# probcomp/PClean

Hardware: AMD Instinct MI355X
Metric: rows/sec per Gibbs sweep on 1M-row synthetic hospital; F1 vs ground truth (higher is better)
Workload: dtype f64

## Files before the change

### pclean_amd/csrc/eval.hip

```cpp
#include "sweep_internal.h"
#include "static_tiles.h"

int build_gauss_dev(pclean_ctx* ctx, const pclean_gauss& g, const CandTable* t, GaussDev& d) {
  memset(&d, 0, sizeof d);
  if (g.x_col < 0 || g.x_col >= ctx->n_xcols) return pclean_fail(ctx, PCLEAN_ERR_ARG, "gauss: numeric column out of range");
  const MeanTable& m = ctx->mean[g.mean_table];
  if (!m.valid) return pclean_fail(ctx, PCLEAN_ERR_STATE, "gauss: mean table %d not set", g.mean_table);
  d.on = 1;
  d.n_dims = g.n_dims;
  d.n_locals = g.n_locals;
  d.x = ctx->xnum.p + (size_t)g.x_col * ctx->n_rows + ctx->active_begin;
  d.mu = m.v.p;
  for (int i = 0; i < g.n_dims; ++i) {
    d.src_kind[i] = g.src_kind[i];
    d.src_slot[i] = g.src[i];
    d.stride[i] = g.stride[i];
    d.src_ptr[i] = nullptr;
    if (g.src_kind[i] == PCLEAN_GSRC_CAND) {
      if (!t || g.src[i] < 0 || g.src[i] >= t->n_cols) return pclean_fail(ctx, PCLEAN_ERR_ARG, "gauss: candidate column out of range");
      d.src_ptr[i] = t->cols.p + (size_t)g.src[i] * t->n_rows;
    } else if (g.src_kind[i] == PCLEAN_GSRC_OBS) {
      if (g.src[i] < 0 || g.src[i] >= ctx->n_cols) return pclean_fail(ctx, PCLEAN_ERR_ARG, "gauss: observed column out of range");
      d.src_ptr[i] = ctx->obs.p + (size_t)g.src[i] * ctx->n_rows + ctx->active_begin;
    }
// ... 663 lines not shown
  fr.zero_row = f.zero_row.p;
  fr.alive = f.alive.p;
  fr.prior_e = c.leaf ? nullptr : f.prior_e.p;
  fr.prior_n = f.prior_n.p;
  fr.logc_m1 = c.leaf ? nullptr : t.logc_m1.p;
  fr.counts = c.leaf ? nullptr : t.counts.p;
  memcpy(fr.scal, t.scal, sizeof fr.scal);
}

static int try_fast_root(pclean_ctx* ctx, int block_id, int node_id, FastRootDev& fr, bool ev_mode = false) {
  if (node_id >= 64) return 0;
  const Block& b = ctx->block[block_id];
  const pclean_node& n = b.nodes[node_id];
  FastRootCall c{ctx, block_id, node_id, ev_mode, EvalSwitches::once(), b, n, ctx->cand[n.table], n.kind == PCLEAN_NODE_LEAF, fr};
  if (!fast_root_eligible(c)) return 0;
  int rc = ensure_compact_tables(c);
  if (!rc) rc = ensure_root_priors(c);
  if (rc) return rc;
  prefilter_bound(c);
  rc = ensure_obs_rowmajor(c);
  if (rc) return rc;
  fill_fast_root(c);
  return 1;
}

static int eval_node_lse(pclean_ctx* ctx, int block_id, int node_id, const ItemList& il, const int32_t* excl,
                         uint64_t seed, uint32_t sweep, double* lse_out);
static int make_item_groups(pclean_ctx* ctx, int block_id, int node_id, const ItemList& il, const int32_t* excl,
                            ItemGroups& g, int split_m = 0, bool want_members = true);

static double subtree_ub(pclean_ctx* ctx, const Block& b, int node_id) {
  const pclean_node& n = b.nodes[node_id];
  if (node_id < (int)b.node_gauss.size() && b.node_gauss[node_id] >= 0) return INFINITY;
  CandTable& t = ctx->cand[n.table];
  if (n.kind == PCLEAN_NODE_LEAF) {
    if (t.h_lse_ver != t.version) {
      double m = -INFINITY, acc = 0.0;
      for (double v : t.h_logc_full) m = std::max(m, v);
      if (m > -INFINITY)
        for (double v : t.h_logc_full) acc += std::exp(v - m);
      t.h_lse = m > -INFINITY ? m + std::log(acc) + 1e-9 : -INFINITY;
      t.h_lse_ver = t.version;
    }
    return t.h_lse;
  }
  double sum = 0.0;
  for (int c = 0; c < n.n_children; ++c) sum += subtree_ub(ctx, b, b.children[n.child_begin + c]);
  return std::max(0.0, sum);
}

__global__ void scatter_f64_kernel(int n, const int32_t* list, const double* src, double* dst) {
  const int j = blockIdx.x * blockDim.x + threadIdx.x;
  if (j < n) dst[list[j]] = src[j];
}
__global__ void sub_items_kernel(int n, const int32_t* list, const int32_t* p_row, const int32_t* p_ctx,
                                 const int32_t* p_excl, const int32_t* p_ev_lo, const int32_t* p_ev_hi,
                                 const int32_t* p_rng, const int32_t* p_origin, int32_t* row, int32_t* ctxv,
                                 int32_t* excl, int32_t* ev_lo, int32_t* ev_hi, int32_t* rng, int32_t* origin) {
  const int j = blockIdx.x * blockDim.x + threadIdx.x;
  if (j >= n) return;
  const int s = list[j];
  row[j] = p_row ? p_row[s] : s;
  excl[j] = p_excl ? p_excl[s] : -1;
  for (int c = 0; c < PCLEAN_MAX_CTX; ++c) ctxv[j * PCLEAN_MAX_CTX + c] = p_ctx ? p_ctx[(size_t)s * PCLEAN_MAX_CTX + c] : 0;
  if (p_ev_lo) {
    ev_lo[j] = p_ev_lo[s];
    ev_hi[j] = p_ev_hi[s];
  }
  if (p_rng) rng[j] = p_rng[s];
  if (origin) origin[j] = p_origin ? p_origin[s] : s;
}

__global__ void group_rep_items_kernel(int n, const int32_t* list, const int32_t* grp_off, const int32_t* members,
                                       const int32_t* p_row, const int32_t* p_ctx, const int32_t* p_excl, int32_t* row,
                                       int32_t* ctxv, int32_t* excl) {
  const int j = blockIdx.x * blockDim.x + threadIdx.x;
  if (j >= n) return;
  const int g = list ? list[j] : j;
  const int s = members[grp_off[g]];
  row[j] = p_row ? p_row[s] : s;
  excl[j] = p_excl ? p_excl[s] : -1;
  for (int c = 0; c < PCLEAN_MAX_CTX; ++c) ctxv[j * PCLEAN_MAX_CTX + c] = p_ctx ? p_ctx[(size_t)s * PCLEAN_MAX_CTX + c] : 0;
}
__global__ void group_scatter_f64_kernel(int n, const int32_t* list, const int32_t* grp_off, const int32_t* members,
                                         const double* src, double* dst) {
  const int j = blockIdx.x * blockDim.x + threadIdx.x;
  if (j >= n) return;
  const int g = list ? list[j] : j;
  const double v = src[j];
  const int hi = grp_off[g + 1];
  for (int mi = grp_off[g]; mi < hi; ++mi) dst[members[mi]] = v;
}

__global__ void member_scatter_f64_kernel(int n_pos, const int32_t* uid, const int32_t* members, const double* src, double* dst) {
  const int mi = blockIdx.x * blockDim.x + threadIdx.x;
  if (mi < n_pos) dst[members[mi]] = src[uid[mi] - 1];
}

struct EvalCall {
  pclean_ctx* ctx;
  const int block_id, node_id;
  const ItemList& il;
  const int32_t* excl;
  const uint64_t seed;
  const uint32_t sweep;
  const int n_draws;
  double* lse_out;
  int32_t* draws_out;
  double* scores_out;
  const double* snew_override;
  const bool time_it;
  Block& b;
  const pclean_node& n;
  SweepState* s;
  const uint32_t site;
  const EvalSwitches sw;
  SweepState::LazyReq lazy_req;
  bool lazy_ok = false;
  int fast_split_m = 0;
  bool tabulated = false;
  NodeDev nd;
  ItemsDev it;
  ChildrenDev ch{};
  FastRootDev fr;
  int fast = 0, fast_ev = 0;
  ItemGroups g_pre;
  ItemGroups ggrp;
  bool fast_tried = false, groups_tried = false;
  const double* pre_score = nullptr;
  const int32_t* pre_obs = nullptr;
  int32_t* oflag = nullptr;
  int32_t* over_list = nullptr;
  unsigned int* over_count = nullptr;
  bool list_mode = false, ev_list_mode = false;
};

static int eval_begin(EvalCall& c) {
  SweepState* s = c.s;
  const ItemList& il = c.il;
  c.lazy_req = s->lazy_req;
  s->lazy_req = SweepState::LazyReq();
  s->lazy_out.valid = false;
  c.lazy_ok = c.lazy_req.on && !c.sw.cached.no_lazy && c.n_draws > 1 && !il.rng_row && !il.ev_lo;
  const bool lazy_sure = c.lazy_ok && (size_t)il.n * ROOT_LZ_CAP * 12 <= ((size_t)4 << 30);
  c.fast_split_m = (lazy_sure && !c.sw.cached.lazy_split) ? 0 : std::max(4, 256 / std::max(c.n_draws, 1));
  int rc = build_node_dev(c.ctx, c.b, c.node_id, c.nd);
  if (rc) return rc;
  c.it = ItemsDev{il.n, 0, il.row, il.ctx, c.excl, c.n_draws == 1 ? il.particle : nullptr, s->row_offset + c.ctx->active_begin,
                  nullptr, il.ev_lo, il.ev_hi, il.ev_rows, il.ev_ctx, il.rng_row, nullptr, nullptr, il.draw_is, il.draw_ds,
                  nullptr, nullptr};
  if (il.ev_lo) {
    rc = ensure_agg(c.ctx, c.block_id, c.node_id, il, &c.it.agg);
    if (rc) return rc;
    c.it.ev_item = il.origin;
  }
  c.tabulated = node_has_tabulated(c.b, c.n);
  return PCLEAN_OK;
}

static int launch_enum_scratch(EvalCall& c, const ItemsDev& it, double* scores_out, const ProductDev* product) {
  double* sc_tmp = nullptr;
  if (!scores_out && !product) {
    const size_t sc_n = pclean_enum_split_scores(c.nd, it);
    if (sc_n && !(sc_tmp = scratch<double>(c.ctx, sc_n))) return pclean_fail(c.ctx, PCLEAN_ERR_HIP, "scratch alloc failed");
  }
  return pclean_launch_enum(c.ctx, c.nd, it, c.ch, c.seed, c.sweep, c.site, c.n_draws, c.lse_out, scores_out, c.draws_out, sc_tmp,
                            product);
}

static int sub_items(EvalCall& c, unsigned int n, const int32_t* list, int32_t* row2, int32_t* ctx2, int32_t* excl2, ItemList& sil) {
  const ItemList& il = c.il;
  int32_t* evl2 = il.ev_lo ? scratch<int32_t>(c.ctx, n) : nullptr;
  int32_t* evh2 = il.ev_lo ? scratch<int32_t>(c.ctx, n) : nullptr;
  int32_t* rng2 = il.rng_row ? scratch<int32_t>(c.ctx, n) : nullptr;
  int32_t* org2 = il.ev_lo ? scratch<int32_t>(c.ctx, n) : nullptr;
  if (!row2 || !ctx2 || !excl2 || (il.ev_lo && (!evl2 || !evh2 || !org2)) || (il.rng_row && !rng2))
    return pclean_fail(c.ctx, PCLEAN_ERR_HIP, "scratch alloc failed");
  hipLaunchKernelGGL(sub_items_kernel, grid1(n), dim3(256), 0, c.ctx->stream, (int)n, list, il.row, il.ctx, c.excl, il.ev_lo,
                     il.ev_hi, il.rng_row, il.origin, row2, ctx2, excl2, evl2, evh2, rng2, org2);
  sil = ItemList{(int)n, row2, il.ctx ? ctx2 : nullptr, nullptr, org2, evl2, evh2, il.ev_rows, il.ev_ctx, rng2};
  return PCLEAN_OK;
}

struct OpenUnits {
  bool grouped = false;
  int n_all = 0;
  unsigned int n_need = 0;
  int32_t* list = nullptr;
  ItemList sil;
  const int32_t* sexcl = nullptr;
  bool sub() const { return n_need < (unsigned int)n_all; }
};

static int children_bounds(EvalCall& c, GateDev& gt, int* n_open, bool* gate) {
  for (int k = 0; k < c.n.n_children; ++k) {
    const int cid = c.b.children[c.n.child_begin + k];
    const pclean_node& cn = c.b.nodes[cid];
    if (cn.kind == PCLEAN_NODE_LEAF && cn.cacheable) {
      const int rc = ensure_leaf_cache(c.ctx, c.block_id, cid, &c.ch.arr[k], &c.ch.obs_col[k], &c.ch.n_obs[k]);
      if (rc) return rc;
      gt.cache[k] = c.ch.arr[k];
      gt.obs_col[k] = c.ch.obs_col[k];
      gt.n_obs[k] = c.ch.n_obs[k];
      gt.ub[k] = 0.0;
      if (c.il.ev_lo) gt.ub[k] = subtree_ub(c.ctx, c.b, cid);
    } else {
      ++*n_open;
      gt.cache[k] = nullptr;
      gt.ub[k] = subtree_ub(c.ctx, c.b, cid);
      if (!(gt.ub[k] < INFINITY)) *gate = false;
    }
    if (c.il.ev_lo && !(gt.ub[k] < INFINITY)) *gate = false;
  }
  return PCLEAN_OK;
}

static int gate_and_compact(EvalCall& c, const GateDev& gt, SweepState::GateStat* gstat, OpenUnits& u) {
  pclean_ctx* ctx = c.ctx;
  SweepState* s = c.s;
  ProfScope ps(ctx, "gate_new_branch");
  const int n = u.n_all;
  int32_t* flag = scratch<int32_t>(ctx, n);
  u.list = scratch<int32_t>(ctx, n);
  double* sc = u.grouped ? scratch<double>(ctx, n) : nullptr;
  int32_t* ow = u.grouped ? scratch<int32_t>(ctx, (size_t)n * PCLEAN_MAX_TERMS) : nullptr;
  if (!flag || !u.list || (u.grouped && (!sc || !ow))) return pclean_fail(ctx, PCLEAN_ERR_HIP, "scratch alloc failed");
  if (u.grouped) {
    ItemsDev itg = c.it;
    itg.n = n;
    itg.grp_off = c.g_pre.grp_off;
    itg.members = c.g_pre.members;
    if (c.time_it && s->evg0) (void)hipEventRecord(s->evg0, ctx->stream);
    const int rc = pclean_launch_group_gate(ctx, c.fr, itg, gt, flag, sc, ow);
    if (rc) return rc;
    if (c.time_it && s->evg0) {
      (void)hipEventRecord(s->evg1, ctx->stream);
      s->gate_timed = true;
    }
  } else {
    if (s->counter.alloc(4)) return pclean_fail(ctx, PCLEAN_ERR_HIP, "device alloc failed");
    const int rc = pclean_launch_gate(ctx, c.nd, c.it, gt, flag);
    if (rc) return rc;
  }
  unsigned int* need_ctr = fresh_counter(ctx);
  if (!need_ctr) return pclean_fail(ctx, PCLEAN_ERR_HIP, "counter bank: device alloc failed");
  hipLaunchKernelGGL(compact_new_kernel, grid1(n), dim3(256), 0, ctx->stream, (size_t)n, flag, 1, need_ctr, u.list, nullptr);
  PCLEAN_READ_COUNT(ctx, need_ctr, &u.n_need);
  if (u.grouped) {
    c.pre_score = sc;
    c.pre_obs = ow;
  }
  if (gstat) {
    gstat->all_need_run = !u.sub() ? gstat->all_need_run + 1 : 0;
    if (gstat->all_need_run >= 3) {
      gstat->skip = 16;
      gstat->all_need_run = 2;
    }
  }
  if (!u.sub()) u.list = nullptr;
  return PCLEAN_OK;
}

static int open_sublist(EvalCall& c, OpenUnits& u) {
  const ItemList& il = c.il;
  if (!u.grouped) {
    u.sil = il;
    u.sexcl = c.excl;
  }
  if (u.n_need == 0 || (!u.grouped && !u.sub())) return PCLEAN_OK;
  int32_t* row2 = scratch<int32_t>(c.ctx, u.n_need);
  int32_t* ctx2 = scratch<int32_t>(c.ctx, (size_t)u.n_need * PCLEAN_MAX_CTX);
  int32_t* excl2 = scratch<int32_t>(c.ctx, u.n_need);
  if (u.grouped) {
    if (!row2 || !ctx2 || !excl2) return pclean_fail(c.ctx, PCLEAN_ERR_HIP, "scratch alloc failed");
    hipLaunchKernelGGL(group_rep_items_kernel, grid1(u.n_need), dim3(256), 0, c.ctx->stream, (int)u.n_need, u.list, c.g_pre.grp_off,
                       c.g_pre.members, il.row, il.ctx, c.excl, row2, ctx2, excl2);
    u.sil = ItemList{(int)u.n_need, row2, il.ctx ? ctx2 : nullptr, nullptr, nullptr};
  } else {
    const int rc = sub_items(c, u.n_need, u.list, row2, ctx2, excl2, u.sil);
    if (rc) return rc;
  }
  u.sexcl = excl2;
  return PCLEAN_OK;
}

static int eval_open_children(EvalCall& c, const OpenUnits& u) {
  pclean_ctx* ctx = c.ctx;
  const ItemList& il = c.il;
  const ItemList& sil = u.sil;
  const CandTable& t = ctx->cand[c.n.table];
  for (int k = 0; k < c.n.n_children; ++k) {
    const int cid = c.b.children[c.n.child_begin + k];
    const pclean_node& cn = c.b.nodes[cid];
    if (cn.kind == PCLEAN_NODE_LEAF && cn.cacheable) continue;
    double* child_lse = scratch<double>(ctx, il.n);
    if (!child_lse) return pclean_fail(ctx, PCLEAN_ERR_HIP, "scratch alloc failed");
    c.ch.arr[k] = child_lse;
    c.ch.obs_col[k] = nullptr;
    if (u.sub()) {
      hipLaunchKernelGGL(fill_f64_kernel, grid1(il.n), dim3(256), 0, ctx->stream, child_lse, (size_t)il.n, -__builtin_inf());
      if (u.n_need == 0) continue;
    }
    const int32_t* child_excl = nullptr;
    if (cn.kind == PCLEAN_NODE_FK && u.sexcl) {
      if (cn.parent_fk_col < 0 || cn.parent_fk_col >= t.n_cols)
        return pclean_fail(ctx, PCLEAN_ERR_ARG, "node %d: parent_fk_col out of range", cid);
      int32_t* ce = scratch<int32_t>(ctx, sil.n);
      if (!ce) return pclean_fail(ctx, PCLEAN_ERR_HIP, "scratch alloc failed");
      hipLaunchKernelGGL(derive_excl_kernel, grid1(sil.n), dim3(256), 0, ctx->stream, sil.n, u.sexcl, t.counts.p,
                         t.cols.p + (size_t)cn.parent_fk_col * t.n_rows, ce);
      child_excl = ce;
    }
    double* dst = child_lse;
    if (u.grouped || u.sub()) {
      dst = scratch<double>(ctx, sil.n);
      if (!dst) return pclean_fail(ctx, PCLEAN_ERR_HIP, "scratch alloc failed");
    }
    const int rc = eval_node_lse(ctx, c.block_id, cid, sil, child_excl, c.seed, c.sweep, dst);
    if (rc) return rc;
    if (u.grouped && !u.list && c.g_pre.uid && c.fast_split_m == 0)
      hipLaunchKernelGGL(member_scatter_f64_kernel, grid1(il.n), dim3(256), 0, ctx->stream, il.n, c.g_pre.uid, c.g_pre.members, dst,
                         child_lse);
    else if (u.grouped)
      hipLaunchKernelGGL(group_scatter_f64_kernel, grid1(sil.n), dim3(256), 0, ctx->stream, sil.n, u.list, c.g_pre.grp_off,
                         c.g_pre.members, dst, child_lse);
    else if (u.sub())
      hipLaunchKernelGGL(scatter_f64_kernel, grid1(sil.n), dim3(256), 0, ctx->stream, sil.n, u.list, dst, child_lse);
  }
  return PCLEAN_OK;
}

static int new_row_branch(EvalCall& c) {
  pclean_ctx* ctx = c.ctx;
  const pclean_node& n = c.n;
  const ItemList& il = c.il;
  if (n.kind != PCLEAN_NODE_FK) return PCLEAN_OK;
  if (ctx->prior_mode) {
    c.ch.n = 0;
    return PCLEAN_OK;
  }
  if (c.snew_override) {
    c.ch.n = 1;
    c.ch.arr[0] = c.snew_override;
    c.ch.obs_col[0] = nullptr;
    return PCLEAN_OK;
  }
  if (n.n_children > PCLEAN_MAX_CHILDREN) return pclean_fail(ctx, PCLEAN_ERR_CAPACITY, "too many children");
  c.ch.n = n.n_children;
  GateDev gt{};
  gt.n = n.n_children;
  bool gate = c.excl && !c.scores_out && il.n >= c.sw.live.gate_min() && !c.sw.live.no_gate();
  SweepState::GateStat* gstat = (gate && c.node_id < 64 && c.sweep < 0x7ffffff0u && !il.ev_lo && !c.sw.live.gate_always())
                                    ? &c.s->gate_stat[c.block_id * 64 + c.node_id] : nullptr;
  if (gstat && gstat->skip > 0) {
    --gstat->skip;
    gate = false;
    gstat = nullptr;
  }
  int n_open = 0;
  int rc = children_bounds(c, gt, &n_open, &gate);
  if (rc) return rc;
  OpenUnits u;
  if (n_open > 0 && c.n_draws > 0 && c.excl && !c.scores_out && !ctx->force_generic && !c.nd.g.on && !c.tabulated && !il.rng_row &&
      !il.ev_lo && !c.sw.cached.no_group_gate) {
    c.fast = try_fast_root(ctx, c.block_id, c.node_id, c.fr);
    if (c.fast < 0) return c.fast;
    c.fast_tried = true;
    if (c.fast) {
      rc = make_item_groups(ctx, c.block_id, c.node_id, il, c.excl, c.g_pre, c.fast_split_m);
      if (rc) return rc;
      c.groups_tried = true;
      u.grouped = c.g_pre.n_groups > 0;
    }
  }
  u.n_all = u.grouped ? c.g_pre.n_groups : il.n;
  u.n_need = (unsigned int)u.n_all;
  if (gate && n_open > 0) {
    rc = gate_and_compact(c, gt, gstat, u);
    if (rc) return rc;
  }
  rc = open_sublist(c, u);
  if (rc) return rc;
  return eval_open_children(c, u);
}

static int leaf_coarse_draw(EvalCall& c, bool* done) {
  pclean_ctx* ctx = c.ctx;
  *done = c.n.kind == PCLEAN_NODE_LEAF && c.n.cacheable && !c.il.ev_lo && !c.scores_out && !ctx->force_generic && !ctx->obs_override &&
          !c.sw.cached.no_coarse && !c.nd.g.on && !c.tabulated && !ctx->prior_mode;
  if (!*done) return PCLEAN_OK;
  const double* cache = nullptr;
  const int32_t* ocol = nullptr;
  int n_obs = 0;
  const int rc = ensure_leaf_cache(ctx, c.block_id, c.node_id, &cache, &ocol, &n_obs);
  if (rc) return rc;
  ProfScope ps(ctx, "option_list_coarse_draw");
  return pclean_launch_leaf_coarse_draw(ctx, c.nd, c.it, ocol, n_obs, pclean_leaf_coarse_blocks(c.nd.n_cand), cache,
                                        c.b.leaf_m[c.node_id].p, c.b.leaf_U[c.node_id].p, c.b.leaf_coarse[c.node_id].p, c.seed,
                                        c.sweep, PCLEAN_SITE_NODE(c.block_id, c.node_id), c.n_draws, c.lse_out, c.draws_out);
}

static int choose_compact_path(EvalCall& c) {
  pclean_ctx* ctx = c.ctx;
  const ItemList& il = c.il;
  const bool small_lse = !c.sw.cached.no_small_generic && c.n_draws == 0 && il.n <= 1024 && !il.ev_lo &&
                         (size_t)(c.nd.n_cand + 2) * 8 + (16 + 64) * 8 <= (size_t)160 * 1024;
  if (c.fast_tried || c.scores_out || c.snew_override || ctx->force_generic || c.nd.g.on || c.tabulated || ctx->prior_mode || small_lse)
    return PCLEAN_OK;
  if (!il.ev_lo)
    c.fast = try_fast_root(ctx, c.block_id, c.node_id, c.fr);
  else if ((c.n.kind == PCLEAN_NODE_LEAF || (il.n >= c.sw.cached.ev_slot_min_items && !c.sw.live.no_fast_ev_slots())) && c.n_draws <= 1 &&
           !c.sw.live.no_fast_ev())
    c.fast_ev = try_fast_root(ctx, c.block_id, c.node_id, c.fr, true);
  if (c.fast < 0) return c.fast;
  if (c.fast_ev < 0) return c.fast_ev;
  if (c.fast_ev) {
    bool any = false;
    for (int i = 0; i < c.fr.n_terms; ++i) any |= c.fr.terms[i].comp != nullptr;
    if (!any) c.fast_ev = 0;
  }
  return PCLEAN_OK;
}

static int group_for_launch(EvalCall& c) {
  const ItemList& il = c.il;
  const int nc = c.nd.n_cand + (c.n.kind == PCLEAN_NODE_FK ? 1 : 0);
  const bool lds_kernel = (size_t)((nc + 1) & ~1) * 8 + (16 + 64) * 8 <= 160 * 1024;
  if (!(c.n_draws > 0 && !c.scores_out && !c.snew_override && !c.ctx->force_generic && !il.rng_row && !il.ev_lo &&
        (c.fast || lds_kernel)))
    return PCLEAN_OK;
  ItemGroups g = c.g_pre;
  if (!c.groups_tried) {
    const int rc = make_item_groups(c.ctx, c.block_id, c.node_id, il, c.excl, g, c.fast ? c.fast_split_m : 0);
    if (rc) return rc;
  }
  if (g.n_groups > 0) {
    c.it.n = g.n_groups;
    c.it.grp_off = g.grp_off;
    c.it.members = g.members;
    if (c.fast && c.fast_split_m == 0) c.it.grp_uid = g.uid;
    c.ggrp = g;
  }
  return PCLEAN_OK;
}

static void note_root_stats(EvalCall& c) {
  pclean_root_stats& rs = c.ctx->root_stats;
  rs = pclean_root_stats{};
  rs.fast = c.fast;
  rs.n_items = c.il.n;
  rs.n_groups = c.it.n;
  rs.n_cand = c.nd.n_cand;
  rs.n_terms = c.n.n_terms;
  rs.n_draws = c.n_draws;
  rs.pre_scored = c.pre_score ? 1 : 0;
  if (c.fast) {
    const FastRootDev& fr = c.fr;
    rs.kpad = fr.kscan;
    rs.cstride = std::min(fr.cstride, (((fr.kscan + 63) >> 6) + 15) & ~15);
    rs.n_pre = fr.n_pre;
    for (int p = 0; p < 3; ++p) rs.pre_obs_col[p] = p < fr.n_pre ? c.b.terms[c.n.term_begin + fr.pre[p]].obs_col : -1;
  }
}

static int launch_generic(EvalCall& c) {
  ProductDev prd;
  const bool product = pclean_product_plan(c.ctx->cand[c.n.table], c.nd, c.it, &prd);
  ProfScope ps(c.ctx, c.n.kind == PCLEAN_NODE_FK ? "enum_fk_generic" : (product ? "enum_leaf_product" : "enum_leaf_generic"));
  if (c.time_it) (void)hipEventRecord(c.s->ev0, c.ctx->stream);
  const int rc = launch_enum_scratch(c, c.it, c.scores_out, product ? &prd : nullptr);
  if (c.time_it) (void)hipEventRecord(c.s->ev1, c.ctx->stream);
  return rc;
}

static int overflow_setup(EvalCall& c) {
  pclean_ctx* ctx = c.ctx;
  SweepState* s = c.s;
  const ItemList& il = c.il;
  c.oflag = scratch<int32_t>(ctx, il.n);
  if (!c.oflag || s->counter.alloc(4)) return pclean_fail(ctx, PCLEAN_ERR_HIP, "scratch alloc failed");
  c.list_mode = c.fast && !c.sw.cached.no_fast_over && pclean_overflow_fast_ok(c.fr, c.it) && s->over_rec.size() < OVER_SLOTS &&
                s->over_ctr.p != nullptr;
// ... 1050 lines not shown
    if (k0 == k[0] && e[1] == k[1] && e[2] == k[2]) {
      lse_out[i] = m.vals[slot];
      miss = 0;
      break;
    }
    slot = (slot + 1) & m.cap_mask;
  }
  miss_flag[i] = miss;
}
__global__ void memo_insert_kernel(int n, const int32_t* list, KeyColsDev kc, const int32_t* row, const int32_t* ctxv,
                                   MemoDev m, const double* __restrict__ src) {
  const int j = blockIdx.x * blockDim.x + threadIdx.x;
  if (j >= n) return;
  if (*m.count >= m.max_fill) return;
  const int i = list ? list[j] : j;
  uint64_t k[3];
  memo_key(kc, row ? row[i] : i, ctxv, (size_t)i, k);
  uint32_t slot = memo_hash(k) & m.cap_mask;
  for (int p = 0; p < MEMO_PROBES; ++p) {
    unsigned long long* e = (unsigned long long*)(m.keys + (size_t)slot * 3);
    const unsigned long long old = atomicCAS(e, ~0ull, (unsigned long long)k[0]);
    if (old == ~0ull) {
      e[1] = k[1];
      e[2] = k[2];
      m.vals[slot] = src[j];
      atomicAdd(m.count, 1u);
      return;
    }
    slot = (slot + 1) & m.cap_mask;
  }
}

static int eval_node_lse_core(pclean_ctx* ctx, int block_id, int node_id, const ItemList& il, const int32_t* excl,
                              uint64_t seed, uint32_t sweep, double* lse_out);

static int eval_node_lse(pclean_ctx* ctx, int block_id, int node_id, const ItemList& il, const int32_t* excl,
                         uint64_t seed, uint32_t sweep, double* lse_out) {
  Block& b = ctx->block[block_id];
  const pclean_node& n = b.nodes[node_id];
  SweepState* s = st(ctx);
  std::set<int> cols;
  bool use_ctx = false;
  static const bool no_memo = getenv("PCLEAN_NO_MEMO") != nullptr;
  const bool memo_ok = !no_memo && n.kind == PCLEAN_NODE_LEAF && !il.ev_lo && il.n >= 4096 && node_id < 64 &&
                       subtree_key(ctx, b, node_id, cols, use_ctx) &&
                       (int)cols.size() + (use_ctx ? PCLEAN_MAX_CTX : 0) <= 6 && (!use_ctx || il.ctx);
  if (!memo_ok) return eval_node_lse_core(ctx, block_id, node_id, il, excl, seed, sweep, lse_out);
  ProfScope ps(ctx, "option_marginal_memo");
  uint64_t ver = ctx->cand[n.table].version;
  for (int i = 0; i < n.n_terms; ++i) {
    const pclean_term& tm = b.terms[n.term_begin + i];
    ver = ver * 1000003ull + ctx->pair[tm.pair_table].version;
    if (tm.ctx_slot >= 0) ver = ver * 1000003ull + (uint64_t)(tm.fn_table + 1);
    if (tm.dens_kind == PCLEAN_DENS_NAME3) {
      for (const Name3Term& x : b.name3)
        if (x.term == n.term_begin + i) ver = ver * 1000003ull + ctx->pair[x.suffix_table].version;
      ver = ver * 1000003ull + b.version;
    }
  }
  SweepState::LeafMemo& mm = s->memo[block_id * 64 + node_id];
  const int cap = 1 << 21;
  if (mm.cap != cap) {
    if (mm.keys.alloc((size_t)cap * 3) || mm.vals.alloc(cap) || mm.count.alloc(4))
      return pclean_fail(ctx, PCLEAN_ERR_HIP, "device alloc failed (memo)");
    mm.cap = cap;
    mm.ver = 0;
  }
  if (mm.ver != ver) {
    HIPCHK(ctx, hipMemsetAsync(mm.keys.p, 0xff, (size_t)cap * 3 * sizeof(uint64_t), ctx->stream));
    HIPCHK(ctx, hipMemsetAsync(mm.count.p, 0, sizeof(unsigned int), ctx->stream));
    mm.ver = ver;
  }
  MemoDev md{mm.keys.p, mm.vals.p, mm.count.p, (unsigned int)(cap - 1), (unsigned int)(cap / 2)};
  KeyColsDev kc{};
  kc.use_ctx = use_ctx ? 1 : 0;
  for (int c : cols) kc.col[kc.n_cols++] = ctx->obs.p + (size_t)c * ctx->n_rows + ctx->active_begin;
  const int N = il.n;
  int32_t* flag = scratch<int32_t>(ctx, N);
  int32_t* list = scratch<int32_t>(ctx, N);
  if (!flag || !list || s->counter.alloc(4)) return pclean_fail(ctx, PCLEAN_ERR_HIP, "scratch alloc failed");
  hipLaunchKernelGGL(memo_lookup_kernel, grid1(N), dim3(256), 0, ctx->stream, N, kc, il.row, il.ctx, md, lse_out, flag);
  unsigned int* miss_ctr = fresh_counter(ctx);
  if (!miss_ctr) return pclean_fail(ctx, PCLEAN_ERR_HIP, "counter bank: device alloc failed");
  hipLaunchKernelGGL(compact_new_kernel, grid1(N), dim3(256), 0, ctx->stream, (size_t)N, flag, 1, miss_ctr, list, nullptr);
  unsigned int n_miss = 0;
  PCLEAN_READ_COUNT(ctx, miss_ctr, &n_miss);
  if (n_miss == 0) return PCLEAN_OK;
  if (n_miss == (unsigned int)N) {
    int rc = eval_node_lse_core(ctx, block_id, node_id, il, excl, seed, sweep, lse_out);
    if (rc) return rc;
    hipLaunchKernelGGL(memo_insert_kernel, grid1(N), dim3(256), 0, ctx->stream, N, (const int32_t*)nullptr, kc, il.row,
                       il.ctx, md, lse_out);
    return PCLEAN_OK;
  }
  int32_t* row2 = scratch<int32_t>(ctx, n_miss);
  int32_t* ctx2 = scratch<int32_t>(ctx, (size_t)n_miss * PCLEAN_MAX_CTX);
  int32_t* excl2 = scratch<int32_t>(ctx, n_miss);
  double* dst = scratch<double>(ctx, n_miss);
  if (!row2 || !ctx2 || !excl2 || !dst) return pclean_fail(ctx, PCLEAN_ERR_HIP, "scratch alloc failed");
  hipLaunchKernelGGL(sub_items_kernel, grid1(n_miss), dim3(256), 0, ctx->stream, (int)n_miss, list, il.row, il.ctx, excl,
                     (const int32_t*)nullptr, (const int32_t*)nullptr, (const int32_t*)nullptr, (const int32_t*)nullptr, row2,
                     ctx2, excl2, (int32_t*)nullptr, (int32_t*)nullptr, (int32_t*)nullptr, (int32_t*)nullptr);
  ItemList sil{(int)n_miss, row2, il.ctx ? ctx2 : nullptr, nullptr, nullptr};
  int rc = eval_node_lse_core(ctx, block_id, node_id, sil, excl ? excl2 : nullptr, seed, sweep, dst);
  if (rc) return rc;
  hipLaunchKernelGGL(scatter_f64_kernel, grid1(n_miss), dim3(256), 0, ctx->stream, (int)n_miss, list, dst, lse_out);
  hipLaunchKernelGGL(memo_insert_kernel, grid1(n_miss), dim3(256), 0, ctx->stream, (int)n_miss, list, kc, il.row, il.ctx, md,
                     dst);
  return PCLEAN_OK;
}

static int eval_node_lse_core(pclean_ctx* ctx, int block_id, int node_id, const ItemList& il, const int32_t* excl,
                              uint64_t seed, uint32_t sweep, double* lse_out) {
  ItemGroups g;
  int rc0 = make_item_groups(ctx, block_id, node_id, il, excl, g, 0, false);
  if (rc0) return rc0;
  if (g.n_groups == 0)
    return eval_node(ctx, block_id, node_id, il, excl, seed, sweep, 0, lse_out, nullptr, nullptr, nullptr, false);
  const int n = il.n;
  const int32_t n_unique = g.n_groups;
  int32_t* uid_of_item = scratch<int32_t>(ctx, n);
  if (!uid_of_item) return pclean_fail(ctx, PCLEAN_ERR_HIP, "scratch alloc failed");
  int32_t* row2 = scratch<int32_t>(ctx, n_unique);
  int32_t* ctx2 = scratch<int32_t>(ctx, (size_t)n_unique * PCLEAN_MAX_CTX);
  int32_t* excl2 = scratch<int32_t>(ctx, n_unique);
  double* lse_u = scratch<double>(ctx, n_unique);
  if (!row2 || !ctx2 || !excl2 || !lse_u) return pclean_fail(ctx, PCLEAN_ERR_HIP, "scratch alloc failed");
  if (g.hg_incl)
    hipLaunchKernelGGL(hg_unique_kernel, grid1(n), dim3(256), 0, ctx->stream, n, g.hg_incl, g.hg_rep, g.hg_slot_of, il.row, il.ctx,
                       excl, uid_of_item, row2, ctx2, excl2);
  else
    hipLaunchKernelGGL(item_unique_kernel, grid1(n), dim3(256), 0, ctx->stream, n, g.members, g.head, g.uid, il.row, il.ctx, excl,
                       uid_of_item, row2, ctx2, excl2);
  ItemList il2;
  il2.n = n_unique;
  il2.row = row2;
  il2.ctx = il.ctx ? ctx2 : nullptr;
  int rc = eval_node(ctx, block_id, node_id, il2, excl ? excl2 : nullptr, seed, sweep, 0, lse_u, nullptr, nullptr, nullptr,
                     false);
  if (rc) return rc;
  hipLaunchKernelGGL(gather_f64_kernel, grid1(n), dim3(256), 0, ctx->stream, n, uid_of_item, lse_u, lse_out);
  return PCLEAN_OK;
}

int sample_children(pclean_ctx* ctx, int block_id, int node_id, const ItemList& il, const int32_t* excl,
                           uint64_t seed, uint32_t sweep, int32_t* vals, int n_nodes) {
  Block& b = ctx->block[block_id];
  const pclean_node& n = b.nodes[node_id];
  const CandTable& t = ctx->cand[n.table];
  for (int c = 0; c < n.n_children; ++c) {
    const int cid = b.children[n.child_begin + c];
    const pclean_node& cn = b.nodes[cid];
    int32_t* draws = scratch<int32_t>(ctx, il.n);
    if (!draws) return pclean_fail(ctx, PCLEAN_ERR_HIP, "scratch alloc failed");
    const int32_t* child_excl = nullptr;
    if (cn.kind == PCLEAN_NODE_FK && excl) {
      int32_t* ce = scratch<int32_t>(ctx, il.n);
      if (!ce) return pclean_fail(ctx, PCLEAN_ERR_HIP, "scratch alloc failed");
      hipLaunchKernelGGL(derive_excl_kernel, grid1(il.n), dim3(256), 0, ctx->stream, il.n, excl, t.counts.p,
                         t.cols.p + (size_t)cn.parent_fk_col * t.n_rows, ce);
      child_excl = ce;
    }
    int rc = eval_node(ctx, block_id, cid, il, child_excl, seed, sweep, 1, nullptr, draws, nullptr, nullptr, false);
    if (rc) return rc;
    hipLaunchKernelGGL(scatter_vals_kernel, grid1(il.n), dim3(256), 0, ctx->stream, il.n, il.origin, draws, n_nodes,
                       cid, vals);
    if (cn.kind == PCLEAN_NODE_FK && cn.n_children > 0) {
      unsigned int* new_ctr = fresh_counter(ctx);
      if (!new_ctr) return pclean_fail(ctx, PCLEAN_ERR_HIP, "counter bank: device alloc failed");
      hipLaunchKernelGGL(compact_new_kernel, grid1(il.n), dim3(256), 0, ctx->stream, (size_t)il.n, draws, 0, new_ctr, nullptr,
                         nullptr);
      unsigned int cnt = 0;
      PCLEAN_READ_COUNT(ctx, new_ctr, &cnt);
      if (cnt) {
        int32_t* list = scratch<int32_t>(ctx, cnt);
        int32_t* row = scratch<int32_t>(ctx, cnt);
        int32_t* cx = scratch<int32_t>(ctx, (size_t)cnt * PCLEAN_MAX_CTX);
        int32_t* part = scratch<int32_t>(ctx, cnt);
        int32_t* org = scratch<int32_t>(ctx, cnt);
        int32_t* sub_excl = scratch<int32_t>(ctx, cnt);
        if (!list || !row || !cx || !part || !org || !sub_excl) return pclean_fail(ctx, PCLEAN_ERR_HIP, "scratch alloc failed");
        unsigned int* list_ctr = fresh_counter(ctx);
        if (!list_ctr) return pclean_fail(ctx, PCLEAN_ERR_HIP, "counter bank: device alloc failed");
        hipLaunchKernelGGL(compact_new_kernel, grid1(il.n), dim3(256), 0, ctx->stream, (size_t)il.n, draws, 1, list_ctr, list, nullptr);
        int32_t* evl = il.ev_lo ? scratch<int32_t>(ctx, cnt) : nullptr;
        int32_t* evh = il.ev_lo ? scratch<int32_t>(ctx, cnt) : nullptr;
        int32_t* rng = il.rng_row ? scratch<int32_t>(ctx, cnt) : nullptr;
        if ((il.ev_lo && (!evl || !evh)) || (il.rng_row && !rng)) return pclean_fail(ctx, PCLEAN_ERR_HIP, "scratch alloc failed");
        hipLaunchKernelGGL(sublist_items_kernel, grid1(cnt), dim3(256), 0, ctx->stream, (int)cnt, list, il.row, il.ctx,
                           il.particle, il.origin, row, cx, part, org, il.ev_lo, il.ev_hi, il.rng_row, evl, evh, rng);
        if (child_excl)
          hipLaunchKernelGGL(gather_i32_kernel, grid1(cnt), dim3(256), 0, ctx->stream, (int)cnt, list, child_excl,
                             sub_excl);
        ItemList sub{(int)cnt, row, cx, part, org, evl, evh, il.ev_rows, il.ev_ctx, rng};
        rc = sample_children(ctx, block_id, cid, sub, child_excl ? sub_excl : nullptr, seed, sweep, vals, n_nodes);
        if (rc) return rc;
      }
    }
  }
  return PCLEAN_OK;
}

int prefetch_fast_root(pclean_ctx* ctx, int block_id, int node_id, hipStream_t side) {
  hipStream_t saved = ctx->stream;
  ctx->stream = side;
  FastRootDev fr;
  const int rc = try_fast_root(ctx, block_id, node_id, fr);
  ctx->stream = saved;
  return rc < 0 ? rc : PCLEAN_OK;
}

extern "C" int pclean_prepare(pclean_ctx* ctx, uint32_t ev_blocks) {
  if (!ctx) return PCLEAN_ERR_ARG;
  HIPCHK(ctx, hipSetDevice(ctx->device));
  {
    const int rcb = begin_call(ctx);
    if (rcb) return rcb;
  }
  for (int bi = 0; bi < PCLEAN_MAX_BLOCKS; ++bi) {
    Block& b = ctx->block[bi];
    if (!b.valid || b.is_score) continue;
    for (int node = 0; node < (int)b.nodes.size() && node < 64; ++node) {
      const pclean_node& n = b.nodes[node];
      if (n.table < 0 || n.table >= PCLEAN_MAX_TABLES || !ctx->cand[n.table].valid) continue;
      if (node < (int)b.node_gauss.size() && b.node_gauss[node] >= 0) continue;
      FastRootDev fr;
      const int rc = try_fast_root(ctx, bi, node, fr, n.kind == PCLEAN_NODE_LEAF && ((ev_blocks >> bi) & 1u));
      if (rc < 0) return rc;
      if (n.kind == PCLEAN_NODE_LEAF && n.cacheable && n.n_terms == 1 && b.terms[n.term_begin].ctx_slot < 0) {
        const double* cache;
        const int32_t* ocol;
        int n_obs;
        const int rcl = ensure_leaf_cache(ctx, bi, node, &cache, &ocol, &n_obs);
        if (rcl) return rcl;
      }
    }
  }
  PCLEAN_SYNC(ctx);
  return PCLEAN_OK;
}

int ensure_plan_dev(pclean_ctx* ctx, int block_id) {
  SweepState* s = st(ctx);
  BlockRun& r = s->run[block_id];
  const Block& b = ctx->block[block_id];
  const int nn = (int)b.nodes.size();
  std::vector<int32_t> kind(nn), nrows(nn), cmb(nn);
  std::vector<const int32_t*> cols(nn);
  for (int i = 0; i < nn; ++i) {
    const CandTable& t = ctx->cand[b.nodes[i].table];
    kind[i] = b.nodes[i].kind;
    nrows[i] = t.n_rows;
    cmb[i] = b.nodes[i].colmap_begin;
    cols[i] = t.cols.p;
  }
  if (r.plan_ready && r.plan_sig_block == b.version && r.plan_sig_nrows == nrows && r.plan_sig_cols == cols && r.plan_sig_colmap == b.colmap.size() &&
// ... 24 lines not shown
```

### pclean_amd/csrc/sweep.hip

```cpp
#include <optional>

#include "sweep_internal.h"
#include "tail_tiles.h"

int g_pclean_sync_count = 0;

__global__ void publish_count_kernel(const unsigned int* __restrict__ src, volatile unsigned int* __restrict__ dst, unsigned int seq) {
  dst[0] = *src;
  __threadfence_system();
  dst[1] = seq;
}
int read_count(pclean_ctx* ctx, const void* dev, void* out, const char* func, int line) {
  SweepState* s = st(ctx);
  static const bool no_poll = getenv("PCLEAN_NO_POLL") != nullptr;
  static const bool trace = getenv("PCLEAN_TRACE_SYNC") != nullptr;
  if (trace) fprintf(stderr, "[pclean sync %d] %s:%d (count)\n", ++g_pclean_sync_count, func, line);
  if (!no_poll && !s->h_poll) {
    if (hipHostMalloc((void**)&s->h_poll, 64, hipHostMallocMapped | hipHostMallocCoherent) != hipSuccess) s->h_poll = nullptr;
    if (s->h_poll) {
      s->h_poll[0] = s->h_poll[1] = 0;
      if (hipHostGetDevicePointer((void**)&s->d_poll, (void*)s->h_poll, 0) != hipSuccess) {
        (void)hipHostFree((void*)s->h_poll);
        s->h_poll = nullptr;
      }
    }
  }
  if (no_poll || !s->h_poll) {
    HIPCHK(ctx, hipMemcpyAsync(out, dev, 4, hipMemcpyDeviceToHost, ctx->stream));
    HIPCHK(ctx, hipStreamSynchronize(ctx->stream));
    return PCLEAN_OK;
  }
  const unsigned int seq = ++s->poll_seq;
  hipLaunchKernelGGL(publish_count_kernel, dim3(1), dim3(1), 0, ctx->stream, (const unsigned int*)dev, s->d_poll, seq);
  if (s->on_first_wait) {
    std::function<int()> f;
    f.swap(s->on_first_wait);
    const int rcf = f();
    if (rcf) return rcf;
  }
  volatile unsigned int* h = s->h_poll;
  for (long spins = 0; h[1] != seq; ++spins)
    if (spins > 2000000) {
      HIPCHK(ctx, hipStreamSynchronize(ctx->stream));
      if (h[1] != seq) return pclean_fail(ctx, PCLEAN_ERR_HIP, "count read-back: the publishing kernel did not run");
    }
  *(unsigned int*)out = h[0];
  return PCLEAN_OK;
}

__device__ int32_t resolve_new_value(const PlanDev& pl, int node, int col, const int32_t* vals) {
  for (int depth = 0; depth < 16; ++depth) {
    const int cn = pl.colmap[2 * (pl.colmap_begin[node] + col)];
    const int cc = pl.colmap[2 * (pl.colmap_begin[node] + col) + 1];
    if (cn < 0) return -1;
    const int choice = vals[cn];
    if (pl.kind[cn] == PCLEAN_NODE_LEAF) return pl.cols[cn][choice];
    if (choice >= 0) return pl.cols[cn][(size_t)cc * pl.n_rows[cn] + choice];
    node = cn;
    col = cc;
  }
  return -1;
}




struct CtxSrc {
  int32_t n_ctx;
  const int32_t* pchoice[PCLEAN_MAX_CTX];
  const int32_t* pnewpos[PCLEAN_MAX_CTX];
  const int32_t* vals[PCLEAN_MAX_CTX];
  int32_t n_nodes[PCLEAN_MAX_CTX];
  const int32_t* root_col[PCLEAN_MAX_CTX];
  int32_t col[PCLEAN_MAX_CTX];
  PlanDev plan[PCLEAN_MAX_CTX];
};

__global__ void gather_ctx_kernel(size_t NP, CtxSrc cs, int32_t* it_ctx) {
  size_t t = (size_t)blockIdx.x * blockDim.x + threadIdx.x;
  if (t >= NP) return;
  for (int s = 0; s < cs.n_ctx; ++s) {
    int32_t v;
    const int choice = cs.pchoice[s][t];
    if (choice >= 0)
      v = cs.root_col[s][choice];
    else
      v = resolve_new_value(cs.plan[s], 0, cs.col[s], cs.vals[s] + (size_t)cs.pnewpos[s][t] * cs.n_nodes[s]);
    it_ctx[(size_t)s * NP + t] = v;
  }
}

__global__ void ctx_count_kernel(int N, int P, int n_ctx, const int32_t* __restrict__ it_ctx, int32_t* __restrict__ rep,
                                 int32_t* __restrict__ n_distinct) {
  const int i = blockIdx.x * blockDim.x + threadIdx.x;
  if (i >= N) return;
  const size_t NP = (size_t)N * P;
  int nd = 0;
  for (int p = 0; p < P; ++p) {
    const size_t sp = (size_t)p * N + i;
    int c[PCLEAN_MAX_CTX];
    for (int k = 0; k < PCLEAN_MAX_CTX; ++k) c[k] = k < n_ctx ? it_ctx[(size_t)k * NP + sp] : 0;
    int q = 0;
    for (; q < p; ++q) {
      bool same = true;
      for (int k = 0; k < PCLEAN_MAX_CTX; ++k)
        if (k < n_ctx) same &= it_ctx[(size_t)k * NP + (size_t)q * N + i] == c[k];
      if (same) break;
    }
    rep[sp] = q;
    nd += q == p ? 1 : 0;
  }
  n_distinct[i] = nd;
}
__global__ void ctx_fill_kernel(int N, int P, int n_ctx, const int32_t* __restrict__ it_ctx, const int32_t* __restrict__ rep,
                                const int32_t* __restrict__ off, const int32_t* __restrict__ cur_b,
                                int32_t* __restrict__ slot_item, int32_t* __restrict__ row, int32_t* __restrict__ ctxv,
                                int32_t* __restrict__ excl) {
  const int i = blockIdx.x * blockDim.x + threadIdx.x;
  if (i >= N) return;
  const size_t NP = (size_t)N * P;
  int j = off[i];
  for (int p = 0; p < P; ++p) {
    const size_t sp = (size_t)p * N + i;
    const int q = rep[sp];
    if (q == p) {
      row[j] = i;
      excl[j] = cur_b ? cur_b[i] : -1;
      for (int k = 0; k < PCLEAN_MAX_CTX; ++k) ctxv[(size_t)j * PCLEAN_MAX_CTX + k] = k < n_ctx ? it_ctx[(size_t)k * NP + sp] : 0;
      slot_item[sp] = j++;
    } else {
// ... 44 lines not shown
            it_ctx[(size_t)s * NP + (size_t)(p0 + u) * N + i] = v[u];
            all_same &= v[u] == c0[s];
          }
      }
    }
    row[i] = i;
    excl[i] = cur_b ? cur_b[i] : -1;
    for (int k = 0; k < PCLEAN_MAX_CTX; ++k) ctxv[(size_t)i * PCLEAN_MAX_CTX + k] = c0[k];
    if (all_same) {
      for (int p = 0; p < P; ++p) slot_item[(size_t)p * N + i] = i;
    } else {
      slot_item[i] = i;
      for (int p = 1; p < P; ++p) {
        const size_t sp = (size_t)p * N + i;
        int q = 0;
        for (; q < p; ++q) {
          bool same = true;
          for (int k = 0; k < cs.n_ctx; ++k) same &= it_ctx[(size_t)k * NP + (size_t)q * N + i] == it_ctx[(size_t)k * NP + sp];
          if (same) break;
        }
        if (q == p) {
          slot_item[sp] = -1 - (int)mine;
          ++mine;
        } else {
          slot_item[sp] = slot_item[(size_t)q * N + i];
        }
      }
    }
  }
  const unsigned long long any = __ballot(mine != 0u);
  unsigned int incl = mine;
  if (any) {
    for (int o = 1; o < 64; o <<= 1) {
      const unsigned int x = __shfl_up(incl, o, 64);
      if (lane >= o) incl += x;
    }
  }
  if (lane == 63) wcnt[wave] = any ? incl : 0u;
  __syncthreads();
  if (threadIdx.x == 0) {
    const unsigned int tot = wcnt[0] + wcnt[1] + wcnt[2] + wcnt[3];
    bbase = tot ? atomicAdd(n_extra, tot) : 0u;
  }
  __syncthreads();
  if (!mine) return;
  unsigned int base = bbase + incl - mine;
  for (int w = 0; w < wave; ++w) base += wcnt[w];
  for (int p = 1; p < P; ++p) {
    const size_t sp = (size_t)p * N + i;
    const int si = slot_item[sp];
    if (si >= 0) continue;
    int q = 0;
    for (; q < p; ++q) {
      bool same = true;
      for (int k = 0; k < cs.n_ctx; ++k) same &= it_ctx[(size_t)k * NP + (size_t)q * N + i] == it_ctx[(size_t)k * NP + sp];
      if (same) break;
    }
    if (q < p) {
      slot_item[sp] = slot_item[(size_t)q * N + i];
      continue;
    }
    const unsigned int e = base + (unsigned int)(-1 - si);
    const int j = N + (int)e;
    slot_item[sp] = j;
    if (e < (unsigned int)extra_cap) {
      row[j] = i;
      excl[j] = cur_b ? cur_b[i] : -1;
      for (int k = 0; k < PCLEAN_MAX_CTX; ++k) ctxv[(size_t)j * PCLEAN_MAX_CTX + k] = k < cs.n_ctx ? it_ctx[(size_t)k * NP + sp] : 0;
    }
  }
}
#define PU_T 1024
__global__ __launch_bounds__(PU_T) void particle_update_kernel(int N, int P, const int32_t* __restrict__ draws_rm,
                                                              const double* __restrict__ lse,
                                                              const int32_t* __restrict__ slot_item,
                                                              const int32_t* __restrict__ draws_item,
                                                              const double* __restrict__ lse_item,
                                                              const int32_t* __restrict__ cur_b,
                                                              int32_t* __restrict__ pchoice, double* __restrict__ w,
                                                              unsigned int* __restrict__ n_new,
                                                              int32_t* __restrict__ new_list,
                                                              int32_t* __restrict__ pnewpos, int first,
                                                              const int32_t* __restrict__ emit_rows, int only_emit,
                                                              int stage_stride, const double* __restrict__ w_uni, int skip_w) {
  __shared__ unsigned int wsum[PU_T / 64];
  __shared__ unsigned int bbase;
  extern __shared__ int32_t pu_stage[];
  const int i = blockIdx.x * blockDim.x + threadIdx.x;
  const int lane = threadIdx.x & 63, wave = threadIdx.x >> 6;
  if (stage_stride > 0) {
    const int r0 = blockIdx.x * PU_T;
    const int n_here = min(PU_T, N - r0);
    const int n_words = n_here * P;
    const int32_t* src = draws_rm + (size_t)r0 * P;
    for (int k = threadIdx.x; k < n_words; k += PU_T) {
      const int row = k / P, col = k - row * P;
      pu_stage[row * stage_stride + col] = src[k];
    }
    __syncthreads();
  }
  uint64_t newmask = 0;
  if (i < N && !(only_emit && !emit_rows[i])) {
    const int keep = cur_b ? cur_b[i] : -1;
    for (int p = 0; p < P; ++p) {
      const size_t sp = (size_t)p * N + i;
      int d;
      double l;
      if (slot_item) {
        const int item = slot_item[sp];
        d = draws_item[(size_t)item * P + p];
        l = lse_item[item];
      } else {
        d = stage_stride > 0 ? pu_stage[threadIdx.x * stage_stride + p] : draws_rm[(size_t)i * P + p];
        l = lse[i];
      }
      const int c = (p == 0 && keep >= 0) ? keep : d;
      pchoice[sp] = c;
      if (!skip_w) w[sp] = first ? 0.0 + l : (w_uni ? (0.0 + w_uni[i]) + l : w[sp] + l);
      if (c == PCLEAN_CHOICE_NEW) newmask |= 1ull << p;
      if (p == 0 && !(l > -__builtin_inf())) atomicOr(n_new, 0x80000000u);
    }
    if (emit_rows && !emit_rows[i]) newmask = 0;
  }
  const unsigned int mine = (unsigned int)__popcll(newmask);
  unsigned int incl = mine;
  for (int o = 1; o < 64; o <<= 1) {
    const unsigned int x = __shfl_up(incl, o, 64);
    if (lane >= o) incl += x;
  }
  if (lane == 63) wsum[wave] = incl;
  __syncthreads();
  if (threadIdx.x == 0) {
    unsigned int total = 0;
    for (int k = 0; k < PU_T / 64; ++k) total += wsum[k];
    bbase = total ? (atomicAdd(n_new, total) & 0x7fffffffu) : 0u;
  }
  __syncthreads();
  if (!mine) return;
  unsigned int pos = bbase + incl - mine;
  for (int k = 0; k < wave; ++k) pos += wsum[k];
  for (uint64_t mm = newmask; mm; mm &= mm - 1) {
    const int p = __builtin_ctzll(mm);
    const size_t sp = (size_t)p * N + i;
    new_list[pos] = (int32_t)sp;
    pnewpos[sp] = (int32_t)pos;
    ++pos;
  }
}

__global__ void chosen_new_kernel(int N, const int32_t* __restrict__ chosen, const int32_t* __restrict__ pchoice,
                                  unsigned int* __restrict__ counter, int32_t* __restrict__ list,
                                  int32_t* __restrict__ pnewpos) {
  const int i = blockIdx.x * blockDim.x + threadIdx.x;
  if (i >= N) return;
  const size_t s = (size_t)chosen[i] * N + i;
  if (pchoice[s] != PCLEAN_CHOICE_NEW) return;
  const unsigned int pos = atomicAdd(counter, 1u);
  list[pos] = (int32_t)s;
  pnewpos[s] = (int32_t)pos;
}

struct SrcDev {
  const int32_t* pchoice;
  const int32_t* pnewpos;
  const int32_t* vals;
  const int32_t* root_col;
  int32_t n_nodes, col;
  PlanDev plan;
};
__device__ __forceinline__ int src_value(const SrcDev& s, size_t slot) {
  const int choice = s.pchoice[slot];
  if (choice >= 0) return s.root_col[choice];
  return resolve_new_value(s.plan, 0, s.col, s.vals + (size_t)s.pnewpos[slot] * s.n_nodes);
}
struct ScoreTermDev {
  const int32_t* obs_col;
  const uint8_t* pair;
  const int32_t* nopt_fn;
  int32_t n_lat, other_val;
  SrcDev val, key;
};
struct ScoreBlockDev {
  int32_t n_terms, prob_nb;
  const int32_t* prob_fn;
  const double* prob_same;
  const double* prob_diff;
  const double* logn;
  SrcDev pa, pb;
  ScoreTermDev t[8];
};
__global__ void score_block_kernel(int n_rows, int P, ScoreBlockDev sb, double* w) {
  size_t slot = (size_t)blockIdx.x * blockDim.x + threadIdx.x;
  if (slot >= (size_t)n_rows * P) return;
  const int i = (int)(slot % n_rows);
  const int pidx = sb.prob_fn[(size_t)src_value(sb.pa, slot) * sb.prob_nb + src_value(sb.pb, slot)];
  double acc = 0.0;
  for (int k = 0; k < sb.n_terms; ++k) {
    const ScoreTermDev& t = sb.t[k];
    const int val = src_value(t.val, slot);
    const int o = t.obs_col[i];
    double dens;
    if (o < 0)
      dens = val >= t.other_val ? -1000.0 : 0.0;
    else if (t.pair[(size_t)o * t.n_lat + val] == 0)
      dens = sb.prob_same[pidx];
    else
      dens = sb.prob_diff[pidx] - sb.logn[t.nopt_fn[src_value(t.key, slot)]];
    acc += dens;
  }
  w[slot] += acc;
}

__global__ void materialise_w_kernel(int N, int P, const double* __restrict__ w_uni, double* __restrict__ w) {
  const int i = blockIdx.x * blockDim.x + threadIdx.x;
  if (i >= N) return;
  const double v = 0.0 + w_uni[i];
  for (int p = 0; p < P; ++p) w[(size_t)p * N + i] = v;
}
__global__ void add_weight_kernel(size_t n, const double* lse, double* w) {
  size_t t = (size_t)blockIdx.x * blockDim.x + threadIdx.x;
  if (t < n) w[t] += lse[t];
}



__global__ void rootlist_items_kernel(int n, int N, size_t NP, const int32_t* list, const int32_t* b_ctx,
                                      const int32_t* cur_b, int32_t* row, int32_t* ctxv, int32_t* particle,
                                      int32_t* origin, int32_t* excl) {
  int j = blockIdx.x * blockDim.x + threadIdx.x;
  if (j >= n) return;
  const int slot = list[j];
  const int i = slot % N;
  row[j] = i;
  particle[j] = slot / N;
  origin[j] = j;
  excl[j] = cur_b ? cur_b[i] : -1;
  for (int c = 0; c < PCLEAN_MAX_CTX; ++c) ctxv[j * PCLEAN_MAX_CTX + c] = b_ctx ? b_ctx[(size_t)c * NP + slot] : 0;
}

__global__ void set_col_kernel(int n, int n_nodes, int node, int32_t v, int32_t* vals) {
  int j = blockIdx.x * blockDim.x + threadIdx.x;
  if (j < n) vals[(size_t)j * n_nodes + node] = v;
}
__global__ void gather_items_kernel(int n, const int32_t* list, const int32_t* row, const int32_t* ctxv,
                                    const int32_t* excl, const int32_t* particle, int32_t* row2, int32_t* ctx2,
                                    int32_t* excl2, int32_t* part2) {
  int j = blockIdx.x * blockDim.x + threadIdx.x;
  if (j >= n) return;
  const int s = list[j];
  row2[j] = row ? row[s] : s;
  excl2[j] = excl ? excl[s] : -1;
  part2[j] = particle ? particle[s] : 0;
  for (int c = 0; c < PCLEAN_MAX_CTX; ++c) ctx2[j * PCLEAN_MAX_CTX + c] = ctxv ? ctxv[(size_t)s * PCLEAN_MAX_CTX + c] : 0;
}


template <int PMAX>
__global__ void maybe_resample_kernel(int n_rows, int P, const double* logw, size_t sr, size_t sp, int retain_first,
                                      const int32_t* csmc_flag, uint64_t seed, uint32_t sweep, uint32_t block,
                                      int64_t row_offset, int32_t* ancestors, double* logml_inc, double* ess_out,
                                      int32_t* did) {
  int i = blockIdx.x * blockDim.x + threadIdx.x;
  if (i >= n_rows) return;
  FixW<PMAX> f;
  fix_weights<PMAX>(logw + (size_t)i * sr, sp, P, f);
  const double Ud = (double)f.U;
  double s2 = 0.0;
#pragma unroll
  for (int p = 0; p < PMAX; ++p)
    if (p < P) s2 += (double)f.u[p] * (double)f.u[p];
  const double ess = f.U ? (Ud * Ud) / s2 : 0.0;
  if (ess_out) ess_out[i] = ess;
  const bool retain = csmc_flag ? (csmc_flag[i] >= 0) : (retain_first != 0);
  int32_t* anc = ancestors + (size_t)i * sr;
  if (ess < (double)P / 2.0) {
    const uint32_t rr = (uint32_t)((int64_t)i + row_offset);
    for (int p = 0; p < P; ++p) {
      if (p == 0 && retain)
        anc[0] = 0;
      else
        anc[(size_t)p * sp] = fix_pick<PMAX>(f, P, pclean_rand64(seed, rr, PCLEAN_SITE_RESAMPLE(block), (uint32_t)p, sweep));
    }
    logml_inc[i] = pclean_lse_from_fix(f.m, f.U) - pclean_log((double)P);
    if (did) did[i] = 1;
  } else {
    for (int p = 0; p < P; ++p) anc[(size_t)p * sp] = p;
    logml_inc[i] = 0.0;
    if (did) did[i] = 0;
  }
}

struct AncestorArrays {
  int32_t* p[2 * PCLEAN_MAX_BLOCKS];
  int64_t* pairs[PCLEAN_MAX_BLOCKS];
  int n_pairs;
};
__global__ void apply_ancestors_kernel(int n_rows, int P, const int32_t* ancestors, int n_arrays, AncestorArrays arrays,
                                       double* w, const int32_t* did, const double* logml_inc, double* logml_acc) {
  int i = blockIdx.x * blockDim.x + threadIdx.x;
  if (i >= n_rows) return;
  logml_acc[i] += logml_inc[i];
  if (!did[i]) return;
  int32_t tmp[MAXP];
  for (int a = 0; a < n_arrays; ++a) {
    int32_t* arr = arrays.p[a] + i;
    for (int p = 0; p < P; ++p) tmp[p] = arr[(size_t)ancestors[(size_t)p * n_rows + i] * n_rows];
    for (int p = 0; p < P; ++p) arr[(size_t)p * n_rows] = tmp[p];
  }
  for (int a = 0; a < arrays.n_pairs; ++a) {
    int64_t* arr = arrays.pairs[a] + i;
    int64_t t2[MAXP];
    for (int p = 0; p < P; ++p) t2[p] = arr[(size_t)ancestors[(size_t)p * n_rows + i] * n_rows];
    for (int p = 0; p < P; ++p) arr[(size_t)p * n_rows] = t2[p];
  }
  for (int p = 0; p < P; ++p) w[(size_t)p * n_rows + i] = 0.0;
}

template <int PMAX>
__global__ void final_choice_kernel(int n_rows, int P, const double* logw, size_t sr, size_t sp, int use_mh,
                                    int is_csmc, const int32_t* csmc_flag, uint64_t seed, uint32_t sweep,
                                    int64_t row_offset, int32_t* chosen, double* log_total, const double* logml_acc,
                                    double* logml, const int32_t* __restrict__ only_rows) {
  int i = blockIdx.x * blockDim.x + threadIdx.x;
  if (i >= n_rows) return;
  if (only_rows && !only_rows[i]) return;
  FixW<PMAX> f;
// ... 88 lines not shown
  const uint32_t rr = (uint32_t)((int64_t)i + row_offset);
  const bool csmc = csmc_flag[i] >= 0;
  int c;
  if (use_mh && csmc && P >= 2) {
    const double Ud = (double)f.U;
    const double w0 = (double)f.u[0] / Ud, w1 = (double)f.u[PMAX > 1 ? 1 : 0] / Ud;
    double ratio = w1 / (1e-10 + w0);
    if (ratio > 1.0) ratio = 1.0;
    const double x = pclean_u01(pclean_rand64(seed, rr, PCLEAN_SITE_MH, 0u, sweep));
    c = (f.U != 0 && x < ratio) ? 1 : 0;
  } else {
    c = fix_pick<PMAX>(f, P, pclean_rand64(seed, rr, PCLEAN_SITE_FINAL, 0u, sweep));
  }
  chosen[i] = c;
  logml[i] = logml_acc[i] + pclean_lse_from_fix(f.m, f.U) - pclean_log((double)P);
}

__global__ __launch_bounds__(256) void finalize_block_kernel(int n_rows, const int32_t* chosen, const int32_t* pchoice,
                                                             const int32_t* pnewpos, const int32_t* cur_b,
                                                             int32_t* choice, int32_t* chosen_newpos,
                                                             unsigned long long* stats, int hist_rows,
                                                             int32_t* moved_flag, int32_t* new_flag,
                                                             unsigned int* __restrict__ wg_moved,
                                                             unsigned int* __restrict__ wg_new) {
  extern __shared__ int32_t hist[];
  for (int k = threadIdx.x; k < hist_rows; k += 256) hist[k] = 0;
  if (hist_rows) __syncthreads();
  int i = blockIdx.x * blockDim.x + threadIdx.x;
  int is_moved = 0, is_new = 0;
  if (i < n_rows) {
    const size_t s = (size_t)chosen[i] * n_rows + i;
    const int c = pchoice[s];
    const int o = cur_b[i];
    choice[i] = c;
    const int np = c == PCLEAN_CHOICE_NEW ? pnewpos[s] : -1;
    chosen_newpos[i] = np;
    new_flag[i] = is_new = np >= 0 ? 1 : 0;
    moved_flag[i] = is_moved = c != o ? 1 : 0;
    if (o != c) {
      if (hist_rows) {
        if (o >= 0) atomicAdd(&hist[o], -1);
        if (c >= 0) atomicAdd(&hist[c], 1);
      } else {
        if (o >= 0) atomicAdd(&stats[o], (unsigned long long)(-1ll));
        if (c >= 0) atomicAdd(&stats[c], 1ull);
      }
    }
  }
  if (hist_rows) {
    __syncthreads();
    for (int k = threadIdx.x; k < hist_rows; k += 256) {
      const int v = hist[k];
      if (v) atomicAdd(&stats[k], (unsigned long long)(long long)v);
    }
  }
  const int n_moved = __syncthreads_count(is_moved), n_newr = __syncthreads_count(is_new);
  if (threadIdx.x == 0) {
    wg_moved[blockIdx.x] = (unsigned int)n_moved;
    wg_new[blockIdx.x] = (unsigned int)n_newr;
  }
}

struct TailBlock {
  const int32_t* pchoice;
  int32_t* pnewpos;
  const int32_t* cur_b;
  int32_t* choice;
  int32_t* chosen_newpos;
  unsigned long long* stats;
  int32_t* moved_flag;
  int32_t* new_flag;
  unsigned int* wg_moved;
  unsigned int* wg_new;
  unsigned int* new_ctr;
  int32_t* new_slots;
  int32_t hist_rows, on, lazy, pad;
};
struct TailBlocks {
  TailBlock b[PCLEAN_MAX_BLOCKS];
};
#define TAIL_WG_THREADS 1024
#define TAIL_STEP (TAIL_WG_THREADS / TAIL_TILE_ROWS)
__global__ __launch_bounds__(TAIL_WG_THREADS) void finalize_tail_kernel(int n_rows, int n_tiles, const int32_t* __restrict__ chosen,
                                                                        TailBlocks tb) {
  extern __shared__ int32_t hist[];
  __shared__ unsigned int wcnt[2][2][TAIL_WG_THREADS / 64];
  const TailBlock& b = tb.b[blockIdx.y];
  if (!b.on) return;
  const TailTileRange tr = tail_tile_range(n_tiles, (int)gridDim.x, (int)blockIdx.x);
  if (tr.begin >= tr.end) return;
  const int hist_rows = b.hist_rows;
  const int lane = threadIdx.x & 63, wave = threadIdx.x >> 6;
  const int sub = threadIdx.x / TAIL_TILE_ROWS, in_tile = threadIdx.x % TAIL_TILE_ROWS;
  for (int k = threadIdx.x; k < hist_rows; k += TAIL_WG_THREADS) hist[k] = 0;
  if (hist_rows) __syncthreads();
  int ch_next = 0, o_next = 0;
  {
    const int i0 = (tr.begin + sub) * TAIL_TILE_ROWS + in_tile;
    if (tr.begin + sub < tr.end && i0 < n_rows) {
      ch_next = chosen[i0];
      o_next = b.cur_b[i0];
    }
  }
  for (int t0 = tr.begin; t0 < tr.end; t0 += TAIL_STEP) {
    const int tile = t0 + sub;
    const bool mine = tile < tr.end;
    const int i = mine ? tile * TAIL_TILE_ROWS + in_tile : n_rows;
    const int par = ((t0 - tr.begin) / TAIL_STEP) & 1;
    bool is_moved = false, is_new = false, wants_pos = false;
    size_t s = 0;
    int c = 0;
    const int ch = ch_next, o = o_next;
    {
      const int i1 = (tile + TAIL_STEP) * TAIL_TILE_ROWS + in_tile;
      if (tile + TAIL_STEP < tr.end && i1 < n_rows) {
        ch_next = chosen[i1];
        o_next = b.cur_b[i1];
      }
    }
    if (i < n_rows) {
      s = (size_t)ch * n_rows + i;
      c = b.pchoice[s];
      wants_pos = b.lazy && c == PCLEAN_CHOICE_NEW;
    }
    int np = -1;
    if (b.lazy) {
      const unsigned long long mk = __ballot(wants_pos);
      if (mk) {
        unsigned int base = 0;
        if (lane == __builtin_ctzll(mk)) base = atomicAdd(b.new_ctr, (unsigned int)__popcll(mk));
        base = __shfl(base, __builtin_ctzll(mk), 64);
        if (wants_pos) {
          np = (int)(base + (unsigned int)__popcll(mk & ((1ull << lane) - 1ull)));
          b.new_slots[np] = (int32_t)s;
          b.pnewpos[s] = np;
        }
      }
    } else if (i < n_rows && c == PCLEAN_CHOICE_NEW) {
      np = b.pnewpos[s];
    }
    if (i < n_rows) {
      b.choice[i] = c;
      b.chosen_newpos[i] = np;
      is_new = np >= 0;
      is_moved = c != o;
      b.new_flag[i] = is_new ? 1 : 0;
      b.moved_flag[i] = is_moved ? 1 : 0;
      if (o != c) {
        if (hist_rows) {
          if (o >= 0) atomicAdd(&hist[o], -1);
          if (c >= 0) atomicAdd(&hist[c], 1);
        } else {
          if (o >= 0) atomicAdd(&b.stats[o], (unsigned long long)(-1ll));
          if (c >= 0) atomicAdd(&b.stats[c], 1ull);
        }
      }
    }
    const unsigned long long mm = __ballot(is_moved), mn = __ballot(is_new);
    if (lane == 0) {
      wcnt[par][0][wave] = (unsigned int)__popcll(mm);
      wcnt[par][1][wave] = (unsigned int)__popcll(mn);
    }
    __syncthreads();
    if (in_tile == 0 && mine) {
      b.wg_moved[tile] = wcnt[par][0][wave] + wcnt[par][0][wave + 1] + wcnt[par][0][wave + 2] + wcnt[par][0][wave + 3];
      b.wg_new[tile] = wcnt[par][1][wave] + wcnt[par][1][wave + 1] + wcnt[par][1][wave + 2] + wcnt[par][1][wave + 3];
    }
  }
  if (hist_rows) {
    __syncthreads();
    for (int k = threadIdx.x; k < hist_rows; k += TAIL_WG_THREADS) {
      const int v = hist[k];
      if (v) atomicAdd(&b.stats[k], (unsigned long long)(long long)v);
    }
  }
}

#define TAIL_MAX_LISTS (2 * PCLEAN_MAX_BLOCKS)
#define TAIL_CUS_PER_WG 2
__global__ __launch_bounds__(1024) void tail_scan_kernel(int nb, unsigned int* __restrict__ wg_cnt, int32_t* __restrict__ totals) {
  __shared__ unsigned int wsum[16];
  unsigned int* c = wg_cnt + (size_t)blockIdx.x * nb;
  const int lane = threadIdx.x & 63, wave = threadIdx.x >> 6;
  unsigned int carry = 0;
  for (int base = 0; base < nb; base += 1024) {
    const int j = base + threadIdx.x;
    const unsigned int v = j < nb ? c[j] : 0u;
    unsigned int incl = v;
    for (int o = 1; o < 64; o <<= 1) {
      const unsigned int x = __shfl_up(incl, o, 64);
      if (lane >= o) incl += x;
    }
    if (lane == 63) wsum[wave] = incl;
    __syncthreads();
    unsigned int wbase = 0, tot = 0;
    for (int k = 0; k < 16; ++k) {
      if (k < wave) wbase += wsum[k];
      tot += wsum[k];
    }
    if (j < nb) c[j] = carry + wbase + incl - v;
    carry += tot;
    __syncthreads();
  }
  if (threadIdx.x == 0) totals[blockIdx.x] = (int32_t)carry;
}
struct TailLists {
  const int32_t* flag[TAIL_MAX_LISTS];
  int32_t* list[TAIL_MAX_LISTS];
};
__global__ __launch_bounds__(256) void tail_scatter_kernel(int n_rows, int nb, TailLists tl, const unsigned int* __restrict__ wg_off) {
  __shared__ unsigned int wcnt[4];
  const int l = blockIdx.y;
  const int32_t* flag = tl.flag[l];
  if (!flag) return;
  const int i = blockIdx.x * 256 + threadIdx.x;
  const int lane = threadIdx.x & 63, wave = threadIdx.x >> 6;
  const bool f = i < n_rows && flag[i] != 0;
  const unsigned long long mk = __ballot(f);
  if (lane == 0) wcnt[wave] = (unsigned int)__popcll(mk);
  __syncthreads();
  if (!f) return;
  unsigned int pos = wg_off[(size_t)l * nb + blockIdx.x] + (unsigned int)__popcll(mk & ((1ull << lane) - 1ull));
  for (int w = 0; w < wave; ++w) pos += wcnt[w];
  tl.list[l][pos] = i;
}

__global__ void gauss_prior_kernel(int n_rows, int P, GaussDev g0, const GaussDev* __restrict__ more, int n_more, PlanDev plan,
                                   const int32_t* __restrict__ pchoice,
                                   const int32_t* __restrict__ pnewpos, const int32_t* __restrict__ vals, int n_nodes,
                                   const int32_t* __restrict__ cur_b, const int32_t* __restrict__ cur_locals, uint64_t seed,
                                   uint32_t sweep, uint32_t block, int64_t row_offset, double* __restrict__ w,
                                   int32_t* __restrict__ plocals) {
  const size_t slot = (size_t)blockIdx.x * blockDim.x + threadIdx.x;
  if (slot >= (size_t)n_rows * P) return;
  const int p = (int)(slot / (size_t)n_rows), i = (int)(slot % (size_t)n_rows);
  const int choice = pchoice[slot];
  const int32_t* v = choice >= 0 ? nullptr : vals + (size_t)pnewpos[slot] * n_nodes;
  const bool keep = p == 0 && cur_b && cur_b[i] >= 0 && cur_locals;
  const uint32_t rr = (uint32_t)((int64_t)i + row_offset);
  int l[2] = {0, 0}, out[2] = {-1, -1};
  double s = 0.0;
  for (int k = 0; k < g0.n_locals; ++k) {
    const int o = g0.local_obs[k] ? g0.local_obs[k][i] : -1;
    if (o >= 0) {
      l[k] = o;
      s += g0.local_logp[k];
    } else if (keep && cur_locals[2 * (size_t)i + k] >= 0) {
      l[k] = cur_locals[2 * (size_t)i + k];
    } else {
      l[k] = (int)pclean_mulhi64(pclean_rand64(seed, rr, PCLEAN_SITE_LOCALS(block), (uint32_t)p | ((uint32_t)(k + 1) << 16), sweep),
                                 (uint64_t)g0.local_n[k]);
// ... 160 lines not shown
        if (o < 0) continue;
        if (L < 0) {
          const uint64_t key = pclean_dummy_seed(seed, PCLEAN_SITE_NODE(dp.site_block, lf.node), (uint32_t)particle, sweep);
          L = dummy_draw_string(key, (uint32_t)((int64_t)row + row_offset), lf.min_len, lf.max_len, dp.lm_init, dp.lm_trans,
                                dp.letter_sym, drawn);
        }
        const int sid = tm.obs_ids[o];
        const uint16_t* os = dp.sym + dp.off[sid];
        const int ol = (int)(dp.off[sid + 1] - dp.off[sid]);
        if (ol > DUMMY_MAX_LEN) {
          dp.dp_ctr[1] = 1u;
          continue;
        }
        int16_t* H = dp.dp + (size_t)jl * dp.slot_cells + tm.dp_off;
        const int d = dummy_distance(tm.dist_mode, os, ol, drawn, L, H);
        double l;
        if (tm.max_typos >= 0 && d > tm.max_typos) {
          l = -1e5;
        } else {
          l = dp.nb[(size_t)((L + 4) / 5) * dp.nb_stride + d];
          l -= dp.logl[L] * (double)d;
          l -= 1.629048269010741 * (double)d;
        }
        const size_t pi = (size_t)o * tm.n_lat + lf.dummy_val;
        const int dph = tm.elem_bytes == 1 ? (int)tm.pair[pi] : (int)((const uint16_t*)tm.pair)[pi];
        double lph;
        if (tm.max_typos >= 0 && dph > tm.max_typos) {
          lph = -1e5;
        } else {
          const int Lp = tm.lat_len[lf.dummy_val];
          lph = dp.nb[(size_t)((Lp + 4) / 5) * dp.nb_stride + dph];
          lph -= dp.logl[Lp] * (double)dph;
          lph -= 1.629048269010741 * (double)dph;
        }
        c += l - lph;
      }
    }
    corr += c;
  }
  if (any) w[slot] += corr;
}


void pclean_sweep_state_free(pclean_ctx* ctx) {
  if (!ctx->sweep_state) return;
  SweepState* s = (SweepState*)ctx->sweep_state;
  for (auto& b : s->pool) b.release();
  for (auto& r : s->run) {
    r.pchoice.release(); r.pnewpos.release(); r.draws.release(); r.moved_flag.release(); r.new_flag.release();
    r.moved_list.release(); r.new_list.release(); r.new_slots.release();
    r.locals.release(); r.it_ctx.release(); r.choice.release(); r.chosen_newpos.release(); r.vals.release();
    r.lse.release(); r.plan_kind.release(); r.plan_nrows.release(); r.plan_cmb.release(); r.plan_colmap.release();
    r.plan_cols.release();
  }
  s->did.release(); s->cur.release(); s->chosen.release(); s->ancestors.release(); s->csmc_flag.release(); s->w.release();
  s->log_total.release(); s->logml_inc.release(); s->logml_acc.release(); s->logml.release(); s->counter.release();
  s->arr_ptrs.release();
  for (auto& kv : s->leaf_iota) kv.second.release();
  for (auto& f : s->fast) {
    for (auto& c : f.comp) c.release();
    for (auto& c : f.clen) c.release();
    for (auto& c : f.cblk) c.release();
    f.prior_e.release();
    f.prior_n.release();
    f.alive.release();
    f.zero_row.release();
  }
  s->tail_counts.release();
  for (auto& kv : s->tuple_ids) kv.second.release();
  for (auto& kv : s->memo) {
    kv.second.keys.release();
    kv.second.vals.release();
    kv.second.count.release();
  }
  if (s->h_counts) (void)hipHostFree(s->h_counts);
  if (s->h_over) (void)hipHostFree(s->h_over);
  for (int k = 0; k < SweepState::MAX_SIDE; ++k) {
    if (s->side[k]) (void)hipStreamDestroy(s->side[k]);
    if (s->side_join[k]) (void)hipEventDestroy(s->side_join[k]);
    if (s->side_mid[k]) (void)hipEventDestroy(s->side_mid[k]);
  }
  if (s->side_fork) (void)hipEventDestroy(s->side_fork);
  if (s->h_poll) (void)hipHostFree((void*)s->h_poll);
  s->dummy_dp.release();
  s->dummy_ctr.release();
  s->over_ctr.release();
  for (auto& b : s->more_banks) b.release();
  for (auto e : s->prof_ev) (void)hipEventDestroy(e);
  if (s->ev0) (void)hipEventDestroy(s->ev0);
  if (s->ev1) (void)hipEventDestroy(s->ev1);
  if (s->pre_stream) (void)hipStreamDestroy(s->pre_stream);
  if (s->pre_fork) (void)hipEventDestroy(s->pre_fork);
  if (s->pre_join) (void)hipEventDestroy(s->pre_join);
  if (s->evg0) (void)hipEventDestroy(s->evg0);
  if (s->evg1) (void)hipEventDestroy(s->evg1);
  if (s->evs) (void)hipEventDestroy(s->evs);
  if (s->eve) (void)hipEventDestroy(s->eve);
  delete s;
  ctx->sweep_state = nullptr;
}

int begin_call(pclean_ctx* ctx) {
  SweepState* s = st(ctx);
  s->pool_used = 0;
  s->dbg_desc = nullptr;
  s->dummy_used = false;
  ctx->prior_mode = false;
  s->over_rec.clear();
  if (s->over_ctr.alloc(OVER_SLOTS + STAT_WORDS + CTR_BANK)) return pclean_fail(ctx, PCLEAN_ERR_HIP, "device alloc failed");
  { const int rcz = dev_zero(ctx, s->over_ctr.p, (OVER_SLOTS + STAT_WORDS + CTR_BANK) * sizeof(unsigned int)); if (rcz) return rcz; }
  s->bank_used = 0;
  s->scan_stats_used = false;
  return PCLEAN_OK;
}
__global__ void dev_zero_kernel(uint4* __restrict__ p16, size_t n16, unsigned char* __restrict__ tail, int n_tail) {
  const size_t stride = (size_t)gridDim.x * blockDim.x;
  for (size_t i = (size_t)blockIdx.x * blockDim.x + threadIdx.x; i < n16; i += stride) p16[i] = make_uint4(0u, 0u, 0u, 0u);
  if (blockIdx.x == 0 && (int)threadIdx.x < n_tail) tail[threadIdx.x] = 0;
}
int dev_zero(pclean_ctx* ctx, void* p, size_t bytes) {
  static const bool off = getenv("PCLEAN_NO_ZERO_KERNEL") != nullptr;
  if (bytes == 0) return PCLEAN_OK;
  unsigned char* b = static_cast<unsigned char*>(p);
  const size_t head = (16 - ((uintptr_t)b & 15)) & 15;
  if (!off && bytes <= 256) {
    hipLaunchKernelGGL(dev_zero_kernel, dim3(1), dim3(256), 0, ctx->stream, (uint4*)nullptr, (size_t)0, b, (int)bytes);
    return PCLEAN_OK;
  }
  if (off || head > 0) {
    HIPCHK(ctx, hipMemsetAsync(p, 0, bytes, ctx->stream));
    return PCLEAN_OK;
  }
  const size_t n16 = bytes >> 4;
  const int n_tail = (int)(bytes & 15);
  const unsigned int blocks = (unsigned int)std::min<size_t>(std::max<size_t>((n16 + 255) / 256, 1), 4096);
  hipLaunchKernelGGL(dev_zero_kernel, dim3(blocks), dim3(256), 0, ctx->stream, reinterpret_cast<uint4*>(b), n16, b + (n16 << 4), n_tail);
  return PCLEAN_OK;
}
__global__ void publish_regions_kernel(const SweepState::PubRegions pr) {
  const int r = blockIdx.x;
  const uint32_t* __restrict__ src = pr.src[r];
  uint32_t* __restrict__ dst = pr.dst[r];
  for (uint32_t i = threadIdx.x; i < pr.words[r]; i += blockDim.x) dst[i] = src[i];
}
int d2h_small(pclean_ctx* ctx, void* host, const void* dev, size_t bytes, void* host_base) {
  SweepState* s = st(ctx);
  static const bool off = getenv("PCLEAN_NO_PUBLISH_REGIONS") != nullptr;
  if (bytes == 0) return PCLEAN_OK;
  void* mapped = nullptr;
  if (!off && (bytes & 3) == 0 && bytes <= (size_t)(1 << 20) && s->pub.n < 12) {
    void* base = host_base ? host_base : host;
    auto it = s->pub_map.find(base);
    if (it != s->pub_map.end()) {
      mapped = it->second;
    } else {
      if (hipHostGetDevicePointer(&mapped, base, 0) != hipSuccess) {
        (void)hipGetLastError();
        mapped = nullptr;
      }
      s->pub_map[base] = mapped;
    }
    if (mapped) mapped = static_cast<char*>(mapped) + (static_cast<char*>(host) - static_cast<char*>(base));
  }
  if (!mapped) {
    HIPCHK(ctx, hipMemcpyAsync(host, dev, bytes, hipMemcpyDeviceToHost, ctx->stream));
    return PCLEAN_OK;
  }
  const int k = s->pub.n++;
  s->pub.src[k] = static_cast<const uint32_t*>(dev);
  s->pub.dst[k] = static_cast<uint32_t*>(mapped);
  s->pub.words[k] = (uint32_t)(bytes >> 2);
  return PCLEAN_OK;
}
int d2h_flush(pclean_ctx* ctx) {
  SweepState* s = st(ctx);
  if (s->pub.n == 0) return PCLEAN_OK;
  hipLaunchKernelGGL(publish_regions_kernel, dim3(s->pub.n), dim3(256), 0, ctx->stream, s->pub);
  s->pub.n = 0;
  HIPCHK(ctx, hipGetLastError());
  return PCLEAN_OK;
}
int queue_over_copy(pclean_ctx* ctx) {
  SweepState* s = st(ctx);
  if (s->over_rec.empty() && !s->scan_stats_used) return PCLEAN_OK;
  if (!s->h_over) HIPCHK(ctx, hipHostMalloc((void**)&s->h_over, (OVER_SLOTS + STAT_WORDS) * sizeof(unsigned int), hipHostMallocDefault));
  int rc = PCLEAN_OK;
  if (!s->over_rec.empty()) rc = d2h_small(ctx, s->h_over, s->over_ctr.p, s->over_rec.size() * sizeof(unsigned int));
  if (!rc && s->scan_stats_used) rc = d2h_small(ctx, s->h_over + OVER_SLOTS, s->over_ctr.p + OVER_SLOTS, STAT_WORDS * sizeof(unsigned int), s->h_over);
  return rc;
}
void apply_over_stats(pclean_ctx* ctx) {
  SweepState* s = st(ctx);
  for (size_t i = 0; i < s->over_rec.size(); ++i) {
// ... 439 lines not shown
  *child_begin = dcb;
  *children = dch;
  return PCLEAN_OK;
}

static int ensure_it_ctx(pclean_ctx* ctx, BlockRun& r, size_t NP, int n_ctx) {
  if (r.it_ctx.alloc(NP * PCLEAN_MAX_CTX)) return pclean_fail(ctx, PCLEAN_ERR_HIP, "device alloc failed");
  if (r.it_ctx_np != NP || r.it_ctx_used != n_ctx) {
    HIPCHK(ctx, hipMemsetAsync(r.it_ctx.p, 0, NP * PCLEAN_MAX_CTX * sizeof(int32_t), ctx->stream));
    r.it_ctx_np = NP;
    r.it_ctx_used = n_ctx;
  }
  return PCLEAN_OK;
}

#define ZERO_LIST_MAX 16
struct ZeroList {
  int32_t n, pad;
  void* p[ZERO_LIST_MAX];
  uint32_t words[ZERO_LIST_MAX];
};
__global__ __launch_bounds__(256) void zero_list_kernel(ZeroList zl) {
  uint32_t* p = (uint32_t*)zl.p[blockIdx.y];
  const uint32_t nw = zl.words[blockIdx.y];
  for (uint32_t k = blockIdx.x * 256 + threadIdx.x; k < nw; k += gridDim.x * 256) p[k] = 0u;
}
static int zero_list_flush(pclean_ctx* ctx, ZeroList& zl) {
  if (zl.n == 0) return PCLEAN_OK;
  uint32_t mx = 0;
  for (int k = 0; k < zl.n; ++k) mx = std::max(mx, zl.words[k]);
  const unsigned gx = std::max(1u, std::min(1024u, (mx + 255u) / 256u));
  hipLaunchKernelGGL(zero_list_kernel, dim3(gx, zl.n), dim3(256), 0, ctx->stream, zl);
  zl.n = 0;
  HIPCHK(ctx, hipGetLastError());
  return PCLEAN_OK;
}
static void zero_list_add(pclean_ctx* ctx, ZeroList& zl, void* p, size_t bytes) {
  if (!p || bytes == 0) return;
  if (zl.n == ZERO_LIST_MAX || bytes > (size_t)0xffffffffu * 4) {
    (void)hipMemsetAsync(p, 0, bytes, ctx->stream);
    return;
  }
  zl.p[zl.n] = p;
  zl.words[zl.n] = (uint32_t)(bytes / 4);
  ++zl.n;
}

static bool env_on(const char* name) { return getenv(name) != nullptr; }
struct SweepSwitches {
  const bool no_prefetch = env_on("PCLEAN_NO_COMPACT_PREFETCH");
  const bool late_prefetch = env_on("PCLEAN_LATE_COMPACT_PREFETCH");
  const bool no_pu_stage = env_on("PCLEAN_NO_PU_STAGE");
  const bool no_w_uni = env_on("PCLEAN_NO_UNIFORM_W");
  const bool eager_all = env_on("PCLEAN_EAGER_NEW");
  const bool no_partial = env_on("PCLEAN_NO_PARTIAL_EAGER");
  const bool no_fuse_final = env_on("PCLEAN_NO_FUSED_FINAL");
  const bool no_fused_items = env_on("PCLEAN_NO_FUSED_CTX_ITEMS");
  const bool always_resample = env_on("PCLEAN_ALWAYS_RESAMPLE");
  const bool no_fused_finalize = env_on("PCLEAN_NO_FUSED_FINALIZE");
  const int forced_tail_wgs = getenv("PCLEAN_TAIL_WGS") ? std::max(1, atoi(getenv("PCLEAN_TAIL_WGS"))) : 0;
  const bool trace_tail = env_on("PCLEAN_TRACE_SYNC");
  const bool no_hist = env_on("PCLEAN_NO_HIST");
};
struct SweepCall {
  pclean_ctx* ctx;
  SweepState* s;
  const pclean_infer_config* cfg;
  const SweepSwitches& sw;
  int N, P, n_blocks;
  size_t NP;
  uint64_t seed;
  uint32_t sweep_idx;
  int use_mh;
  bool prior_mode;
  const int32_t* cur_base = nullptr;
  size_t cur_ld = 0;
  int pu_stage_stride = 0;
  size_t pu_stage_bytes = 0;
  bool w_by_first_block = false;
  const double* w_uni = nullptr;
  bool final_fused = false;
  const int32_t* final_only_rows = nullptr;
  bool hot_timed = false, prefetching = false, prefetch_started = false;
  const int32_t* cur_of(int bi) const { return cur_base + (size_t)bi * cur_ld; }
  ~SweepCall() {
    s->on_first_wait = nullptr;
    if (prefetching) (void)hipStreamWaitEvent(ctx->stream, s->pre_join, 0);
    ctx->prior_mode = false;
  }
};
static void materialise_w(SweepCall& c) {
  if (!c.w_uni) return;
  hipLaunchKernelGGL(materialise_w_kernel, grid1(c.N), dim3(256), 0, c.ctx->stream, c.N, c.P, c.w_uni, c.s->w.p);
  c.w_uni = nullptr;
}
static int start_prefetch(SweepCall& c) {
  c.prefetch_started = true;
  if (c.sw.no_prefetch || c.prior_mode || c.ctx->force_generic || c.n_blocks <= 1) return PCLEAN_OK;
  HIPCHK(c.ctx, hipStreamWaitEvent(c.s->pre_stream, c.s->pre_fork, 0));
  for (int bi = 1; bi < c.n_blocks; ++bi) {
    const Block& pb = c.ctx->block[bi];
    if (pb.is_score || pb.nodes.empty() || (!pb.node_gauss.empty() && pb.node_gauss[0] >= 0)) continue;
    if (const int rcp = prefetch_fast_root(c.ctx, bi, 0, c.s->pre_stream)) return rcp;
  }
  HIPCHK(c.ctx, hipEventRecord(c.s->pre_join, c.s->pre_stream));
  c.prefetching = true;
  return PCLEAN_OK;
}

static int sweep_begin(SweepCall& c, const int32_t* cur, bool dev_cur) {
  const int N = c.N, n_blocks = c.n_blocks;
  if (!c.s->ev0)
    for (hipEvent_t* e : {&c.s->ev0, &c.s->ev1, &c.s->evs, &c.s->eve, &c.s->evg0, &c.s->evg1}) HIPCHK(c.ctx, hipEventCreate(e));
  c.s->gate_timed = false;
  if (!c.s->h_counts) HIPCHK(c.ctx, hipHostMalloc((void**)&c.s->h_counts, 4 * PCLEAN_MAX_BLOCKS * sizeof(int32_t), hipHostMallocDefault));
  if (c.s->cur.alloc((size_t)N * n_blocks) || c.s->chosen.alloc(N) || c.s->ancestors.alloc(c.NP) || c.s->w.alloc(c.NP) || c.s->log_total.alloc(N) ||
      c.s->logml_inc.alloc(N) || c.s->logml_acc.alloc(N) || c.s->logml.alloc(N) || c.s->counter.alloc(4) || c.s->arr_ptrs.alloc(2 * PCLEAN_MAX_BLOCKS) ||
      c.s->did.alloc(N) || c.s->tail_counts.alloc(2 * PCLEAN_MAX_BLOCKS))
    return pclean_fail(c.ctx, PCLEAN_ERR_HIP, "device alloc failed");
  c.cur_base = dev_cur ? c.ctx->dev_cur.p + c.ctx->active_begin : c.s->cur.p;
  c.cur_ld = dev_cur ? (size_t)c.ctx->n_rows : (size_t)N;
  if (!dev_cur && c.ctx->cur_stride > 0 && c.ctx->cur_stride != N) {
    if (c.ctx->cur_stride < N) return pclean_fail(c.ctx, PCLEAN_ERR_ARG, "pclean_sweep: cur stride smaller than the active window");
    for (int b = 0; b < n_blocks; ++b)
      HIPCHK(c.ctx, hipMemcpyAsync(c.s->cur.p + (size_t)b * N, cur + (size_t)b * c.ctx->cur_stride, (size_t)N * 4, hipMemcpyHostToDevice,
                                   c.ctx->stream));
  } else if (!dev_cur) {
    HIPCHK(c.ctx, hipMemcpyAsync(c.s->cur.p, cur, (size_t)N * n_blocks * 4, hipMemcpyHostToDevice, c.ctx->stream));
  }
  c.s->last_cur_base = c.cur_base;
  c.s->last_cur_ld = c.cur_ld;
  c.s->last_N = N;
  c.s->last_blocks = n_blocks;
  c.s->last_dev_cur = dev_cur;
  (void)hipEventRecord(c.s->evs, c.ctx->stream);
  c.w_by_first_block = !c.ctx->block[0].is_score;
  if (!c.w_by_first_block) { const int rcz = dev_zero(c.ctx, c.s->w.p, c.NP * sizeof(double)); if (rcz) return rcz; }
  { const int rcz = dev_zero(c.ctx, c.s->logml_acc.p, (size_t)N * sizeof(double)); if (rcz) return rcz; }
  c.ctx->timing = pclean_timing{};
  if (!c.s->pre_stream) {
    HIPCHK(c.ctx, hipStreamCreateWithFlags(&c.s->pre_stream, hipStreamNonBlocking));
    HIPCHK(c.ctx, hipEventCreateWithFlags(&c.s->pre_fork, hipEventDisableTiming));
    HIPCHK(c.ctx, hipEventCreateWithFlags(&c.s->pre_join, hipEventDisableTiming));
  }
  HIPCHK(c.ctx, hipEventRecord(c.s->pre_fork, c.ctx->stream));
  if (!c.sw.late_prefetch) c.s->on_first_wait = [&c]() -> int { return c.prefetch_started ? PCLEAN_OK : start_prefetch(c); };
  constexpr size_t PU_STAGE_MAX_BYTES = 150 * 1024;
  c.pu_stage_stride = c.sw.no_pu_stage ? 0 : (c.P | 1);
  if ((size_t)c.pu_stage_stride * PU_T * sizeof(int32_t) > PU_STAGE_MAX_BYTES) c.pu_stage_stride = 0;
  c.pu_stage_bytes = (size_t)c.pu_stage_stride * PU_T * sizeof(int32_t);
  static bool attr_set = false;
  if (c.pu_stage_bytes > 48 * 1024 && !attr_set) {
    HIPCHK(c.ctx, hipFuncSetAttribute((const void*)particle_update_kernel, hipFuncAttributeMaxDynamicSharedMemorySize, (int)PU_STAGE_MAX_BYTES));
    attr_set = true;
  }
  return PCLEAN_OK;
}
static int run_score_block(SweepCall& c, int bi) {
  Block& b = c.ctx->block[bi];
  if (bi != c.n_blocks - 1) return pclean_fail(c.ctx, PCLEAN_ERR_ARG, "a scoring block must be the last block");
  ProfScope ps(c.ctx, "score_block");
  ScoreBlockDev sb{};
  auto make_src = [&](int blk, int col, SrcDev& out) -> int {
    if (blk < 0 || blk >= bi || c.ctx->block[blk].is_score) return pclean_fail(c.ctx, PCLEAN_ERR_ARG, "score block: bad source block");
    const CandTable& rt = c.ctx->cand[c.ctx->block[blk].nodes[0].table];
    if (col < 0 || col >= rt.n_cols) return pclean_fail(c.ctx, PCLEAN_ERR_ARG, "score block: bad source column");
    out = SrcDev{c.s->run[blk].pchoice.p, c.s->run[blk].pnewpos.p, c.s->run[blk].vals.p, rt.cols.p + (size_t)col * rt.n_rows,
                 (int)c.ctx->block[blk].nodes.size(), col, c.s->run[blk].plan};
    return 0;
  };
  const FnTable& pf = c.ctx->fn[b.prob_fn];
  if (!pf.valid || c.ctx->n_prob == 0) return pclean_fail(c.ctx, PCLEAN_ERR_STATE, "score block: prob fn / prob table not set");
  sb.n_terms = (int)b.score_terms.size();
  sb.prob_nb = pf.n_b;
  sb.prob_fn = pf.fn.p;
  sb.prob_same = c.ctx->prob_same.p;
  sb.prob_diff = c.ctx->prob_diff.p;
  sb.logn = c.ctx->logn.p;
  int rc2 = make_src(b.prob_a_block, b.prob_a_col, sb.pa);
  if (!rc2) rc2 = make_src(b.prob_b_block, b.prob_b_col, sb.pb);
  for (int k = 0; k < sb.n_terms && !rc2; ++k) {
    const ScoreTerm& st_ = b.score_terms[k];
    const PairTable& pt = c.ctx->pair[st_.pair_table];
    const FnTable& nf = c.ctx->fn[st_.nopt_fn];
    if (!pt.valid || !nf.valid || st_.obs_col < 0 || st_.obs_col >= c.ctx->n_cols)
      return pclean_fail(c.ctx, PCLEAN_ERR_ARG, "score block: term %d malformed", k);
    sb.t[k].obs_col = c.ctx->obs.p + (size_t)st_.obs_col * c.ctx->n_rows + c.ctx->active_begin;
    sb.t[k].pair = pt.d.p;
    sb.t[k].n_lat = pt.n_lat;
    sb.t[k].nopt_fn = nf.fn.p;
    sb.t[k].other_val = st_.other_val;
    rc2 = make_src(st_.val_block, st_.val_col, sb.t[k].val);
    if (!rc2) rc2 = make_src(st_.key_block, st_.key_col, sb.t[k].key);
  }
  if (rc2) return rc2;
  materialise_w(c);
  hipLaunchKernelGGL(score_block_kernel, grid1(c.NP), dim3(256), 0, c.ctx->stream, c.N, c.P, sb, c.s->w.p);
  return PCLEAN_OK;
}

struct BlockStep {
  bool drawable = false;
  const int32_t* emit_rows = nullptr;
  bool fuse_final = false, split_final = false;
  unsigned int* n_new_ctr = nullptr;
};
struct DrawSrc {
  const int32_t* draws_rm;
  const double* lse_rm;
  const int32_t* slot_item;
  const int32_t* draws_item;
  const double* lse_item;
};
static int build_ctx_src(SweepCall& c, int bi, CtxSrc& cs) {
  const Block& b = c.ctx->block[bi];
  cs = CtxSrc{};
  cs.n_ctx = b.n_ctx;
  for (int k = 0; k < b.n_ctx; ++k) {
    const int sb = b.ctx_src_block[k];
    if (sb < 0 || sb >= bi) return pclean_fail(c.ctx, PCLEAN_ERR_ARG, "block %d: ctx source must be an earlier block", bi);
    const Block& src = c.ctx->block[sb];
    const CandTable& rt = c.ctx->cand[src.nodes[0].table];
    if (b.ctx_src_col[k] < 0 || b.ctx_src_col[k] >= rt.n_cols) return pclean_fail(c.ctx, PCLEAN_ERR_ARG, "ctx column out of range");
    cs.pchoice[k] = c.s->run[sb].pchoice.p;
    cs.pnewpos[k] = c.s->run[sb].pnewpos.p;
    cs.vals[k] = c.s->run[sb].vals.p;
    cs.n_nodes[k] = (int)src.nodes.size();
    cs.root_col[k] = rt.cols.p + (size_t)b.ctx_src_col[k] * rt.n_rows;
    cs.col[k] = b.ctx_src_col[k];
    cs.plan[k] = c.s->run[sb].plan;
  }
  return PCLEAN_OK;
}
static int launch_particle_update(SweepCall& c, int bi, const DrawSrc& d, const int32_t* emit_rows, bool split, bool skip_w,
                                  unsigned int* n_new_ctr) {
  BlockRun& r = c.s->run[bi];
  const bool rm = d.draws_rm != nullptr;
  hipLaunchKernelGGL(particle_update_kernel, dim3((c.N + PU_T - 1) / PU_T), dim3(PU_T), rm ? c.pu_stage_bytes : 0, c.ctx->stream,
                     c.N, c.P, d.draws_rm, d.lse_rm, d.slot_item, d.draws_item, d.lse_item, c.cur_of(bi), r.pchoice.p, c.s->w.p,
                     n_new_ctr, r.new_slots.p, r.pnewpos.p, (c.w_by_first_block && bi == 0) ? 1 : 0, emit_rows, split ? 1 : 0,
                     rm ? c.pu_stage_stride : 0, c.w_uni, skip_w ? 1 : 0);
  HIPCHK(c.ctx, hipGetLastError());
  return PCLEAN_OK;
}
static void launch_update_final(SweepCall& c, int bi, const DrawSrc& d, const int32_t* only_rows, bool lazy_valid) {
  BlockRun& r = c.s->run[bi];
  DISPATCH_PMAX(c.P, hipLaunchKernelGGL(particle_update_final_kernel<PMAX>, grid1(c.N), dim3(256), 0, c.ctx->stream, c.N, c.P, d.draws_rm, d.lse_rm,
                                        d.slot_item, d.draws_item, d.lse_item, c.cur_of(bi), r.pchoice.p, c.s->w.p, (c.w_by_first_block &&
                                        bi == 0) ? 1 : 0, c.use_mh, c.cur_base, c.seed, c.sweep_idx, c.s->row_offset + c.ctx->active_begin,
                                        c.s->chosen.p, c.s->logml_acc.p, c.s->logml.p, only_rows, lazy_valid ? 1 : 0, c.w_uni));
}
static int lazy_draws(SweepCall& c, int bi, SweepState::LazyOut& lazy) {
  if (!lazy.valid) return PCLEAN_OK;
  ProfScope psl(c.ctx, "lazy_draws");
  lazy.args.n_rows = c.N;
  lazy.args.n_particles = c.P;
  lazy.args.chosen = c.s->chosen.p;
  lazy.args.cur_b = c.cur_of(bi);
  lazy.args.pchoice = c.s->run[bi].pchoice.p;
  return pclean_launch_lazy_draws(c.ctx, lazy.args, c.seed, c.sweep_idx, lazy.site);
}
static int eval_block_root(SweepCall& c, int bi, const BlockStep& bs, const ItemList& il, const int32_t* excl, double* lse, int32_t* draws) {
  if (bs.fuse_final || bs.split_final) c.s->lazy_req = SweepState::LazyReq{true, bs.split_final ? bs.emit_rows : nullptr};
  const int rc = eval_node(c.ctx, bi, 0, il, excl, c.seed, c.sweep_idx, c.P, lse, draws, nullptr, nullptr, bi == c.ctx->timed_block);
  c.s->lazy_req = SweepState::LazyReq();
  return rc;
}
static int update_after_eval(SweepCall& c, int bi, BlockStep& bs, const DrawSrc& d) {
  SweepState::LazyOut lazy = c.s->lazy_out;
  c.s->lazy_out.valid = false;
  lazy.args.slot_item = d.slot_item;
  if (bi == c.ctx->timed_block) {
    c.hot_timed = true;
    c.ctx->timing.hot_kernel_launches += 1;
  }
  ProfScope ps(c.ctx, "particle_update");
  if (bs.fuse_final) {
    launch_update_final(c, bi, d, nullptr, lazy.valid);
    c.final_fused = true;
    return lazy_draws(c, bi, lazy);
  }
  if (!(bs.n_new_ctr = fresh_counter(c.ctx))) return pclean_fail(c.ctx, PCLEAN_ERR_HIP, "counter bank: device alloc failed");
  const bool skip_w = bi == 0 && c.w_by_first_block && bi < c.n_blocks - 1 && !bs.split_final && !bs.emit_rows && !c.sw.no_w_uni;
  if (const int rc = launch_particle_update(c, bi, d, bs.emit_rows, bs.split_final, skip_w, bs.n_new_ctr)) return rc;
  if (skip_w || !bs.split_final) c.w_uni = skip_w ? c.s->run[bi].lse.p : nullptr;
  if (!bs.split_final) return PCLEAN_OK;
  launch_update_final(c, bi, d, bs.emit_rows, lazy.valid);
  c.final_only_rows = bs.emit_rows;
  return lazy_draws(c, bi, lazy);
}
static int propose_prior(SweepCall& c, int bi, BlockStep& bs) {
  Block& b = c.ctx->block[bi];
  BlockRun& r = c.s->run[bi];
  const ItemList il{c.N, nullptr, nullptr, nullptr, nullptr};
  c.ctx->prior_mode = true;
  const int rc = eval_node(c.ctx, bi, 0, il, c.cur_of(bi), c.seed, c.sweep_idx, c.P, nullptr, r.draws.p, nullptr, nullptr, false);
  if (rc) return rc;
  { const int rcz = dev_zero(c.ctx, r.lse.p, (size_t)c.N * sizeof(double)); if (rcz) return rcz; }
  if (!(bs.n_new_ctr = fresh_counter(c.ctx))) return pclean_fail(c.ctx, PCLEAN_ERR_HIP, "counter bank: device alloc failed");
  const int rcu = launch_particle_update(c, bi, DrawSrc{r.draws.p, r.lse.p, nullptr, nullptr, nullptr}, nullptr, false, false, bs.n_new_ctr);
  if (rcu) return rcu;
  if (b.n_ctx > 0) {
    { const int rci = ensure_it_ctx(c.ctx, r, c.NP, b.n_ctx); if (rci) return rci; }
    CtxSrc cs;
    if (const int rcs = build_ctx_src(c, bi, cs)) return rcs;
    hipLaunchKernelGGL(gather_ctx_kernel, grid1(c.NP), dim3(256), 0, c.ctx->stream, c.NP, cs, r.it_ctx.p);
  }
  return PCLEAN_OK;
}
static int propose_plain(SweepCall& c, int bi, BlockStep& bs) {
  BlockRun& r = c.s->run[bi];
  const ItemList il{c.N, nullptr, nullptr, nullptr, nullptr};
  if (const int rc = eval_block_root(c, bi, bs, il, c.cur_of(bi), r.lse.p, r.draws.p)) return rc;
  return update_after_eval(c, bi, bs, DrawSrc{r.draws.p, r.lse.p, nullptr, nullptr, nullptr});
}
struct CtxItems {
  unsigned int n = 0;
  int32_t *slot_item = nullptr, *row = nullptr, *ctx = nullptr, *excl = nullptr;
};
static int context_items(SweepCall& c, int bi, const CtxSrc& cs, CtxItems& it) {
  Block& b = c.ctx->block[bi];
  BlockRun& r = c.s->run[bi];
  const int N = c.N, P = c.P;
  const int32_t* cur_b = c.cur_of(bi);
  it.slot_item = scratch<int32_t>(c.ctx, c.NP);
  if (!it.slot_item) return pclean_fail(c.ctx, PCLEAN_ERR_HIP, "scratch alloc failed");
  if (!c.sw.no_fused_items) {
    ProfScope ps(c.ctx, "ctx_items");
    for (int attempt = 0;; ++attempt) {
      const int cap = std::max(r.ctx_extra_cap, 4096);
      it.row = scratch<int32_t>(c.ctx, (size_t)N + cap);
      it.ctx = scratch<int32_t>(c.ctx, ((size_t)N + cap) * PCLEAN_MAX_CTX);
      it.excl = scratch<int32_t>(c.ctx, (size_t)N + cap);
      unsigned int* extra_ctr = fresh_counter(c.ctx);
      if (!it.row || !it.ctx || !it.excl || !extra_ctr) return pclean_fail(c.ctx, PCLEAN_ERR_HIP, "scratch alloc failed");
      hipLaunchKernelGGL(ctx_items_kernel, grid1(N), dim3(256), 0, c.ctx->stream, N, P, cs, cur_b, r.it_ctx.p, it.slot_item, it.row,
                         it.ctx, it.excl, extra_ctr, cap);
      unsigned int n_extra = 0;
      PCLEAN_READ_COUNT(c.ctx, extra_ctr, &n_extra);
      r.ctx_extra_cap = (int)std::min<size_t>((size_t)n_extra * 2 + 4096, c.NP);
      if (n_extra <= (unsigned int)cap) {
        it.n = (unsigned int)N + n_extra;
        return PCLEAN_OK;
      }
      if (attempt >= 2) return pclean_fail(c.ctx, PCLEAN_ERR_STATE, "pclean_sweep: the context items did not fit twice in a row");
    }
  }
  int32_t* rep = scratch<int32_t>(c.ctx, c.NP);
  int32_t* n_distinct = scratch<int32_t>(c.ctx, (size_t)N + 1);
  int32_t* off = scratch<int32_t>(c.ctx, (size_t)N + 1);
  size_t tmp_scan = 0;
  HIPCHK(c.ctx, hipcub::DeviceScan::ExclusiveSum(nullptr, tmp_scan, n_distinct, off, N + 1, c.ctx->stream));
  unsigned char* tmp = scratch<unsigned char>(c.ctx, tmp_scan);
  if (!rep || !n_distinct || !off || !tmp) return pclean_fail(c.ctx, PCLEAN_ERR_HIP, "scratch alloc failed");
  {
    ProfScope ps(c.ctx, "ctx_items");
    hipLaunchKernelGGL(gather_ctx_kernel, grid1(c.NP), dim3(256), 0, c.ctx->stream, c.NP, cs, r.it_ctx.p);
    HIPCHK(c.ctx, hipMemsetAsync(n_distinct + N, 0, sizeof(int32_t), c.ctx->stream));
    hipLaunchKernelGGL(ctx_count_kernel, grid1(N), dim3(256), 0, c.ctx->stream, N, P, (int)b.n_ctx, r.it_ctx.p, rep, n_distinct);
    HIPCHK(c.ctx, hipcub::DeviceScan::ExclusiveSum(tmp, tmp_scan, n_distinct, off, N + 1, c.ctx->stream));
    PCLEAN_READ_COUNT(c.ctx, off + N, &it.n);
  }
  it.row = scratch<int32_t>(c.ctx, it.n);
  it.ctx = scratch<int32_t>(c.ctx, (size_t)it.n * PCLEAN_MAX_CTX);
  it.excl = scratch<int32_t>(c.ctx, it.n);
  if (!it.row || !it.ctx || !it.excl) return pclean_fail(c.ctx, PCLEAN_ERR_HIP, "scratch alloc failed");
  hipLaunchKernelGGL(ctx_fill_kernel, grid1(N), dim3(256), 0, c.ctx->stream, N, P, (int)b.n_ctx, r.it_ctx.p, rep, off, cur_b,
                     it.slot_item, it.row, it.ctx, it.excl);
  return PCLEAN_OK;
}
static int propose_ctx(SweepCall& c, int bi, BlockStep& bs) {
  Block& b = c.ctx->block[bi];
  { const int rci = ensure_it_ctx(c.ctx, c.s->run[bi], c.NP, b.n_ctx); if (rci) return rci; }
  CtxSrc cs;
  if (const int rc = build_ctx_src(c, bi, cs)) return rc;
  CtxItems it;
  if (const int rc = context_items(c, bi, cs, it)) return rc;
  double* lse_item = scratch<double>(c.ctx, it.n);
  int32_t* draws_item = scratch<int32_t>(c.ctx, (size_t)it.n * c.P);
  if (!lse_item || !draws_item) return pclean_fail(c.ctx, PCLEAN_ERR_HIP, "scratch alloc failed");
  ItemList il{(int)it.n, it.row, it.ctx, nullptr, nullptr};
  if (!c.sw.no_fused_items) il.n_primary = c.N;
  if (const int rc = eval_block_root(c, bi, bs, il, it.excl, lse_item, draws_item)) return rc;
  return update_after_eval(c, bi, bs, DrawSrc{nullptr, nullptr, it.slot_item, draws_item, lse_item});
}
static int propose_block(SweepCall& c, int bi, BlockStep& bs) {
  Block& b = c.ctx->block[bi];
  BlockRun& r = c.s->run[bi];
  const int N = c.N;
  if (c.prefetching && bi >= 1) {
    HIPCHK(c.ctx, hipStreamWaitEvent(c.ctx->stream, c.s->pre_join, 0));
    c.prefetching = false;
  }
  if (r.pchoice.alloc(c.NP) || r.pnewpos.alloc(c.NP) || r.new_slots.alloc(c.NP) || r.choice.alloc(N) || r.chosen_newpos.alloc(N) ||
      r.moved_flag.alloc(N) || r.new_flag.alloc(N) || r.moved_list.alloc(N) || r.new_list.alloc(N) ||
      ((c.prior_mode || b.n_ctx == 0) && (r.draws.alloc(c.NP) || r.lse.alloc(N))))
    return pclean_fail(c.ctx, PCLEAN_ERR_HIP, "device alloc failed");
  if (const int rc = ensure_plan_dev(c.ctx, bi)) return rc;
  const bool last = bi == c.n_blocks - 1;
  bool dummy_by_row = false;
  bs.drawable = c.prior_mode;
  if (!c.prior_mode)
    if (const int rc = block_dummy_drawable(c.ctx, bi, &bs.drawable, &dummy_by_row)) return rc;
  if (last && !c.sw.eager_all && !c.sw.no_partial && !c.prior_mode && bs.drawable && dummy_by_row) {
    bool none = false;
    if (const int rc = dummy_rows_flags(c.ctx, bi, N, &bs.emit_rows, &none)) return rc;
    if (none) bs.drawable = false;
  }
  const bool last_plain = last && !c.prior_mode && !c.sw.eager_all && !c.sw.no_fuse_final;
  bs.fuse_final = last_plain && !bs.drawable;
  bs.split_final = last_plain && bs.drawable && bs.emit_rows != nullptr;
  r.plocals_on = false;
  if (const int rc = c.prior_mode ? propose_prior(c, bi, bs) : b.n_ctx > 0 ? propose_ctx(c, bi, bs) : propose_plain(c, bi, bs)) return rc;
  return c.prefetch_started ? PCLEAN_OK : start_prefetch(c);
}
static int sample_new_rows(SweepCall& c, int bi, unsigned int count) {
  Block& b = c.ctx->block[bi];
  BlockRun& r = c.s->run[bi];
  const int nn = (int)b.nodes.size();
  hipLaunchKernelGGL(fill_i32_kernel, grid1((size_t)count * nn), dim3(256), 0, c.ctx->stream, r.vals.p, (size_t)count * nn, -2);
  int32_t* row = scratch<int32_t>(c.ctx, count);
  int32_t* cx = scratch<int32_t>(c.ctx, (size_t)count * PCLEAN_MAX_CTX);
  int32_t* part = scratch<int32_t>(c.ctx, count);
  int32_t* org = scratch<int32_t>(c.ctx, count);
  int32_t* ex = scratch<int32_t>(c.ctx, count);
  if (!row || !cx || !part || !org || !ex) return pclean_fail(c.ctx, PCLEAN_ERR_HIP, "scratch alloc failed");
  hipLaunchKernelGGL(rootlist_items_kernel, grid1(count), dim3(256), 0, c.ctx->stream, (int)count, c.N, c.NP, r.new_slots.p,
                     b.n_ctx > 0 ? r.it_ctx.p : nullptr, c.cur_of(bi), row, cx, part, org, ex);
  hipLaunchKernelGGL(set_col_kernel, grid1(count), dim3(256), 0, c.ctx->stream, (int)count, nn, 0, (int32_t)PCLEAN_CHOICE_NEW, r.vals.p);
  ItemList sub{(int)count, row, cx, part, org};
  return sample_children(c.ctx, bi, 0, sub, ex, c.seed, c.sweep_idx, r.vals.p, nn);
}
static int slot_gauss_dev(SweepCall& c, int bi, GaussDev& gd, const GaussDev** more, int* n_more) {
  const Block& b = c.ctx->block[bi];
  const CandTable& rt = c.ctx->cand[b.nodes[0].table];
  const int rc = build_gauss_dev(c.ctx, b.gauss[b.node_gauss[0]], &rt, gd);
  return rc ? rc : build_gauss_more(c.ctx, b, 0, &rt, more, n_more);
}
static int prior_terms_and_gauss(SweepCall& c, int bi) {
  Block& b = c.ctx->block[bi];
  BlockRun& r = c.s->run[bi];
  const int nn = (int)b.nodes.size();
  c.ctx->prior_mode = false;
  const NodeDev* nds;
  const int32_t *dnc, *dcb, *dch;
  int rc = upload_plan_nodes(c.ctx, bi, &nds, &dnc, &dcb, &dch);
  if (!rc)
    rc = pclean_launch_prior_terms(c.ctx, c.NP, c.N, nn, nds, dnc, dcb, dch, r.pchoice.p, r.pnewpos.p, r.vals.p,
                                   b.n_ctx > 0 ? r.it_ctx.p : nullptr, c.s->w.p);
  if (rc || b.node_gauss.empty() || b.node_gauss[0] < 0) return rc;
  GaussDev gd;
  const GaussDev* gmore;
  int n_gmore;
  if (const int rc = slot_gauss_dev(c, bi, gd, &gmore, &n_gmore)) return rc;
  if (r.plocals.alloc((size_t)c.NP * 2)) return pclean_fail(c.ctx, PCLEAN_ERR_HIP, "device alloc failed");
  const int32_t* cl = (b.cur_locals.p && b.cur_locals_rows == c.ctx->n_rows) ? b.cur_locals.p + (size_t)c.ctx->active_begin * 2 : nullptr;
  hipLaunchKernelGGL(gauss_prior_kernel, grid1(c.NP), dim3(256), 0, c.ctx->stream, c.N, c.P, gd, gmore, n_gmore, r.plan, r.pchoice.p, r.pnewpos.p,
                     r.vals.p, nn, c.cur_of(bi), cl, c.seed, c.sweep_idx, (uint32_t)bi, c.s->row_offset + c.ctx->active_begin, c.s->w.p, r.plocals.p);
  r.plocals_on = true;
  return PCLEAN_OK;
}

static int new_rows_of_block(SweepCall& c, int bi, const BlockStep& bs, bool* weights_touched) {
  BlockRun& r = c.s->run[bi];
  const int nn = (int)c.ctx->block[bi].nodes.size();
  unsigned int n_new = 0;
  if (!c.final_fused) PCLEAN_READ_COUNT(c.ctx, bs.n_new_ctr, &n_new);
  const bool degenerate_rows = (n_new & 0x80000000u) != 0u;
  n_new &= 0x7fffffffu;
  r.n_new = c.final_fused ? -1 : (int)n_new;
  r.lazy_new = c.final_fused || (bi == c.n_blocks - 1 && !c.sw.eager_all && (!bs.drawable || bs.emit_rows != nullptr));
  if (r.lazy_new && !bs.emit_rows) n_new = 0;
  if (bs.emit_rows) r.n_new = -1;
  if (r.vals.alloc(std::max<size_t>((size_t)n_new * nn, 1))) return pclean_fail(c.ctx, PCLEAN_ERR_HIP, "device alloc failed");
  *weights_touched = (bs.drawable && n_new > 0) || degenerate_rows;
  std::optional<ProfScope> ps;
  int rc = PCLEAN_OK;
  if (n_new) {
    ps.emplace(c.ctx, "new_row_sampling");
    if (const int rc = sample_new_rows(c, bi, n_new)) return rc;
  }
  if (c.prior_mode)
    if (const int rc = prior_terms_and_gauss(c, bi)) return rc;
  if (n_new && bs.drawable) {
    if (!bs.split_final) materialise_w(c);
    rc = apply_dummy_corrections(c.ctx, bi, r.new_slots.p, r.vals.p, (int)n_new, c.N, c.seed, c.sweep_idx, c.s->w.p);
  }
  c.ctx->prior_mode = false;
  return rc;
}
static int resample_between_blocks(SweepCall& c, int bi, bool weights_touched) {
  const Block& b = c.ctx->block[bi];
  const int N = c.N, P = c.P;
  const int grp_here = b.group >= 0 ? b.group : bi;
  const int grp_next = bi + 1 < c.n_blocks ? (c.ctx->block[bi + 1].group >= 0 ? c.ctx->block[bi + 1].group : bi + 1) : -2;
  const bool equal_weights = bi == 0 && c.w_by_first_block && b.n_ctx == 0 && !c.prior_mode && !weights_touched;
  if (c.use_mh || bi >= c.n_blocks - 1 || grp_here == grp_next || (equal_weights && !c.sw.always_resample)) return PCLEAN_OK;
  ProfScope ps(c.ctx, "resample");
  materialise_w(c);
  DISPATCH_PMAX(P, hipLaunchKernelGGL(maybe_resample_kernel<PMAX>, grid1(N), dim3(256), 0, c.ctx->stream, N, P, c.s->w.p, (size_t)1, (size_t)N, 1,
                                      c.cur_of(bi), c.seed, c.sweep_idx, (uint32_t)bi, c.s->row_offset + c.ctx->active_begin, c.s->ancestors.p,
                                      c.s->logml_inc.p, (double*)nullptr, c.s->did.p));
  AncestorArrays arrs{};
  int n_arr = 0;
  for (int k = 0; k <= bi; ++k) {
    if (c.ctx->block[k].is_score) continue;
    arrs.p[n_arr++] = c.s->run[k].pchoice.p;
    arrs.p[n_arr++] = c.s->run[k].pnewpos.p;
    if (c.s->run[k].plocals_on) arrs.pairs[arrs.n_pairs++] = reinterpret_cast<int64_t*>(c.s->run[k].plocals.p);
  }
  hipLaunchKernelGGL(apply_ancestors_kernel, grid1(N), dim3(256), 0, c.ctx->stream, N, P, c.s->ancestors.p, n_arr, arrs, c.s->w.p,
                     c.s->did.p, c.s->logml_inc.p, c.s->logml_acc.p);
  return PCLEAN_OK;
}
static void final_choice(SweepCall& c) {
  if (c.final_fused) return;
  if (!c.final_only_rows) materialise_w(c);
  DISPATCH_PMAX(c.P, hipLaunchKernelGGL(final_choice_kernel<PMAX>, grid1(c.N), dim3(256), 0, c.ctx->stream, c.N, c.P, c.s->w.p, (size_t)1,
                                        (size_t)c.N, c.use_mh, 1, c.cur_base, c.seed, c.sweep_idx, c.s->row_offset + c.ctx->active_begin, c.s->chosen.p,
                                        (double*)nullptr, c.s->logml_acc.p, c.s->logml.p, c.final_only_rows));
}

struct SweepTail {
  int nb_wg = 0;
  unsigned int* wg_cnt = nullptr;
  unsigned int* chosen_ctr[PCLEAN_MAX_BLOCKS] = {};
  int hist_rows[PCLEAN_MAX_BLOCKS] = {};
  TailLists tl{};
  ZeroList zl{};
};
static int sample_chosen(SweepCall& c, const SweepTail& t, int bi) {
  BlockRun& r = c.s->run[bi];
  ProfScope ps2(c.ctx, "new_row_sampling_chosen");
  const int nn = (int)c.ctx->block[bi].nodes.size();
  unsigned int cnt = 0;
  PCLEAN_READ_COUNT(c.ctx, t.chosen_ctr[bi], &cnt);
  if (c.sw.trace_tail)
    fprintf(stderr, "[pclean tail] block %d: %u chosen NEW rows listed by %s\n", bi, cnt,
            c.sw.no_fused_finalize ? "chosen_new_kernel" : "finalize_tail_kernel");
  if (r.vals.alloc(std::max<size_t>((size_t)cnt * nn, 1))) return pclean_fail(c.ctx, PCLEAN_ERR_HIP, "device alloc failed");
  return cnt ? sample_new_rows(c, bi, cnt) : PCLEAN_OK;
}
static int tail_begin(SweepCall& c, SweepTail& t) {
  t.wg_cnt = scratch<unsigned int>(c.ctx, (size_t)2 * c.n_blocks * t.nb_wg);
  return t.wg_cnt ? zero_list_flush(c.ctx, t.zl) : pclean_fail(c.ctx, PCLEAN_ERR_HIP, "scratch alloc failed");
}
static int tail_lists(SweepCall& c, const SweepTail& t) {
  for (int bi = 0; bi < c.n_blocks; ++bi)
    if (c.ctx->block[bi].is_score)
      HIPCHK(c.ctx, hipMemsetAsync(t.wg_cnt + (size_t)(2 * bi) * t.nb_wg, 0, (size_t)2 * t.nb_wg * sizeof(unsigned int), c.ctx->stream));
  hipLaunchKernelGGL(tail_scan_kernel, dim3(2 * c.n_blocks), dim3(1024), 0, c.ctx->stream, t.nb_wg, t.wg_cnt, c.s->tail_counts.p);
  hipLaunchKernelGGL(tail_scatter_kernel, dim3(t.nb_wg, 2 * c.n_blocks), dim3(256), 0, c.ctx->stream, c.N, t.nb_wg, t.tl, t.wg_cnt);
  return PCLEAN_OK;
}
static int tail_fused(SweepCall& c, SweepTail& t) {
  if (const int rc = tail_begin(c, t)) return rc;
  TailBlocks tb{};
  int max_hist = 0;
  for (int bi = 0; bi < c.n_blocks; ++bi) {
    if (c.ctx->block[bi].is_score) continue;
    BlockRun& r = c.s->run[bi];
    tb.b[bi] = TailBlock{r.pchoice.p, r.pnewpos.p, c.cur_of(bi), r.choice.p, r.chosen_newpos.p,
                         (unsigned long long*)c.ctx->cand[c.ctx->block[bi].nodes[0].table].stats.p, r.moved_flag.p, r.new_flag.p,
                         t.wg_cnt + (size_t)(2 * bi) * t.nb_wg, t.wg_cnt + (size_t)(2 * bi + 1) * t.nb_wg, t.chosen_ctr[bi], r.new_slots.p,
                         t.hist_rows[bi],  1,  t.chosen_ctr[bi] ? 1 : 0, 0};
    max_hist = std::max(max_hist, t.hist_rows[bi]);
  }
  static int tail_cap = 0;
  if (!tail_cap) {
    int n_cu = 256;
    hipDeviceProp_t prop;
    if (hipGetDeviceProperties(&prop, c.ctx->device) == hipSuccess && prop.multiProcessorCount > 0) n_cu = prop.multiProcessorCount;
    tail_cap = std::max(1, n_cu / TAIL_CUS_PER_WG);
  }
  const int n_wgs = tail_wg_count(t.nb_wg, tail_cap, c.sw.forced_tail_wgs);
  if (c.sw.trace_tail)
    fprintf(stderr, "[pclean tail] finalize_tail_kernel: %d tiles, %d workgroups per block, at most %d tiles per workgroup\n",
            t.nb_wg, n_wgs, (t.nb_wg + n_wgs - 1) / n_wgs);
  hipLaunchKernelGGL(finalize_tail_kernel, dim3(n_wgs, c.n_blocks), dim3(TAIL_WG_THREADS), (size_t)max_hist * sizeof(int32_t), c.ctx->stream,
                     c.N, t.nb_wg, c.s->chosen.p, tb);
  int rc = tail_lists(c, t);
  for (int bi = 0; bi < c.n_blocks && !rc; ++bi)
    if (t.chosen_ctr[bi]) rc = sample_chosen(c, t, bi);
  return rc;
}
static int tail_per_block(SweepCall& c, SweepTail& t) {
  for (int bi = 0; bi < c.n_blocks; ++bi) {
    if (!t.chosen_ctr[bi]) continue;
    BlockRun& r = c.s->run[bi];
    hipLaunchKernelGGL(chosen_new_kernel, grid1(c.N), dim3(256), 0, c.ctx->stream, c.N, c.s->chosen.p, r.pchoice.p, t.chosen_ctr[bi],
                       r.new_slots.p, r.pnewpos.p);
    if (const int rc = sample_chosen(c, t, bi)) return rc;
  }
  if (const int rc = tail_begin(c, t)) return rc;
  for (int bi = 0; bi < c.n_blocks; ++bi) {
    if (c.ctx->block[bi].is_score) continue;
    BlockRun& r = c.s->run[bi];
    hipLaunchKernelGGL(finalize_block_kernel, grid1(c.N), dim3(256), (size_t)t.hist_rows[bi] * sizeof(int32_t), c.ctx->stream, c.N,
                       c.s->chosen.p, r.pchoice.p, r.pnewpos.p, c.cur_of(bi), r.choice.p, r.chosen_newpos.p,
                       (unsigned long long*)c.ctx->cand[c.ctx->block[bi].nodes[0].table].stats.p, t.hist_rows[bi], r.moved_flag.p,
                       r.new_flag.p, t.wg_cnt + (size_t)(2 * bi) * t.nb_wg, t.wg_cnt + (size_t)(2 * bi + 1) * t.nb_wg);
  }
  if (c.sw.trace_tail) fprintf(stderr, "[pclean tail] finalize_block_kernel: one launch per block\n");
  return tail_lists(c, t);
}
static int sweep_tail(SweepCall& c) {
  SweepTail t;
  t.nb_wg = (c.N + TAIL_TILE_ROWS - 1) / TAIL_TILE_ROWS;
  for (int bi = 0; bi < c.n_blocks; ++bi) {
    BlockRun& r = c.s->run[bi];
    Block& bb = c.ctx->block[bi];
    bb.locals_host.clear();
    r.locals_rows = 0;
    if (bb.is_score) continue;
    if (r.lazy_new && r.n_new != 0) {
      if (!(t.chosen_ctr[bi] = fresh_counter(c.ctx))) return pclean_fail(c.ctx, PCLEAN_ERR_HIP, "counter bank: device alloc failed");
    }
    const CandTable& rt = c.ctx->cand[bb.nodes[0].table];
    const int rows_in_use = (rt.n_used > 0 && rt.n_used <= rt.n_rows) ? std::min(rt.n_rows, (rt.n_used + 63) & ~63) : rt.n_rows;
    t.hist_rows[bi] = (rt.n_rows <= 12288 && !c.sw.no_hist) ? rows_in_use : 0;
    bool seen = false;
    for (int k = 0; k < t.zl.n; ++k) seen |= t.zl.p[k] == (void*)rt.stats.p;
    if (!seen) zero_list_add(c.ctx, t.zl, rt.stats.p, (size_t)std::max(rt.n_rows, 1) * 8);
    t.tl.flag[2 * bi] = r.moved_flag.p;
    t.tl.list[2 * bi] = r.moved_list.p;
    t.tl.flag[2 * bi + 1] = r.new_flag.p;
    t.tl.list[2 * bi + 1] = r.new_list.p;
  }
  return c.sw.no_fused_finalize ? tail_per_block(c, t) : tail_fused(c, t);
}
static int block_outputs(SweepCall& c, int32_t* choice, int32_t* chosen_particle, double* logml) {
  const int N = c.N;
  for (int bi = 0; bi < c.n_blocks; ++bi) {
    BlockRun& r = c.s->run[bi];
    Block& bb = c.ctx->block[bi];
    if (bb.is_score) continue;
    if (choice) HIPCHK(c.ctx, hipMemcpyAsync(choice + (size_t)bi * N, r.choice.p, (size_t)N * 4, hipMemcpyDeviceToHost, c.ctx->stream));
    if (bb.node_gauss.empty() || bb.node_gauss[0] < 0 || bb.gauss[bb.node_gauss[0]].n_locals <= 0) continue;
    if (r.locals.alloc((size_t)N * 2)) return pclean_fail(c.ctx, PCLEAN_ERR_HIP, "device alloc failed");
    if (r.plocals_on) {
      hipLaunchKernelGGL(locals_pick_kernel, grid1(N), dim3(256), 0, c.ctx->stream, N, c.s->chosen.p, r.plocals.p, r.locals.p);
    } else {
      GaussDev gd;
      const GaussDev* gmore;
      int n_gmore;
      if (const int rc = slot_gauss_dev(c, bi, gd, &gmore, &n_gmore)) return rc;
      hipLaunchKernelGGL(locals_tail_kernel, grid1(N), dim3(256), 0, c.ctx->stream, N, c.P, gd, gmore, n_gmore, r.plan, c.s->chosen.p,
                         r.pchoice.p, r.pnewpos.p, r.vals.p, (int)bb.nodes.size(), c.seed, c.sweep_idx, (uint32_t)bi,
                         c.s->row_offset + c.ctx->active_begin, r.locals.p);
    }
    r.locals_rows = N;
    if (!c.ctx->defer_outputs) {
      bb.locals_host.resize((size_t)N * 2);
      HIPCHK(c.ctx, hipMemcpyAsync(bb.locals_host.data(), r.locals.p, (size_t)N * 8, hipMemcpyDeviceToHost, c.ctx->stream));
    }
  }
  (void)hipEventRecord(c.s->eve, c.ctx->stream);
  if (chosen_particle) HIPCHK(c.ctx, hipMemcpyAsync(chosen_particle, c.s->chosen.p, (size_t)N * 4, hipMemcpyDeviceToHost, c.ctx->stream));
  if (logml) HIPCHK(c.ctx, hipMemcpyAsync(logml, c.s->logml.p, (size_t)N * 8, hipMemcpyDeviceToHost, c.ctx->stream));
  return PCLEAN_OK;
}
static int sweep_end(SweepCall& c, int32_t* choice) {
  c.s->last_hot_timed = c.hot_timed;
  c.s->outputs_pending = true;
  c.s->lists_on_host = false;
  const int tb = c.ctx->timed_block;
  const Block& b0 = c.ctx->block[(tb >= 0 && tb < c.n_blocks && !c.ctx->block[tb].is_score) ? tb : 0];
  const double F = b0.nodes[0].n_terms, K = c.ctx->cand[b0.nodes[0].table].n_rows;
  c.ctx->timing.hot_kernel_alg_bytes = (double)c.N * (4.0 * F + (K + 1.0) * (8.0 * F + 4.0) + 8.0 * c.P);
  if (c.ctx->defer_outputs) return PCLEAN_OK;
  if (const int rcf = pclean_sweep_finish_queue(c.ctx)) return rcf;
  PCLEAN_SYNC(c.ctx);
  if (const int rcf = pclean_sweep_finish_synced(c.ctx)) return rcf;
  if (choice)
    for (int bi = 0; bi < c.n_blocks; ++bi)
      if (c.ctx->block[bi].is_score)
        for (int i = 0; i < c.N; ++i) choice[(size_t)bi * c.N + i] = 0;
  return pclean_sweep_fetch_lists(c.ctx);
}

extern "C" int pclean_sweep(pclean_ctx* ctx, const pclean_infer_config* cfg, uint64_t seed, uint32_t sweep_idx, int32_t n_blocks,
                            const int32_t* cur, int32_t* choice, int32_t* chosen_particle, double* logml) {
  if (!ctx || !cfg || n_blocks <= 0 || n_blocks > PCLEAN_MAX_BLOCKS) return pclean_fail(ctx, PCLEAN_ERR_ARG, "pclean_sweep: bad arguments");
  const bool dev_cur = cur == nullptr;
  if (dev_cur && (!ctx->dev_cur_valid || ctx->dev_cur_blocks != n_blocks || !ctx->dev_cur.p))
    return pclean_fail(ctx, PCLEAN_ERR_STATE, "pclean_sweep: cur == NULL needs pclean_set_cur (device-resident referents)");
  if (ctx->defer_outputs && (choice || chosen_particle || logml))
    return pclean_fail(ctx, PCLEAN_ERR_ARG, "pclean_sweep: deferred outputs (pclean_set_sweep_mode) take no per-row output buffers");
  const bool prior_mode = !cfg->use_dd_proposals;
  for (int b = 0; b < n_blocks && prior_mode; ++b)
    if (const int rcp = prior_mode_supported(ctx, ctx->block[b], "pclean_sweep")) return rcp;
  const int N = ctx->active_count >= 0 ? ctx->active_count : ctx->n_rows;
  const int use_mh = cfg->use_mh_instead_of_pg != 0;
  const int P = use_mh ? 2 : cfg->num_particles;
  if (N <= 0) return pclean_fail(ctx, PCLEAN_ERR_STATE, "pclean_sweep: no observed rows loaded");
  if (P < 1 || P > MAXP) return pclean_fail(ctx, PCLEAN_ERR_ARG, "pclean_sweep: num_particles must be in 1..%d", MAXP);
  for (int b = 0; b < n_blocks; ++b)
    if (!ctx->block[b].valid) return pclean_fail(ctx, PCLEAN_ERR_STATE, "pclean_sweep: block %d not loaded", b);
  HIPCHK(ctx, hipSetDevice(ctx->device));
  if (const int rc = begin_call(ctx)) return rc;
  static const SweepSwitches sw;
  SweepCall call{ctx, st(ctx), cfg, sw, N, P, n_blocks, (size_t)N * P, seed, sweep_idx, use_mh, prior_mode};
  if (const int rc = sweep_begin(call, cur, dev_cur)) return rc;
  for (int bi = 0; bi < n_blocks; ++bi) {
    if (ctx->block[bi].is_score) {
      if (const int rc = run_score_block(call, bi)) return rc;
      continue;
    }
    BlockStep bs;
    bool weights_touched = false;
    if (const int rc = propose_block(call, bi, bs)) return rc;
    if (const int rc = new_rows_of_block(call, bi, bs, &weights_touched)) return rc;
    if (const int rc = resample_between_blocks(call, bi, weights_touched)) return rc;
  }
  if (call.prefetching) HIPCHK(ctx, hipStreamWaitEvent(ctx->stream, call.s->pre_join, 0));
  {
    ProfScope ps(ctx, "final_choice_and_outputs");
    final_choice(call);
    if (const int rc = sweep_tail(call)) return rc;
    if (const int rc = block_outputs(call, choice, chosen_particle, logml)) return rc;
  }
  return sweep_end(call, choice);
}

int pclean_sweep_finish_queue(pclean_ctx* ctx) {
  SweepState* s = st(ctx);
  if (!s->outputs_pending) return PCLEAN_OK;
  int rc = d2h_small(ctx, s->h_counts, s->tail_counts.p, 2 * s->last_blocks * sizeof(int32_t));
  if (rc) return rc;
  const int rco = queue_over_copy(ctx);
  if (rco) return rco;
  s->h_counts[3 * PCLEAN_MAX_BLOCKS] = 0;
  if (s->dummy_used) rc = d2h_small(ctx, s->h_counts + 3 * PCLEAN_MAX_BLOCKS, s->dummy_ctr.p + 1, sizeof(int32_t), s->h_counts);
  if (rc) return rc;
  return d2h_flush(ctx);
}
int pclean_sweep_finish_synced(pclean_ctx* ctx) {
  SweepState* s = st(ctx);
  if (!s->outputs_pending) return PCLEAN_OK;
  s->outputs_pending = false;
  apply_over_stats(ctx);
  if (s->prof_on) prof_collect(ctx);
  float tot = 0;
  HIPCHK(ctx, hipEventElapsedTime(&tot, s->evs, s->eve));
  ctx->timing.total_ms = tot;
  ctx->timing.hot_kernel_ms = 0.f;
  if (s->last_hot_timed) {
    float ms = 0;
    HIPCHK(ctx, hipEventElapsedTime(&ms, s->ev0, s->ev1));
    ctx->timing.hot_kernel_ms = ms;
    if (s->gate_timed) {
      float mg = 0;
      HIPCHK(ctx, hipEventElapsedTime(&mg, s->evg0, s->evg1));
      ctx->timing.hot_kernel_ms += mg;
    }
  }
  if (s->h_counts[3 * PCLEAN_MAX_BLOCKS])
    return pclean_fail(ctx, PCLEAN_ERR_CAPACITY, "pclean_sweep: an observed string longer than %d symbols below a chosen "
                                                 "dummy value", DUMMY_MAX_LEN);
  return PCLEAN_OK;
}
int pclean_sweep_fetch_lists(pclean_ctx* ctx) {
  SweepState* s = st(ctx);
  if (s->lists_on_host) return PCLEAN_OK;
  for (int bi = 0; bi < s->last_blocks; ++bi) {
    BlockRun& r = s->run[bi];
    Block& b = ctx->block[bi];
    const int nn = (int)b.nodes.size();
    b.new_rows_host.clear();
    b.new_vals_host.clear();
    b.moved_rows_host.clear();
    b.moved_choice_host.clear();
    if (b.is_score) continue;
    const int n_moved = s->h_counts[2 * bi], n_newrows = s->h_counts[2 * bi + 1];
    if (n_moved > 0) {
      int32_t* ch_d = scratch<int32_t>(ctx, n_moved);
      if (!ch_d) return pclean_fail(ctx, PCLEAN_ERR_HIP, "scratch alloc failed");
      hipLaunchKernelGGL(gather_moved_kernel, grid1(n_moved), dim3(256), 0, ctx->stream, n_moved, r.moved_list.p,
                         r.choice.p, ch_d);
      b.moved_rows_host.resize(n_moved);
      b.moved_choice_host.resize(n_moved);
      HIPCHK(ctx, hipMemcpyAsync(b.moved_rows_host.data(), r.moved_list.p, (size_t)n_moved * 4, hipMemcpyDeviceToHost, ctx->stream));
      HIPCHK(ctx, hipMemcpyAsync(b.moved_choice_host.data(), ch_d, (size_t)n_moved * 4, hipMemcpyDeviceToHost, ctx->stream));
    }
    if (n_newrows > 0) {
// ... 240 lines not shown
```

### pclean_amd/csrc/sweep_internal.h

```cpp
#pragma once
#include <algorithm>
#include <cmath>
#include <map>
#include <set>

#include <hipcub/hipcub.hpp>
#include <rocprim/rocprim.hpp>

#include "../../include/pclean_detmath.h"
#include "../../include/pclean_philox.h"
#include "dummy_dev.h"
#include "enum.h"
#include "gauss_dev.h"
#include "sweep_state.h"

extern int g_pclean_sync_count;
int read_count(pclean_ctx* ctx, const void* dev, void* out, const char* func, int line);
#define PCLEAN_READ_COUNT(ctx, dev, out)                                  \
  do {                                                                    \
    const int rc_ = read_count(ctx, (dev), (out), __func__, __LINE__);    \
    if (rc_) return rc_;                                                  \
  } while (0)

#define PCLEAN_SYNC(ctx)                                                                                   \
  do {                                                                                                     \
    static const bool trace_ = getenv("PCLEAN_TRACE_SYNC") != nullptr;                                     \
    if (trace_) fprintf(stderr, "[pclean sync %d] %s:%d\n", ++g_pclean_sync_count, __func__, __LINE__);          \
    HIPCHK(ctx, hipStreamSynchronize(ctx->stream));                                                        \
  } while (0)

static inline dim3 grid1(size_t n, int bs = 256) { return dim3((unsigned)((n + bs - 1) / bs)); }

struct ItemList {
  int n = 0;
  const int32_t* row = nullptr;
  const int32_t* ctx = nullptr;
  const int32_t* particle = nullptr;
  const int32_t* origin = nullptr;
  const int32_t* ev_lo = nullptr;
  const int32_t* ev_hi = nullptr;
  const int32_t* ev_rows = nullptr;
  const int32_t* ev_ctx = nullptr;
  const int32_t* rng_row = nullptr;
  int draw_is = 0, draw_ds = 0;
  int n_primary = 0;
};
struct ItemGroups {
  int n_groups = 0;
  const int32_t* grp_off = nullptr;
  const int32_t* members = nullptr;
  const int32_t* head = nullptr;
  const int32_t* uid = nullptr;
  const uint64_t* hg_incl = nullptr;
  const int32_t* hg_rep = nullptr;
  const int32_t* hg_slot_of = nullptr;
};

template <typename T>
static T* scratch(pclean_ctx* ctx, size_t count) {
  SweepState* s = st(ctx);
  if (s->pool_used == s->pool.size()) s->pool.emplace_back();
  DevBuf<unsigned char>& b = s->pool[s->pool_used++];
  const size_t need = std::max<size_t>(count * sizeof(T), 16);
  if (need > b.n && b.alloc(std::max(need, b.n + b.n / 2))) {
    if (b.alloc(need)) return nullptr;
  }
  return (T*)b.p;
}

static unsigned int* fresh_counter(pclean_ctx* ctx) {
  SweepState* s = st(ctx);
  if (!s->over_ctr.p) return nullptr;
  unsigned int* bank = s->over_ctr.p + OVER_SLOTS + STAT_WORDS;
  static const int first = [] {
    const char* e = getenv("PCLEAN_CTR_BANK");
    return e ? std::max(1, std::min(atoi(e), CTR_BANK)) : CTR_BANK;
  }();
  if (s->bank_used < first) return bank + s->bank_used++;
  const int idx = s->bank_used - first, b = idx / CTR_BANK, o = idx % CTR_BANK;
  while ((int)s->more_banks.size() <= b) s->more_banks.emplace_back();
  if (s->more_banks[b].alloc(CTR_BANK)) return nullptr;
  if (o == 0 && hipMemsetAsync(s->more_banks[b].p, 0, CTR_BANK * sizeof(unsigned int), ctx->stream) != hipSuccess) return nullptr;
  ++s->bank_used;
  return s->more_banks[b].p + o;
}

int prof_phase_id(SweepState* s, const char* name);
struct ProfScope {
  pclean_ctx* ctx;
  SweepState* s;
  size_t rec = (size_t)-1;
  ProfScope(pclean_ctx* c, const char* name) : ctx(c), s(st(c)) {
    if (!s->prof_on) return;
    rec = s->prof_used++;
    while (s->prof_ev.size() < 2 * (rec + 1)) {
      hipEvent_t e;
      if (hipEventCreate(&e) != hipSuccess) {
        rec = (size_t)-1;
        --s->prof_used;
        return;
      }
      s->prof_ev.push_back(e);
    }
    if (s->prof_phase.size() <= rec) s->prof_phase.resize(rec + 1);
    s->prof_phase[rec] = prof_phase_id(s, name);
// ... 4 lines not shown
  }
};

#define MAXP 64

template <int PMAX>
struct FixW {
  double m;
  uint64_t U;
  uint64_t u[PMAX];
};
template <int PMAX>
__device__ __forceinline__ void fix_weights(const double* w, size_t sp, int P, FixW<PMAX>& f) {
  f.m = -__builtin_inf();
  f.U = 0;
#pragma unroll
  for (int p = 0; p < PMAX; ++p)
    if (p < P) f.m = fmax(f.m, w[(size_t)p * sp]);
#pragma unroll
  for (int p = 0; p < PMAX; ++p) {
    f.u[p] = (p < P && f.m != -__builtin_inf()) ? pclean_fixw(w[(size_t)p * sp] - f.m) : 0ull;
    f.U += f.u[p];
  }
}
template <int PMAX>
__device__ __forceinline__ int fix_pick(const FixW<PMAX>& f, int P, uint64_t R) {
  if (f.U == 0) return P - 1;
  const uint64_t x = pclean_mulhi64(R, f.U);
  uint64_t acc = 0;
  int res = P - 1;
  bool found = false;
#pragma unroll
  for (int p = 0; p < PMAX; ++p) {
    acc += f.u[p];
    if (!found && p < P && acc > x) {
      res = p;
      found = true;
    }
  }
  return res;
}

#define DISPATCH_PMAX(P, ...)   \
  do {                          \
    if ((P) <= 2) {             \
      constexpr int PMAX = 2;   \
      __VA_ARGS__;              \
    } else if ((P) <= 8) {      \
      constexpr int PMAX = 8;   \
      __VA_ARGS__;              \
    } else if ((P) <= 32) {     \
      constexpr int PMAX = 32;  \
      __VA_ARGS__;              \
    } else {                    \
      constexpr int PMAX = 64;  \
      __VA_ARGS__;              \
    }                           \
  } while (0)

static __global__ void iota_missing_kernel(int32_t* p, int n_obs) {
  int i = blockIdx.x * blockDim.x + threadIdx.x;
  if (i <= n_obs) p[i] = i < n_obs ? i : -1;
}

static __global__ void fill_i32_kernel(int32_t* p, size_t n, int32_t v) {
  size_t i = (size_t)blockIdx.x * blockDim.x + threadIdx.x;
  if (i < n) p[i] = v;
}

static __global__ void fill_f64_kernel(double* p, size_t n, double v) {
  size_t i = (size_t)blockIdx.x * blockDim.x + threadIdx.x;
  if (i < n) p[i] = v;
}

static __global__ void derive_excl_kernel(int n, const int32_t* parent_excl, const int64_t* parent_counts,
                                   const int32_t* parent_fk_col, int32_t* out) {
  int t = blockIdx.x * blockDim.x + threadIdx.x;
  if (t >= n) return;
  const int e = parent_excl ? parent_excl[t] : -1;
  out[t] = (e >= 0 && parent_counts[e] <= 1) ? parent_fk_col[e] : -1;
}

static __global__ __launch_bounds__(256) void compact_new_kernel(size_t n, const int32_t* choice, int fill,
                                                          unsigned int* counter, int32_t* list, int32_t* pos_out) {
  __shared__ unsigned int wcnt[4];
  __shared__ unsigned int bbase;
  const size_t t = (size_t)blockIdx.x * blockDim.x + threadIdx.x;
  const int lane = threadIdx.x & 63, wave = threadIdx.x >> 6;
  const bool hit = t < n && choice[t] == PCLEAN_CHOICE_NEW;
  const unsigned long long mask = __ballot(hit);
  if (lane == 0) wcnt[wave] = (unsigned int)__popcll(mask);
  __syncthreads();
  if (threadIdx.x == 0) {
    const unsigned int total = wcnt[0] + wcnt[1] + wcnt[2] + wcnt[3];
    bbase = total ? atomicAdd(counter, total) : 0u;
  }
  __syncthreads();
  if (t >= n || !fill) return;
  if (!hit) {
    if (pos_out) pos_out[t] = -1;
    return;
  }
  unsigned int pos = bbase + (unsigned int)__popcll(mask & ((1ull << lane) - 1ull));
  for (int w = 0; w < wave; ++w) pos += wcnt[w];
  list[pos] = (int32_t)t;
  if (pos_out) pos_out[t] = (int32_t)pos;
}

static __global__ void sublist_items_kernel(int n, const int32_t* list, const int32_t* p_row, const int32_t* p_ctx,
                                     const int32_t* p_particle, const int32_t* p_origin, int32_t* row, int32_t* ctxv,
                                     int32_t* particle, int32_t* origin, const int32_t* p_ev_lo,
                                     const int32_t* p_ev_hi, const int32_t* p_rng, int32_t* ev_lo, int32_t* ev_hi,
                                     int32_t* rng) {
  int j = blockIdx.x * blockDim.x + threadIdx.x;
  if (j >= n) return;
  const int s = list[j];
  if (p_ev_lo) {
    ev_lo[j] = p_ev_lo[s];
    ev_hi[j] = p_ev_hi[s];
  }
  if (p_rng) rng[j] = p_rng[s];
  row[j] = p_row ? p_row[s] : s;
  particle[j] = p_particle[s];
  origin[j] = p_origin ? p_origin[s] : j;
  for (int c = 0; c < PCLEAN_MAX_CTX; ++c) ctxv[j * PCLEAN_MAX_CTX + c] = p_ctx ? p_ctx[s * PCLEAN_MAX_CTX + c] : 0;
}

static __global__ void scatter_vals_kernel(int n, const int32_t* origin, const int32_t* draws, int n_nodes, int node,
                                    int32_t* vals) {
  int j = blockIdx.x * blockDim.x + threadIdx.x;
  if (j < n) vals[(size_t)origin[j] * n_nodes + node] = draws[j];
}

static __global__ void gather_i32_kernel(int n, const int32_t* list, const int32_t* src, int32_t* dst) {
  int j = blockIdx.x * blockDim.x + threadIdx.x;
  if (j < n) dst[j] = src[list[j]];
}

int begin_call(pclean_ctx* ctx);
int queue_over_copy(pclean_ctx* ctx);
void apply_over_stats(pclean_ctx* ctx);
int finish_call(pclean_ctx* ctx);
void prof_collect(pclean_ctx* ctx);
int prior_mode_supported(pclean_ctx* ctx, const Block& b, const char* who);
int upload_plan_nodes(pclean_ctx* ctx, int bi, const NodeDev** nds, const int32_t** n_children,
                             const int32_t** child_begin, const int32_t** children);
int build_gauss_dev(pclean_ctx* ctx, const pclean_gauss& g, const CandTable* t, GaussDev& d);
int build_gauss_more(pclean_ctx* ctx, const Block& b, int node_id, const CandTable* t, const GaussDev** more, int* n_more);
int build_node_dev(pclean_ctx* ctx, const Block& b, int node_id, NodeDev& nd);
int ensure_leaf_cache(pclean_ctx* ctx, int block_id, int node_id, const double** out, const int32_t** obs_col,
                             int* n_obs);
int eval_node(pclean_ctx* ctx, int block_id, int node_id, const ItemList& il, const int32_t* excl,
                     uint64_t seed, uint32_t sweep, int n_draws, double* lse_out, int32_t* draws_out,
                     double* scores_out, const double* snew_override, bool time_it);
int sample_children(pclean_ctx* ctx, int block_id, int node_id, const ItemList& il, const int32_t* excl,
                           uint64_t seed, uint32_t sweep, int32_t* vals, int n_nodes);
int ensure_plan_dev(pclean_ctx* ctx, int block_id);
int prefetch_fast_root(pclean_ctx* ctx, int block_id, int node_id, hipStream_t side);
int ensure_agg(pclean_ctx* ctx, int block_id, int node_id, const ItemList& il, const AggDev** out);
```

### pclean_amd/csrc/sweep_state.h

```cpp
#pragma once
#include <functional>
#include <map>
#include <string>
#include <deque>
#include <vector>

#include "ctx.h"
#include "enum.h"

struct PlanDev {
  int32_t n_nodes;
  const int32_t* kind;
  const int32_t* const* cols;
  const int32_t* n_rows;
  const int32_t* colmap_begin;
  const int32_t* colmap;
};


struct BlockRun {
  DevBuf<int32_t> pchoice, pnewpos, draws, it_ctx, choice, chosen_newpos, vals, locals, moved_flag, new_flag, moved_list,
      new_list, new_slots;
  DevBuf<double> lse;
  int n_new = 0;
  int locals_rows = 0;
  DevBuf<int32_t> plocals;
  bool plocals_on = false;
  size_t it_ctx_np = 0;
  int it_ctx_used = -1;
  bool lazy_new = false;
  int ctx_extra_cap = 0;
  DevBuf<int32_t> plan_kind, plan_nrows, plan_cmb, plan_colmap;
  DevBuf<const int32_t*> plan_cols;
  PlanDev plan{};
  bool plan_ready = false;
  std::vector<int32_t> plan_sig_nrows, plan_sig_kind, plan_sig_cmb;
  std::vector<const int32_t*> plan_sig_cols;
  size_t plan_sig_colmap = 0;
  uint64_t plan_sig_block = 0;
};

struct FastRoot {
  std::vector<DevBuf<uint8_t>> comp, clen, cblk;
  std::vector<uint64_t> ver;
  DevBuf<double> prior_e, prior_n;
  DevBuf<uint16_t> alive;
  DevBuf<uint8_t> zero_row;
  int disabled = 0;
  int backoff = 64;
  uint64_t cmin_key = 0;
  double cmin = 0.0;
  uint64_t prior_ver = 0;
  int kpad = 0;
  double logc_max = 0.0;
  int wl_off = 0;
  DevBuf<int32_t> obs_rm;
  uint64_t obs_rm_key = 0;
};

struct SweepState {
  FastRoot fast[PCLEAN_MAX_BLOCKS * 64];
  std::vector<DevBuf<unsigned char>> pool;
  size_t pool_used = 0;
  BlockRun run[PCLEAN_MAX_BLOCKS];
  DevBuf<int32_t> cur, chosen, ancestors, csmc_flag, did;
  const int32_t* last_cur_base = nullptr;
  size_t last_cur_ld = 0;
  int last_N = 0, last_blocks = 0;
  bool last_dev_cur = false, last_hot_timed = false;
  volatile unsigned int* h_poll = nullptr;
  unsigned int* d_poll = nullptr;
  unsigned int poll_seq = 0;
  bool outputs_pending = false;
  bool lists_on_host = false;
  DevBuf<double> w, log_total, logml_inc, logml_acc, logml;
  DevBuf<unsigned int> counter;
  DevBuf<int32_t*> arr_ptrs;
  std::map<int, DevBuf<int32_t>> leaf_iota;
  std::map<int, uint64_t> leaf_version;
  int64_t row_offset = 0;
  hipEvent_t ev0 = nullptr, ev1 = nullptr, evs = nullptr, eve = nullptr;
  hipEvent_t evg0 = nullptr, evg1 = nullptr;
  hipStream_t pre_stream = nullptr;
  std::function<int()> on_first_wait;
  hipEvent_t pre_fork = nullptr, pre_join = nullptr;
  bool gate_timed = false;
  struct LeafMemo {
    DevBuf<uint64_t> keys;
    DevBuf<double> vals;
    DevBuf<unsigned int> count;
    uint64_t ver = 0;
    int cap = 0;
  };
  std::map<int, LeafMemo> memo;
  struct TupleIds {
    DevBuf<int32_t> id;
    DevBuf<uint32_t> pre;
    uint64_t sig = 0;
    struct StaticOrder {
      int begin = 0, n = 0, n_tiles = 0, n_wave = 0, n_long = 0, n_chunks = 0;
      DevBuf<int32_t> order, tid, tile_off;
      DevBuf<int32_t> wave_tiles, long_tiles, chunk_tile, chunk_off;
      void release() {
        order.release(); tid.release(); tile_off.release();
        wave_tiles.release(); long_tiles.release(); chunk_tile.release(); chunk_off.release();
      }
    };
    std::vector<StaticOrder> windows;
    void release() {
      id.release();
      pre.release();
      for (auto& w : windows) w.release();
      windows.clear();
    }
  };
  std::map<int, TupleIds> tuple_ids;
  struct GateStat { int all_need_run = 0, skip = 0; };
  std::map<int, GateStat> gate_stat;
  struct DummyRows { DevBuf<int32_t> flag; uint64_t sig = 0; int n = 0, n_flagged = 0; };
  std::map<int, DummyRows> dummy_rows;
  const int32_t* lat_off = nullptr;
  const int32_t* lat_item_of_pos = nullptr;
  int lat_items = 0, lat_ev = 0, lat_max_ev = 0;
  std::map<int, const AggDev*> lat_agg;
  DevBuf<int32_t> tail_counts;
  int32_t* h_counts = nullptr;
  bool prof_on = false;
  std::vector<hipEvent_t> prof_ev;
  std::vector<int> prof_phase;
  size_t prof_used = 0;
  std::vector<std::string> prof_names;
  std::vector<float> prof_ms;
  std::vector<int32_t> prof_launches;
  bool scan_stats_used = false;
  int bank_used = 0;
  DevBuf<unsigned int> over_ctr;
  std::deque<DevBuf<unsigned int>> more_banks;
  struct PubRegions { const uint32_t* src[12]; uint32_t* dst[12]; uint32_t words[12]; int n; } pub = {};
  std::map<void*, void*> pub_map;
  struct OverRec { int block, node, n_items; bool time_it, leaf; int min_items; };
  std::vector<OverRec> over_rec;
  static const int MAX_SIDE = 8;
  hipStream_t side[MAX_SIDE] = {};
  hipEvent_t side_fork = nullptr, side_join[MAX_SIDE] = {}, side_mid[MAX_SIDE] = {};
  int n_side = -1;
  unsigned int* h_over = nullptr;
  DevBuf<int16_t> dummy_dp;
  DevBuf<unsigned int> dummy_ctr;
  bool dummy_used = false;
  struct LazyReq { bool on = false; const int32_t* eager_rows = nullptr; } lazy_req;
  struct LazyOut { bool valid = false; LazyDrawArgs args{}; uint32_t site = 0; } lazy_out;
  const int32_t* dbg_desc = nullptr;
  const int32_t* dbg_grp_off = nullptr;
  const int32_t* dbg_members = nullptr;
  const int32_t* dbg_oflag = nullptr;
  int dbg_groups = 0, dbg_items = 0;
};

#define OVER_SLOTS 256
#define STAT_WORDS (64 * 32)
#define CTR_BANK 2048
static SweepState* st(pclean_ctx* ctx) {
  if (!ctx->sweep_state) ctx->sweep_state = new SweepState();
  return (SweepState*)ctx->sweep_state;
}


int pclean_sweep_finish_queue(pclean_ctx* ctx);
int d2h_small(pclean_ctx* ctx, void* host, const void* dev, size_t bytes, void* host_base = nullptr);
int d2h_flush(pclean_ctx* ctx);
int dev_zero(pclean_ctx* ctx, void* p, size_t bytes);
int pclean_sweep_finish_synced(pclean_ctx* ctx);
int pclean_sweep_fetch_lists(pclean_ctx* ctx);
```

Baseline: 460.4 million.

## Fold count publication into compaction kernels and merge small prep kernels

Count read-backs no longer launch a separate single-thread publish kernel. The last workgroup of the compaction kernel (found through hierarchical ticket atomics) writes the count to mapped host memory, and a ring of poll slots lets several counts be in flight at once. Separate launches are also merged: group-rep items, exclusion derivation and -inf fills become one open_prep kernel, leaf coarse draws write straight into the vals array instead of going through a scatter, and root-list items plus set-col become one kernel. The aim is fewer kernel launches and less host-device sync latency on the per-sweep critical path, at the cost of added atomic and ticket-reset complexity and a bounded number of outstanding reads.

```diff
diff --git a/pclean_amd/csrc/eval.hip b/pclean_amd/csrc/eval.hip
--- a/pclean_amd/csrc/eval.hip
+++ b/pclean_amd/csrc/eval.hip
@@ -769,6 +769,40 @@
   excl[j] = p_excl ? p_excl[s] : -1;
   for (int c = 0; c < PCLEAN_MAX_CTX; ++c) ctxv[j * PCLEAN_MAX_CTX + c] = p_ctx ? p_ctx[(size_t)s * PCLEAN_MAX_CTX + c] : 0;
 }
+struct OpenPrep {
+  int32_t n_rep, n_items, n_derive, n_fills;
+  size_t n_fill;
+  const int32_t *list, *grp_off, *members, *p_row, *p_ctx, *p_excl;
+  int32_t *row, *ctxv, *excl;
+  const int32_t* sexcl;
+  const int64_t* counts;
+  const int32_t* fk_col[PCLEAN_MAX_CHILDREN];
+  int32_t* ce[PCLEAN_MAX_CHILDREN];
+  double* fill[PCLEAN_MAX_CHILDREN];
+};
+__global__ void open_prep_kernel(OpenPrep pp) {
+  const size_t t = (size_t)blockIdx.x * blockDim.x + threadIdx.x;
+  if (t < (size_t)pp.n_items) {
+    const int j = (int)t;
+    int e;
+    if (pp.n_rep > 0) {
+      const int g = pp.list ? pp.list[j] : j;
+      const int s = pp.members[pp.grp_off[g]];
+      pp.row[j] = pp.p_row ? pp.p_row[s] : s;
+      e = pp.p_excl ? pp.p_excl[s] : -1;
+      pp.excl[j] = e;
+      for (int c = 0; c < PCLEAN_MAX_CTX; ++c) pp.ctxv[j * PCLEAN_MAX_CTX + c] = pp.p_ctx ? pp.p_ctx[(size_t)s * PCLEAN_MAX_CTX + c] : 0;
+    } else {
+      e = pp.sexcl ? pp.sexcl[j] : -1;
+    }
+    if (pp.n_derive > 0) {
+      const bool gone = e >= 0 && pp.counts[e] <= 1;
+      for (int d = 0; d < pp.n_derive; ++d) pp.ce[d][j] = gone ? pp.fk_col[d][e] : -1;
+    }
+  }
+  if (t < pp.n_fill)
+    for (int f = 0; f < pp.n_fills; ++f) pp.fill[f][t] = -__builtin_inf();
+}
 __global__ void group_scatter_f64_kernel(int n, const int32_t* list, const int32_t* grp_off, const int32_t* members,
                                          const double* src, double* dst) {
   const int j = blockIdx.x * blockDim.x + threadIdx.x;
@@ -803,6 +837,7 @@
   const uint32_t site;
   const EvalSwitches sw;
   SweepState::LazyReq lazy_req;
+  SweepState::ValsReq vals_req;
   bool lazy_ok = false;
   int fast_split_m = 0;
   bool tabulated = false;
@@ -828,6 +863,9 @@
   c.lazy_req = s->lazy_req;
   s->lazy_req = SweepState::LazyReq();
   s->lazy_out.valid = false;
+  c.vals_req = s->vals_req;
+  s->vals_req = SweepState::ValsReq();
+  s->vals_done = false;
   c.lazy_ok = c.lazy_req.on && !c.sw.cached.no_lazy && c.n_draws > 1 && !il.rng_row && !il.ev_lo;
   const bool lazy_sure = c.lazy_ok && (size_t)il.n * ROOT_LZ_CAP * 12 <= ((size_t)4 << 30);
   c.fast_split_m = (lazy_sure && !c.sw.cached.lazy_split) ? 0 : std::max(4, 256 / std::max(c.n_draws, 1));
@@ -876,6 +914,8 @@
   int32_t* list = nullptr;
   ItemList sil;
   const int32_t* sexcl = nullptr;
+  int32_t* rep_ctx = nullptr;
+  bool rep_pending = false;
   bool sub() const { return n_need < (unsigned int)n_all; }
 };
 
@@ -931,8 +971,13 @@
   }
   unsigned int* need_ctr = fresh_counter(ctx);
   if (!need_ctr) return pclean_fail(ctx, PCLEAN_ERR_HIP, "counter bank: device alloc failed");
-  hipLaunchKernelGGL(compact_new_kernel, grid1(n), dim3(256), 0, ctx->stream, (size_t)n, flag, 1, need_ctr, u.list, nullptr);
-  PCLEAN_READ_COUNT(ctx, need_ctr, &u.n_need);
+  const CountPub need_pub = count_pub(ctx);
+  hipLaunchKernelGGL(compact_new_kernel, grid1(n), dim3(256), 0, ctx->stream, (size_t)n, flag, 1, need_ctr, u.list, nullptr, need_pub);
+  PCLEAN_READ_COUNT_PUB(ctx, need_pub, need_ctr, &u.n_need);
+  static const bool trace_gate = getenv("PCLEAN_TRACE_SYNC") != nullptr;
+  if (trace_gate)
+    fprintf(stderr, "[pclean gate] block %d node %d: %u of %d %s need the open children\n", c.block_id, c.node_id, u.n_need, n,
+            u.grouped ? "groups" : "items");
   if (u.grouped) {
     c.pre_score = sc;
     c.pre_obs = ow;
@@ -960,8 +1005,11 @@
   int32_t* excl2 = scratch<int32_t>(c.ctx, u.n_need);
   if (u.grouped) {
     if (!row2 || !ctx2 || !excl2) return pclean_fail(c.ctx, PCLEAN_ERR_HIP, "scratch alloc failed");
-    hipLaunchKernelGGL(group_rep_items_kernel, grid1(u.n_need), dim3(256), 0, c.ctx->stream, (int)u.n_need, u.list, c.g_pre.grp_off,
-                       c.g_pre.members, il.row, il.ctx, c.excl, row2, ctx2, excl2);
+    u.rep_pending = pclean_fold_on();
+    u.rep_ctx = ctx2;
+    if (!u.rep_pending)
+      hipLaunchKernelGGL(group_rep_items_kernel, grid1(u.n_need), dim3(256), 0, c.ctx->stream, (int)u.n_need, u.list, c.g_pre.grp_off,
+                         c.g_pre.members, il.row, il.ctx, c.excl, row2, ctx2, excl2);
     u.sil = ItemList{(int)u.n_need, row2, il.ctx ? ctx2 : nullptr, nullptr, nullptr};
   } else {
     const int rc = sub_items(c, u.n_need, u.list, row2, ctx2, excl2, u.sil);
@@ -976,28 +1024,58 @@
   const ItemList& il = c.il;
   const ItemList& sil = u.sil;
   const CandTable& t = ctx->cand[c.n.table];
+  const bool fold = pclean_fold_on();
+  double* lse_of[PCLEAN_MAX_CHILDREN] = {};
+  int32_t* ce_of[PCLEAN_MAX_CHILDREN] = {};
+  const bool evaluate = !(u.sub() && u.n_need == 0);
+  OpenPrep pp{};
   for (int k = 0; k < c.n.n_children; ++k) {
     const int cid = c.b.children[c.n.child_begin + k];
     const pclean_node& cn = c.b.nodes[cid];
     if (cn.kind == PCLEAN_NODE_LEAF && cn.cacheable) continue;
-    double* child_lse = scratch<double>(ctx, il.n);
-    if (!child_lse) return pclean_fail(ctx, PCLEAN_ERR_HIP, "scratch alloc failed");
-    c.ch.arr[k] = child_lse;
+    if (!(lse_of[k] = scratch<double>(ctx, il.n))) return pclean_fail(ctx, PCLEAN_ERR_HIP, "scratch alloc failed");
+    c.ch.arr[k] = lse_of[k];
     c.ch.obs_col[k] = nullptr;
-    if (u.sub()) {
-      hipLaunchKernelGGL(fill_f64_kernel, grid1(il.n), dim3(256), 0, ctx->stream, child_lse, (size_t)il.n, -__builtin_inf());
-      if (u.n_need == 0) continue;
-    }
-    const int32_t* child_excl = nullptr;
-    if (cn.kind == PCLEAN_NODE_FK && u.sexcl) {
+    if (u.sub()) pp.fill[pp.n_fills++] = lse_of[k];
+    if (evaluate && cn.kind == PCLEAN_NODE_FK && u.sexcl) {
       if (cn.parent_fk_col < 0 || cn.parent_fk_col >= t.n_cols)
         return pclean_fail(ctx, PCLEAN_ERR_ARG, "node %d: parent_fk_col out of range", cid);
-      int32_t* ce = scratch<int32_t>(ctx, sil.n);
-      if (!ce) return pclean_fail(ctx, PCLEAN_ERR_HIP, "scratch alloc failed");
+      if (!(ce_of[k] = scratch<int32_t>(ctx, sil.n))) return pclean_fail(ctx, PCLEAN_ERR_HIP, "scratch alloc failed");
+      pp.fk_col[pp.n_derive] = t.cols.p + (size_t)cn.parent_fk_col * t.n_rows;
+      pp.ce[pp.n_derive++] = ce_of[k];
+    }
+  }
+  if (fold && (u.rep_pending || pp.n_derive || pp.n_fills)) {
+    pp.n_fill = pp.n_fills ? (size_t)il.n : 0;
+    pp.n_items = (u.rep_pending || pp.n_derive) ? sil.n : 0;
+    pp.sexcl = u.sexcl;
+    pp.counts = t.counts.p;
+    if (u.rep_pending) {
+      pp.n_rep = sil.n;
+      pp.list = u.list;
+      pp.grp_off = c.g_pre.grp_off;
+      pp.members = c.g_pre.members;
+      pp.p_row = il.row;
+      pp.p_ctx = il.ctx;
+      pp.p_excl = c.excl;
+      pp.row = const_cast<int32_t*>(sil.row);
+      pp.ctxv = const_cast<int32_t*>(u.rep_ctx);
+      pp.excl = const_cast<int32_t*>(u.sexcl);
+    }
+    hipLaunchKernelGGL(open_prep_kernel, grid1(std::max(pp.n_fill, (size_t)pp.n_items)), dim3(256), 0, ctx->stream, pp);
+  }
+  for (int k = 0; k < c.n.n_children; ++k) {
+    const int cid = c.b.children[c.n.child_begin + k];
+    const pclean_node& cn = c.b.nodes[cid];
+    if (cn.kind == PCLEAN_NODE_LEAF && cn.cacheable) continue;
+    double* child_lse = lse_of[k];
+    if (u.sub() && !fold)
+      hipLaunchKernelGGL(fill_f64_kernel, grid1(il.n), dim3(256), 0, ctx->stream, child_lse, (size_t)il.n, -__builtin_inf());
+    if (!evaluate) continue;
+    const int32_t* child_excl = ce_of[k];
+    if (child_excl && !fold)
       hipLaunchKernelGGL(derive_excl_kernel, grid1(sil.n), dim3(256), 0, ctx->stream, sil.n, u.sexcl, t.counts.p,
-                         t.cols.p + (size_t)cn.parent_fk_col * t.n_rows, ce);
-      child_excl = ce;
-    }
+                         t.cols.p + (size_t)cn.parent_fk_col * t.n_rows, ce_of[k]);
     double* dst = child_lse;
     if (u.grouped || u.sub()) {
       dst = scratch<double>(ctx, sil.n);
@@ -1082,9 +1160,18 @@
   const int rc = ensure_leaf_cache(ctx, c.block_id, c.node_id, &cache, &ocol, &n_obs);
   if (rc) return rc;
   ProfScope ps(ctx, "option_list_coarse_draw");
-  return pclean_launch_leaf_coarse_draw(ctx, c.nd, c.it, ocol, n_obs, pclean_leaf_coarse_blocks(c.nd.n_cand), cache,
+  ItemsDev it = c.it;
+  int32_t* draws_out = c.draws_out;
+  if (c.vals_req.dst && c.n_draws == 1 && !c.lse_out && !it.out_pos) {
+    it.out_pos = c.vals_req.origin;
+    it.draw_is = c.vals_req.stride;
+    it.draw_ds = 1;
+    draws_out = c.vals_req.dst;
+    c.s->vals_done = true;
+  }
+  return pclean_launch_leaf_coarse_draw(ctx, c.nd, it, ocol, n_obs, pclean_leaf_coarse_blocks(c.nd.n_cand), cache,
                                         c.b.leaf_m[c.node_id].p, c.b.leaf_U[c.node_id].p, c.b.leaf_coarse[c.node_id].p, c.seed,
-                                        c.sweep, PCLEAN_SITE_NODE(c.block_id, c.node_id), c.n_draws, c.lse_out, c.draws_out);
+                                        c.sweep, PCLEAN_SITE_NODE(c.block_id, c.node_id), c.n_draws, c.lse_out, draws_out);
 }
 
 static int choose_compact_path(EvalCall& c) {
@@ -2301,9 +2388,10 @@
   hipLaunchKernelGGL(memo_lookup_kernel, grid1(N), dim3(256), 0, ctx->stream, N, kc, il.row, il.ctx, md, lse_out, flag);
   unsigned int* miss_ctr = fresh_counter(ctx);
   if (!miss_ctr) return pclean_fail(ctx, PCLEAN_ERR_HIP, "counter bank: device alloc failed");
-  hipLaunchKernelGGL(compact_new_kernel, grid1(N), dim3(256), 0, ctx->stream, (size_t)N, flag, 1, miss_ctr, list, nullptr);
+  const CountPub miss_pub = count_pub(ctx);
+  hipLaunchKernelGGL(compact_new_kernel, grid1(N), dim3(256), 0, ctx->stream, (size_t)N, flag, 1, miss_ctr, list, nullptr, miss_pub);
   unsigned int n_miss = 0;
-  PCLEAN_READ_COUNT(ctx, miss_ctr, &n_miss);
+  PCLEAN_READ_COUNT_PUB(ctx, miss_pub, miss_ctr, &n_miss);
   if (n_miss == 0) return PCLEAN_OK;
   if (n_miss == (unsigned int)N) {
     int rc = eval_node_lse_core(ctx, block_id, node_id, il, excl, seed, sweep, lse_out);
@@ -2380,17 +2468,25 @@
                          t.cols.p + (size_t)cn.parent_fk_col * t.n_rows, ce);
       child_excl = ce;
     }
+    SweepState* s = st(ctx);
+    if (pclean_fold_on() && cn.kind == PCLEAN_NODE_LEAF && il.origin)
+      s->vals_req = SweepState::ValsReq{vals + cid, il.origin, n_nodes};
     int rc = eval_node(ctx, block_id, cid, il, child_excl, seed, sweep, 1, nullptr, draws, nullptr, nullptr, false);
+    const bool stored = s->vals_done;
+    s->vals_req = SweepState::ValsReq();
+    s->vals_done = false;
     if (rc) return rc;
-    hipLaunchKernelGGL(scatter_vals_kernel, grid1(il.n), dim3(256), 0, ctx->stream, il.n, il.origin, draws, n_nodes,
-                       cid, vals);
+    if (!stored)
+      hipLaunchKernelGGL(scatter_vals_kernel, grid1(il.n), dim3(256), 0, ctx->stream, il.n, il.origin, draws, n_nodes,
+                         cid, vals);
     if (cn.kind == PCLEAN_NODE_FK && cn.n_children > 0) {
       unsigned int* new_ctr = fresh_counter(ctx);
       if (!new_ctr) return pclean_fail(ctx, PCLEAN_ERR_HIP, "counter bank: device alloc failed");
+      const CountPub new_pub = count_pub(ctx);
       hipLaunchKernelGGL(compact_new_kernel, grid1(il.n), dim3(256), 0, ctx->stream, (size_t)il.n, draws, 0, new_ctr, nullptr,
-                         nullptr);
+                         nullptr, new_pub);
       unsigned int cnt = 0;
-      PCLEAN_READ_COUNT(ctx, new_ctr, &cnt);
+      PCLEAN_READ_COUNT_PUB(ctx, new_pub, new_ctr, &cnt);
       if (cnt) {
         int32_t* list = scratch<int32_t>(ctx, cnt);
         int32_t* row = scratch<int32_t>(ctx, cnt);
diff --git a/pclean_amd/csrc/sweep.hip b/pclean_amd/csrc/sweep.hip
--- a/pclean_amd/csrc/sweep.hip
+++ b/pclean_amd/csrc/sweep.hip
@@ -10,42 +10,75 @@
   __threadfence_system();
   dst[1] = seq;
 }
-int read_count(pclean_ctx* ctx, const void* dev, void* out, const char* func, int line) {
-  SweepState* s = st(ctx);
+#define POLL_SLOTS 8
+static bool poll_ready(SweepState* s) {
   static const bool no_poll = getenv("PCLEAN_NO_POLL") != nullptr;
-  static const bool trace = getenv("PCLEAN_TRACE_SYNC") != nullptr;
-  if (trace) fprintf(stderr, "[pclean sync %d] %s:%d (count)\n", ++g_pclean_sync_count, func, line);
-  if (!no_poll && !s->h_poll) {
-    if (hipHostMalloc((void**)&s->h_poll, 64, hipHostMallocMapped | hipHostMallocCoherent) != hipSuccess) s->h_poll = nullptr;
+  if (no_poll) return false;
+  if (!s->h_poll) {
+    if (hipHostMalloc((void**)&s->h_poll, 2 * POLL_SLOTS * sizeof(unsigned int), hipHostMallocMapped | hipHostMallocCoherent) != hipSuccess)
+      s->h_poll = nullptr;
     if (s->h_poll) {
-      s->h_poll[0] = s->h_poll[1] = 0;
+      for (int k = 0; k < 2 * POLL_SLOTS; ++k) s->h_poll[k] = 0;
       if (hipHostGetDevicePointer((void**)&s->d_poll, (void*)s->h_poll, 0) != hipSuccess) {
         (void)hipHostFree((void*)s->h_poll);
         s->h_poll = nullptr;
       }
     }
   }
-  if (no_poll || !s->h_poll) {
-    HIPCHK(ctx, hipMemcpyAsync(out, dev, 4, hipMemcpyDeviceToHost, ctx->stream));
-    HIPCHK(ctx, hipStreamSynchronize(ctx->stream));
-    return PCLEAN_OK;
-  }
-  const unsigned int seq = ++s->poll_seq;
-  hipLaunchKernelGGL(publish_count_kernel, dim3(1), dim3(1), 0, ctx->stream, (const unsigned int*)dev, s->d_poll, seq);
+  return s->h_poll != nullptr;
+}
+static int wait_count(pclean_ctx* ctx, unsigned int seq, void* out) {
+  SweepState* s = st(ctx);
   if (s->on_first_wait) {
     std::function<int()> f;
     f.swap(s->on_first_wait);
     const int rcf = f();
     if (rcf) return rcf;
   }
-  volatile unsigned int* h = s->h_poll;
+  if (s->poll_seq - seq >= POLL_SLOTS) return pclean_fail(ctx, PCLEAN_ERR_STATE, "count read-back: %u reads since the count's producer was queued", s->poll_seq - seq);
+  volatile unsigned int* h = s->h_poll + 2 * (seq % POLL_SLOTS);
   for (long spins = 0; h[1] != seq; ++spins)
     if (spins > 2000000) {
       HIPCHK(ctx, hipStreamSynchronize(ctx->stream));
-      if (h[1] != seq) return pclean_fail(ctx, PCLEAN_ERR_HIP, "count read-back: the publishing kernel did not run");
+      if (h[1] != seq) {
+        s->pub_tickets.release();
+        return pclean_fail(ctx, PCLEAN_ERR_HIP, "count read-back: the publishing kernel did not run");
+      }
     }
   *(unsigned int*)out = h[0];
   return PCLEAN_OK;
+}
+int read_count(pclean_ctx* ctx, const void* dev, void* out, const char* func, int line) {
+  SweepState* s = st(ctx);
+  static const bool trace = getenv("PCLEAN_TRACE_SYNC") != nullptr;
+  if (trace) fprintf(stderr, "[pclean sync %d] %s:%d (count)\n", ++g_pclean_sync_count, func, line);
+  if (!poll_ready(s)) {
+    HIPCHK(ctx, hipMemcpyAsync(out, dev, 4, hipMemcpyDeviceToHost, ctx->stream));
+    HIPCHK(ctx, hipStreamSynchronize(ctx->stream));
+    return PCLEAN_OK;
+  }
+  const unsigned int seq = ++s->poll_seq;
+  hipLaunchKernelGGL(publish_count_kernel, dim3(1), dim3(1), 0, ctx->stream, (const unsigned int*)dev, s->d_poll + 2 * (seq % POLL_SLOTS), seq);
+  return wait_count(ctx, seq, out);
+}
+CountPub count_pub(pclean_ctx* ctx) {
+  SweepState* s = st(ctx);
+  if (!pclean_fold_on() || !poll_ready(s)) return CountPub();
+  if (!s->pub_tickets.p) {
+    if (s->pub_tickets.alloc((size_t)(1 + PUB_MAX_GROUPS) * PUB_LINE) ||
+        hipMemsetAsync(s->pub_tickets.p, 0, (size_t)(1 + PUB_MAX_GROUPS) * PUB_LINE * sizeof(unsigned int), ctx->stream) != hipSuccess) {
+      s->pub_tickets.release();
+      return CountPub();
+    }
+  }
+  const unsigned int seq = ++s->poll_seq;
+  return CountPub{s->pub_tickets.p, s->d_poll + 2 * (seq % POLL_SLOTS), seq};
+}
+int read_count_pub(pclean_ctx* ctx, const CountPub& pub, const void* dev, void* out, const char* func, int line) {
+  if (!pub.ticket) return read_count(ctx, dev, out, func, line);
+  static const bool trace = getenv("PCLEAN_TRACE_SYNC") != nullptr;
+  if (trace) fprintf(stderr, "[pclean sync %d] %s:%d (count)\n", ++g_pclean_sync_count, func, line);
+  return wait_count(ctx, pub.seq, out);
 }
 
 __device__ int32_t resolve_new_value(const PlanDev& pl, int node, int col, const int32_t* vals) {
@@ -256,7 +289,8 @@
                                                               int32_t* __restrict__ new_list,
                                                               int32_t* __restrict__ pnewpos, int first,
                                                               const int32_t* __restrict__ emit_rows, int only_emit,
-                                                              int stage_stride, const double* __restrict__ w_uni, int skip_w) {
+                                                              int stage_stride, const double* __restrict__ w_uni, int skip_w,
+                                                              CountPub pub) {
   __shared__ unsigned int wsum[PU_T / 64];
   __shared__ unsigned int bbase;
   extern __shared__ int32_t pu_stage[];
@@ -292,7 +326,10 @@
       pchoice[sp] = c;
       if (!skip_w) w[sp] = first ? 0.0 + l : (w_uni ? (0.0 + w_uni[i]) + l : w[sp] + l);
       if (c == PCLEAN_CHOICE_NEW) newmask |= 1ull << p;
-      if (p == 0 && !(l > -__builtin_inf())) atomicOr(n_new, 0x80000000u);
+      if (p == 0 && !(l > -__builtin_inf())) {
+        const unsigned int old = atomicOr(n_new, 0x80000000u);
+        if (pub.ticket) asm volatile("" ::"v"(old));
+      }
     }
     if (emit_rows && !emit_rows[i]) newmask = 0;
   }
@@ -308,6 +345,7 @@
     unsigned int total = 0;
     for (int k = 0; k < PU_T / 64; ++k) total += wsum[k];
     bbase = total ? (atomicAdd(n_new, total) & 0x7fffffffu) : 0u;
+    if (pub.ticket) publish_if_last(pub, n_new, blockIdx.x, gridDim.x, total != 0u);
   }
   __syncthreads();
   if (!mine) return;
@@ -416,6 +454,20 @@
   int j = blockIdx.x * blockDim.x + threadIdx.x;
   if (j < n) vals[(size_t)j * n_nodes + node] = v;
 }
+__global__ void rootlist_vals_kernel(int n, int N, size_t NP, const int32_t* list, const int32_t* b_ctx, const int32_t* cur_b,
+                                     int32_t* row, int32_t* ctxv, int32_t* particle, int32_t* origin, int32_t* excl, int n_nodes,
+                                     int32_t* vals) {
+  int j = blockIdx.x * blockDim.x + threadIdx.x;
+  if (j >= n) return;
+  const int slot = list[j];
+  const int i = slot % N;
+  row[j] = i;
+  particle[j] = slot / N;
+  origin[j] = j;
+  excl[j] = cur_b ? cur_b[i] : -1;
+  for (int c = 0; c < PCLEAN_MAX_CTX; ++c) ctxv[j * PCLEAN_MAX_CTX + c] = b_ctx ? b_ctx[(size_t)c * NP + slot] : 0;
+  for (int k = 0; k < n_nodes; ++k) vals[(size_t)j * n_nodes + k] = k == 0 ? (int32_t)PCLEAN_CHOICE_NEW : -2;
+}
 __global__ void gather_items_kernel(int n, const int32_t* list, const int32_t* row, const int32_t* ctxv,
                                     const int32_t* excl, const int32_t* particle, int32_t* row2, int32_t* ctx2,
                                     int32_t* excl2, int32_t* part2) {
@@ -670,13 +722,17 @@
 #define TAIL_WG_THREADS 1024
 #define TAIL_STEP (TAIL_WG_THREADS / TAIL_TILE_ROWS)
 __global__ __launch_bounds__(TAIL_WG_THREADS) void finalize_tail_kernel(int n_rows, int n_tiles, const int32_t* __restrict__ chosen,
-                                                                        TailBlocks tb) {
+                                                                        TailBlocks tb, CountPub pub, int pub_block) {
   extern __shared__ int32_t hist[];
   __shared__ unsigned int wcnt[2][2][TAIL_WG_THREADS / 64];
   const TailBlock& b = tb.b[blockIdx.y];
   if (!b.on) return;
+  const bool pubs = pub.ticket && (int)blockIdx.y == pub_block;
   const TailTileRange tr = tail_tile_range(n_tiles, (int)gridDim.x, (int)blockIdx.x);
-  if (tr.begin >= tr.end) return;
+  if (tr.begin >= tr.end) {
+    if (pubs && threadIdx.x == 0) publish_if_last(pub, b.new_ctr, blockIdx.x, gridDim.x, false);
+    return;
+  }
   const int hist_rows = b.hist_rows;
   const int lane = threadIdx.x & 63, wave = threadIdx.x >> 6;
   const int sub = threadIdx.x / TAIL_TILE_ROWS, in_tile = threadIdx.x % TAIL_TILE_ROWS;
@@ -755,6 +811,7 @@
       b.wg_new[tile] = wcnt[par][1][wave] + wcnt[par][1][wave + 1] + wcnt[par][1][wave + 2] + wcnt[par][1][wave + 3];
     }
   }
+  if (pubs && threadIdx.x == 0) publish_if_last(pub, b.new_ctr, blockIdx.x, gridDim.x, false);
   if (hist_rows) {
     __syncthreads();
     for (int k = threadIdx.x; k < hist_rows; k += TAIL_WG_THREADS) {
@@ -1081,6 +1138,7 @@
   }
   if (s->side_fork) (void)hipEventDestroy(s->side_fork);
   if (s->h_poll) (void)hipHostFree((void*)s->h_poll);
+  s->pub_tickets.release();
   s->dummy_dp.release();
   s->dummy_ctr.release();
   s->over_ctr.release();
@@ -1099,7 +1157,7 @@
   ctx->sweep_state = nullptr;
 }
 
-int begin_call(pclean_ctx* ctx) {
+int begin_call(pclean_ctx* ctx, bool caller_zeroes) {
   SweepState* s = st(ctx);
   s->pool_used = 0;
   s->dbg_desc = nullptr;
@@ -1107,7 +1165,7 @@
   ctx->prior_mode = false;
   s->over_rec.clear();
   if (s->over_ctr.alloc(OVER_SLOTS + STAT_WORDS + CTR_BANK)) return pclean_fail(ctx, PCLEAN_ERR_HIP, "device alloc failed");
-  { const int rcz = dev_zero(ctx, s->over_ctr.p, (OVER_SLOTS + STAT_WORDS + CTR_BANK) * sizeof(unsigned int)); if (rcz) return rcz; }
+  if (!caller_zeroes) { const int rcz = dev_zero(ctx, s->over_ctr.p, (OVER_SLOTS + STAT_WORDS + CTR_BANK) * sizeof(unsigned int)); if (rcz) return rcz; }
   s->bank_used = 0;
   s->scan_stats_used = false;
   return PCLEAN_OK;
@@ -1713,6 +1771,7 @@
   bool final_fused = false;
   const int32_t* final_only_rows = nullptr;
   bool hot_timed = false, prefetching = false, prefetch_started = false;
+  bool zero_over_ctr = false;
   const int32_t* cur_of(int bi) const { return cur_base + (size_t)bi * cur_ld; }
   ~SweepCall() {
     s->on_first_wait = nullptr;
@@ -1766,8 +1825,16 @@
   c.s->last_dev_cur = dev_cur;
   (void)hipEventRecord(c.s->evs, c.ctx->stream);
   c.w_by_first_block = !c.ctx->block[0].is_score;
-  if (!c.w_by_first_block) { const int rcz = dev_zero(c.ctx, c.s->w.p, c.NP * sizeof(double)); if (rcz) return rcz; }
-  { const int rcz = dev_zero(c.ctx, c.s->logml_acc.p, (size_t)N * sizeof(double)); if (rcz) return rcz; }
+  if (c.zero_over_ctr) {
+    ZeroList zl{};
+    zero_list_add(c.ctx, zl, c.s->over_ctr.p, (OVER_SLOTS + STAT_WORDS + CTR_BANK) * sizeof(unsigned int));
+    if (!c.w_by_first_block) zero_list_add(c.ctx, zl, c.s->w.p, c.NP * sizeof(double));
+    zero_list_add(c.ctx, zl, c.s->logml_acc.p, (size_t)N * sizeof(double));
+    if (const int rcz = zero_list_flush(c.ctx, zl)) return rcz;
+  } else {
+    if (!c.w_by_first_block) { const int rcz = dev_zero(c.ctx, c.s->w.p, c.NP * sizeof(double)); if (rcz) return rcz; }
+    { const int rcz = dev_zero(c.ctx, c.s->logml_acc.p, (size_t)N * sizeof(double)); if (rcz) return rcz; }
+  }
   c.ctx->timing = pclean_timing{};
   if (!c.s->pre_stream) {
     HIPCHK(c.ctx, hipStreamCreateWithFlags(&c.s->pre_stream, hipStreamNonBlocking));
@@ -1835,6 +1902,7 @@
   const int32_t* emit_rows = nullptr;
   bool fuse_final = false, split_final = false;
   unsigned int* n_new_ctr = nullptr;
+  CountPub n_new_pub;
 };
 struct DrawSrc {
   const int32_t* draws_rm;
@@ -1864,13 +1932,13 @@
   return PCLEAN_OK;
 }
 static int launch_particle_update(SweepCall& c, int bi, const DrawSrc& d, const int32_t* emit_rows, bool split, bool skip_w,
-                                  unsigned int* n_new_ctr) {
+                                  unsigned int* n_new_ctr, const CountPub& pub) {
   BlockRun& r = c.s->run[bi];
   const bool rm = d.draws_rm != nullptr;
   hipLaunchKernelGGL(particle_update_kernel, dim3((c.N + PU_T - 1) / PU_T), dim3(PU_T), rm ? c.pu_stage_bytes : 0, c.ctx->stream,
                      c.N, c.P, d.draws_rm, d.lse_rm, d.slot_item, d.draws_item, d.lse_item, c.cur_of(bi), r.pchoice.p, c.s->w.p,
                      n_new_ctr, r.new_slots.p, r.pnewpos.p, (c.w_by_first_block && bi == 0) ? 1 : 0, emit_rows, split ? 1 : 0,
-                     rm ? c.pu_stage_stride : 0, c.w_uni, skip_w ? 1 : 0);
+                     rm ? c.pu_stage_stride : 0, c.w_uni, skip_w ? 1 : 0, pub);
   HIPCHK(c.ctx, hipGetLastError());
   return PCLEAN_OK;
 }
@@ -1913,7 +1981,8 @@
   }
   if (!(bs.n_new_ctr = fresh_counter(c.ctx))) return pclean_fail(c.ctx, PCLEAN_ERR_HIP, "counter bank: device alloc failed");
   const bool skip_w = bi == 0 && c.w_by_first_block && bi < c.n_blocks - 1 && !bs.split_final && !bs.emit_rows && !c.sw.no_w_uni;
-  if (const int rc = launch_particle_update(c, bi, d, bs.emit_rows, bs.split_final, skip_w, bs.n_new_ctr)) return rc;
+  bs.n_new_pub = count_pub(c.ctx);
+  if (const int rc = launch_particle_update(c, bi, d, bs.emit_rows, bs.split_final, skip_w, bs.n_new_ctr, bs.n_new_pub)) return rc;
   if (skip_w || !bs.split_final) c.w_uni = skip_w ? c.s->run[bi].lse.p : nullptr;
   if (!bs.split_final) return PCLEAN_OK;
   launch_update_final(c, bi, d, bs.emit_rows, lazy.valid);
@@ -1929,7 +1998,9 @@
   if (rc) return rc;
   { const int rcz = dev_zero(c.ctx, r.lse.p, (size_t)c.N * sizeof(double)); if (rcz) return rcz; }
   if (!(bs.n_new_ctr = fresh_counter(c.ctx))) return pclean_fail(c.ctx, PCLEAN_ERR_HIP, "counter bank: device alloc failed");
-  const int rcu = launch_particle_update(c, bi, DrawSrc{r.draws.p, r.lse.p, nullptr, nullptr, nullptr}, nullptr, false, false, bs.n_new_ctr);
+  bs.n_new_pub = count_pub(c.ctx);
+  const int rcu = launch_particle_update(c, bi, DrawSrc{r.draws.p, r.lse.p, nullptr, nullptr, nullptr}, nullptr, false, false, bs.n_new_ctr,
+                                         bs.n_new_pub);
   if (rcu) return rcu;
   if (b.n_ctx > 0) {
     { const int rci = ensure_it_ctx(c.ctx, r, c.NP, b.n_ctx); if (rci) return rci; }
@@ -2049,16 +2120,22 @@
   Block& b = c.ctx->block[bi];
   BlockRun& r = c.s->run[bi];
   const int nn = (int)b.nodes.size();
-  hipLaunchKernelGGL(fill_i32_kernel, grid1((size_t)count * nn), dim3(256), 0, c.ctx->stream, r.vals.p, (size_t)count * nn, -2);
+  const bool fold = pclean_fold_on();
+  if (!fold) hipLaunchKernelGGL(fill_i32_kernel, grid1((size_t)count * nn), dim3(256), 0, c.ctx->stream, r.vals.p, (size_t)count * nn, -2);
   int32_t* row = scratch<int32_t>(c.ctx, count);
   int32_t* cx = scratch<int32_t>(c.ctx, (size_t)count * PCLEAN_MAX_CTX);
   int32_t* part = scratch<int32_t>(c.ctx, count);
   int32_t* org = scratch<int32_t>(c.ctx, count);
   int32_t* ex = scratch<int32_t>(c.ctx, count);
   if (!row || !cx || !part || !org || !ex) return pclean_fail(c.ctx, PCLEAN_ERR_HIP, "scratch alloc failed");
-  hipLaunchKernelGGL(rootlist_items_kernel, grid1(count), dim3(256), 0, c.ctx->stream, (int)count, c.N, c.NP, r.new_slots.p,
-                     b.n_ctx > 0 ? r.it_ctx.p : nullptr, c.cur_of(bi), row, cx, part, org, ex);
-  hipLaunchKernelGGL(set_col_kernel, grid1(count), dim3(256), 0, c.ctx->stream, (int)count, nn, 0, (int32_t)PCLEAN_CHOICE_NEW, r.vals.p);
+  if (fold) {
+    hipLaunchKernelGGL(rootlist_vals_kernel, grid1(count), dim3(256), 0, c.ctx->stream, (int)count, c.N, c.NP, r.new_slots.p,
+                       b.n_ctx > 0 ? r.it_ctx.p : nullptr, c.cur_of(bi), row, cx, part, org, ex, nn, r.vals.p);
+  } else {
+    hipLaunchKernelGGL(rootlist_items_kernel, grid1(count), dim3(256), 0, c.ctx->stream, (int)count, c.N, c.NP, r.new_slots.p,
+                       b.n_ctx > 0 ? r.it_ctx.p : nullptr, c.cur_of(bi), row, cx, part, org, ex);
+    hipLaunchKernelGGL(set_col_kernel, grid1(count), dim3(256), 0, c.ctx->stream, (int)count, nn, 0, (int32_t)PCLEAN_CHOICE_NEW, r.vals.p);
+  }
   ItemList sub{(int)count, row, cx, part, org};
   return sample_children(c.ctx, bi, 0, sub, ex, c.seed, c.sweep_idx, r.vals.p, nn);
 }
@@ -2096,7 +2173,7 @@
   BlockRun& r = c.s->run[bi];
   const int nn = (int)c.ctx->block[bi].nodes.size();
   unsigned int n_new = 0;
-  if (!c.final_fused) PCLEAN_READ_COUNT(c.ctx, bs.n_new_ctr, &n_new);
+  if (!c.final_fused) PCLEAN_READ_COUNT_PUB(c.ctx, bs.n_new_pub, bs.n_new_ctr, &n_new);
   const bool degenerate_rows = (n_new & 0x80000000u) != 0u;
   n_new &= 0x7fffffffu;
   r.n_new = c.final_fused ? -1 : (int)n_new;
@@ -2156,6 +2233,8 @@
   int nb_wg = 0;
   unsigned int* wg_cnt = nullptr;
   unsigned int* chosen_ctr[PCLEAN_MAX_BLOCKS] = {};
+  CountPub chosen_pub;
+  int pub_block = -1;
   int hist_rows[PCLEAN_MAX_BLOCKS] = {};
   TailLists tl{};
   ZeroList zl{};
@@ -2165,7 +2244,7 @@
   ProfScope ps2(c.ctx, "new_row_sampling_chosen");
   const int nn = (int)c.ctx->block[bi].nodes.size();
   unsigned int cnt = 0;
-  PCLEAN_READ_COUNT(c.ctx, t.chosen_ctr[bi], &cnt);
+  PCLEAN_READ_COUNT_PUB(c.ctx, bi == t.pub_block ? t.chosen_pub : CountPub(), t.chosen_ctr[bi], &cnt);
   if (c.sw.trace_tail)
     fprintf(stderr, "[pclean tail] block %d: %u chosen NEW rows listed by %s\n", bi, cnt,
             c.sw.no_fused_finalize ? "chosen_new_kernel" : "finalize_tail_kernel");
@@ -2208,8 +2287,16 @@
   if (c.sw.trace_tail)
     fprintf(stderr, "[pclean tail] finalize_tail_kernel: %d tiles, %d workgroups per block, at most %d tiles per workgroup\n",
             t.nb_wg, n_wgs, (t.nb_wg + n_wgs - 1) / n_wgs);
+  int n_listed = 0;
+  for (int bi = 0; bi < c.n_blocks; ++bi)
+    if (t.chosen_ctr[bi]) {
+      ++n_listed;
+      t.pub_block = bi;
+    }
+  if (n_listed == 1) t.chosen_pub = count_pub(c.ctx);
+  if (!t.chosen_pub.ticket) t.pub_block = -1;
   hipLaunchKernelGGL(finalize_tail_kernel, dim3(n_wgs, c.n_blocks), dim3(TAIL_WG_THREADS), (size_t)max_hist * sizeof(int32_t), c.ctx->stream,
-                     c.N, t.nb_wg, c.s->chosen.p, tb);
+                     c.N, t.nb_wg, c.s->chosen.p, tb, t.chosen_pub, t.pub_block);
   int rc = tail_lists(c, t);
   for (int bi = 0; bi < c.n_blocks && !rc; ++bi)
     if (t.chosen_ctr[bi]) rc = sample_chosen(c, t, bi);
@@ -2329,9 +2416,11 @@
   for (int b = 0; b < n_blocks; ++b)
     if (!ctx->block[b].valid) return pclean_fail(ctx, PCLEAN_ERR_STATE, "pclean_sweep: block %d not loaded", b);
   HIPCHK(ctx, hipSetDevice(ctx->device));
-  if (const int rc = begin_call(ctx)) return rc;
+  static const bool fold_zero = pclean_fold_on() && getenv("PCLEAN_NO_ZERO_KERNEL") == nullptr;
+  if (const int rc = begin_call(ctx, fold_zero)) return rc;
   static const SweepSwitches sw;
   SweepCall call{ctx, st(ctx), cfg, sw, N, P, n_blocks, (size_t)N * P, seed, sweep_idx, use_mh, prior_mode};
+  call.zero_over_ctr = fold_zero;
   if (const int rc = sweep_begin(call, cur, dev_cur)) return rc;
   for (int bi = 0; bi < n_blocks; ++bi) {
     if (ctx->block[bi].is_score) {
diff --git a/pclean_amd/csrc/sweep_internal.h b/pclean_amd/csrc/sweep_internal.h
--- a/pclean_amd/csrc/sweep_internal.h
+++ b/pclean_amd/csrc/sweep_internal.h
@@ -21,6 +21,43 @@
     const int rc_ = read_count(ctx, (dev), (out), __func__, __LINE__);    \
     if (rc_) return rc_;                                                  \
   } while (0)
+
+static inline bool pclean_fold_on() {
+  static const bool on = getenv("PCLEAN_NO_FOLD") == nullptr;
+  return on;
+}
+#define PUB_LINE 32
+#define PUB_MAX_GROUPS 256
+struct CountPub {
+  unsigned int* ticket = nullptr;
+  volatile unsigned int* dst = nullptr;
+  unsigned int seq = 0;
+};
+CountPub count_pub(pclean_ctx* ctx);
+int read_count_pub(pclean_ctx* ctx, const CountPub& pub, const void* dev, void* out, const char* func, int line);
+#define PCLEAN_READ_COUNT_PUB(ctx, pub, dev, out)                                   \
+  do {                                                                              \
+    const int rc_ = read_count_pub(ctx, (pub), (dev), (out), __func__, __LINE__);   \
+    if (rc_) return rc_;                                                            \
+  } while (0)
+__device__ __forceinline__ void publish_if_last(const CountPub& pb, const unsigned int* counter, unsigned int wg, unsigned int n_wgs,
+                                                bool added) {
+  if (added) asm volatile("s_waitcnt vmcnt(0)" ::: "memory");
+  const unsigned int G = max(64u, (n_wgs + PUB_MAX_GROUPS - 1) / PUB_MAX_GROUPS);
+  const unsigned int n_groups = (n_wgs + G - 1) / G;
+  if (n_groups > 1) {
+    const unsigned int g = wg / G, size_g = min(G, n_wgs - g * G);
+    if (__hip_atomic_fetch_add(pb.ticket + (size_t)(1 + g) * PUB_LINE, 1u, __ATOMIC_RELAXED, __HIP_MEMORY_SCOPE_AGENT) != size_g - 1u) return;
+  }
+  const unsigned int last = n_groups > 1 ? n_groups - 1u : n_wgs - 1u;
+  if (__hip_atomic_fetch_add(pb.ticket, 1u, __ATOMIC_RELAXED, __HIP_MEMORY_SCOPE_AGENT) != last) return;
+  const unsigned int v = __hip_atomic_load(counter, __ATOMIC_RELAXED, __HIP_MEMORY_SCOPE_AGENT);
+  pb.dst[0] = v;
+  __threadfence_system();
+  pb.dst[1] = pb.seq;
+  for (unsigned int g = 0; g <= (n_groups > 1 ? n_groups : 0u); ++g)
+    __hip_atomic_store(pb.ticket + (size_t)g * PUB_LINE, 0u, __ATOMIC_RELAXED, __HIP_MEMORY_SCOPE_AGENT);
+}
 
 #define PCLEAN_SYNC(ctx)                                                                                   \
   do {                                                                                                     \
@@ -191,7 +228,8 @@
 }
 
 static __global__ __launch_bounds__(256) void compact_new_kernel(size_t n, const int32_t* choice, int fill,
-                                                          unsigned int* counter, int32_t* list, int32_t* pos_out) {
+                                                          unsigned int* counter, int32_t* list, int32_t* pos_out,
+                                                          CountPub pub = CountPub()) {
   __shared__ unsigned int wcnt[4];
   __shared__ unsigned int bbase;
   const size_t t = (size_t)blockIdx.x * blockDim.x + threadIdx.x;
@@ -203,6 +241,7 @@
   if (threadIdx.x == 0) {
     const unsigned int total = wcnt[0] + wcnt[1] + wcnt[2] + wcnt[3];
     bbase = total ? atomicAdd(counter, total) : 0u;
+    if (pub.ticket) publish_if_last(pub, counter, blockIdx.x, gridDim.x, total != 0u);
   }
   __syncthreads();
   if (t >= n || !fill) return;
@@ -246,7 +285,7 @@
   if (j < n) dst[j] = src[list[j]];
 }
 
-int begin_call(pclean_ctx* ctx);
+int begin_call(pclean_ctx* ctx, bool caller_zeroes = false);
 int queue_over_copy(pclean_ctx* ctx);
 void apply_over_stats(pclean_ctx* ctx);
 int finish_call(pclean_ctx* ctx);
diff --git a/pclean_amd/csrc/sweep_state.h b/pclean_amd/csrc/sweep_state.h
--- a/pclean_amd/csrc/sweep_state.h
+++ b/pclean_amd/csrc/sweep_state.h
@@ -71,6 +71,7 @@
   volatile unsigned int* h_poll = nullptr;
   unsigned int* d_poll = nullptr;
   unsigned int poll_seq = 0;
+  DevBuf<unsigned int> pub_tickets;
   bool outputs_pending = false;
   bool lists_on_host = false;
   DevBuf<double> w, log_total, logml_inc, logml_acc, logml;
@@ -150,6 +151,8 @@
   bool dummy_used = false;
   struct LazyReq { bool on = false; const int32_t* eager_rows = nullptr; } lazy_req;
   struct LazyOut { bool valid = false; LazyDrawArgs args{}; uint32_t site = 0; } lazy_out;
+  struct ValsReq { int32_t* dst = nullptr; const int32_t* origin = nullptr; int stride = 0; } vals_req;
+  bool vals_done = false;
   const int32_t* dbg_desc = nullptr;
   const int32_t* dbg_grp_off = nullptr;
   const int32_t* dbg_members = nullptr;
```

New measurement: 465.3 million (median of 6 runs). +1.1%, better.
